# GRAPH-0/JODO

Hardware: AMD Instinct MI355X
Metric: molecules/sec (1000-step ancestral) (higher is better)
Workload: dtype f32

## Files before the change

include/jodo_hip.h:

```cpp
#ifndef JODO_HIP_H
#define JODO_HIP_H
#include <stddef.h>
#include <stdint.h>
#ifdef __cplusplus
extern "C" {
#endif

#define JODO_OK 0
#define JODO_ERR_ARG (-1)
#define JODO_ERR_LAUNCH (-2)
#define JODO_ERR_UNSUPPORTED (-3)

typedef struct {
    int32_t nf;
    int32_t n_layers;
    int32_t n_heads;
    int32_t n_extra;
    int32_t mlp_ratio;
    int32_t in_node_dim;
    int32_t edge_ch;
    int32_t cond_ch;
    float spatial_cut_off;
    float edge_quan_th;
    int32_t layout;
} jodo_cfg;

enum jodo_wslot_global {
    JW_TIME_FREQ = 0, JW_TIME_W1, JW_TIME_B1, JW_TIME_W3, JW_TIME_B3,
    JW_COND_W0, JW_COND_B0, JW_COND_W2, JW_COND_B2, JW_COND_LIN_W, JW_COND_LIN_B,
    JW_MOD_W, JW_MOD_B,
    JW_NODE_EMB_W, JW_NODE_EMB_B, JW_EDGE_EMB_W, JW_EDGE_EMB_B, JW_GBF_TOP,
    JW_NH1_W, JW_NH1_B, JW_NH2_W, JW_NH2_B, JW_NH3_W, JW_NH3_B,
    JW_EH1_W, JW_EH1_B, JW_EH2_W, JW_EH2_B, JW_EH3_W, JW_EH3_B,
    JW_GLOBAL_COUNT
};
enum jodo_wslot_block {
    JB_WQ = 0, JB_BQ, JB_WK, JB_BK, JB_WV, JB_BV,
    JB_EE_W, JB_EE_B, JB_LE0_W, JB_LE1_W, JB_N2E_W, JB_N2E_B,
    JB_FF1_W, JB_FF1_B, JB_FF2_W, JB_FF2_B, JB_FF3_W, JB_FF3_B, JB_FF4_W, JB_FF4_B,
    JB_INE_W, JB_ROW_W, JB_COL_W, JB_IN_B, JB_C0_W, JB_C0_B, JB_C2_W, JB_CSCALE,
    JB_NRO_W, JB_NRO_B, JB_ERO_W, JB_ERO_B, JB_GBF,
    JB_ROWQ_W, JB_COLQ_W, JB_INQ_B, JB_LQ_W, JB_INEC_W, JB_QT_W,
    JB_BLOCK_COUNT
};

typedef struct {
    const char* name;
    const float* data;
    const int64_t* shape;
    int32_t ndim;
} jodo_tensor;
int jodo_dgt_packed_size(const jodo_cfg* cfg, const jodo_tensor* tensors, int n_tensors, size_t* n_floats, int* n_woff);
int jodo_dgt_pack_weights_host(const jodo_cfg* cfg, const jodo_tensor* tensors, int n_tensors, float* packed_host,
                               size_t cap_floats, int64_t* woff_out, int n_woff);
int jodo_dgt_pack_weights(const jodo_cfg* cfg, const jodo_tensor* tensors, int n_tensors, void* packed_dev,
                          size_t cap_floats, int64_t* woff_out, int n_woff, void* stream);

typedef struct jodo_plan jodo_plan;

int jodo_plan_create(const jodo_cfg* cfg, int B, int N, const int32_t* n_nodes_host, int max_chunk,
                     jodo_plan** out);
void jodo_plan_destroy(jodo_plan* plan);
size_t jodo_plan_desc_bytes(const jodo_plan* plan);
size_t jodo_plan_workspace_bytes(const jodo_plan* plan);
int64_t jodo_plan_mod_len(const jodo_plan* plan);
int jodo_plan_upload(jodo_plan* plan, void* desc_dev, void* stream);
int jodo_plan_stats(const jodo_plan* plan, int64_t* out6);

int jodo_dgt_forward(jodo_plan* plan, const void* desc_dev, const float* packed_w, const int64_t* woff,
                     int n_woff, const float* xh, const float* edge_x, const float* cond_x,
                     const float* cond_edge_x, const float* noise_level, const float* context,
                     float* out_xh, float* out_edge, int32_t* flags_dev, void* workspace, void* stream);

int jodo_plan_work(const jodo_plan* plan, int uniform_t, int symmetric, double* mfma_flops_per_class);

enum jodo_plan_option {
    JODO_OPT_FUSE_NEXT_QKV = 0,
    JODO_OPT_DIR_SPLIT = 1,
    JODO_OPT_NODE_POST_WAVES = 2,
    JODO_OPT_ATTN_VARIANT = 3,
    JODO_OPT_PIN_SYMMETRIC = 4,
    JODO_OPT_PIN_UNIFORM_T = 5,
    JODO_OPT_ROT_STATS = 6,
    JODO_OPT_NODE_MIX = 7,
    JODO_OPT_HEADS_MIX = 8,
    JODO_OPT_HALF_ROWS = 9,
    JODO_OPT_PRE_EMBED = 10,
    JODO_OPT_AB_PRE = 11,
    JODO_OPT_Z_SPLIT = 12,
    JODO_OPT_SPLIT_BF16 = 13,
    JODO_OPT_COUNT
};
int jodo_plan_set_option(jodo_plan* plan, int option, int value);

int jodo_debug_attn_schedule(const jodo_plan* plan, int64_t* out8);

int jodo_debug_fetch(jodo_plan* plan, const void* workspace, int what, float* dst_dev, int64_t* count,
                     void* stream);
int jodo_debug_set_max_blocks(jodo_plan* plan, int max_blocks);
int jodo_debug_set_force_directed(jodo_plan* plan, int on);
int jodo_debug_set_timing_buffer(jodo_plan* plan, void* dev16xu64);

enum jodo_prof_class {
    JODO_PROF_PROLOGUE = 0, JODO_PROF_NODE_PRE, JODO_PROF_EDGE_ATTN, JODO_PROF_RESERVED3, JODO_PROF_RESERVED4,
    JODO_PROF_NODE_POST, JODO_PROF_EDGE_UPDATE, JODO_PROF_EPILOGUE, JODO_PROF_COUNT
};
int jodo_profile_enable(jodo_plan* plan, int enable);
int jodo_profile_read(jodo_plan* plan, float* ms_sum, int32_t* launches);

int jodo_sampler_step(int B, int N, int node_feats, int edge_ch, const int32_t* n_nodes_dev, float c_x, float c_pred,
                      float sigma, const float* x, const float* edge_x, const float* pred, const float* edge_pred,
                      const float* eps_pos, const float* eps_feat, const float* eps_edge, float* x_next,
                      float* edge_next, float* x_mean, float* edge_mean, void* stream);
int jodo_sampler_step_tab(int B, int N, int node_feats, int edge_ch, const int32_t* n_nodes_dev, const float* coef_tab_dev,
                          const int32_t* step_dev, const float* x, const float* edge_x, const float* pred,
                          const float* edge_pred, const float* eps_pos, const float* eps_feat, const float* eps_edge,
                          float* x_next, float* edge_next, float* x_mean, float* edge_mean, void* stream);
int jodo_sampler_step_rng(int B, int N, int node_feats, int edge_ch, const int32_t* n_nodes_dev, float c_x, float c_pred,
                          float sigma, const float* coef_tab_dev, const int32_t* step_dev, uint64_t seed, uint32_t draw,
                          const float* x, const float* edge_x, const float* pred, const float* edge_pred, float* x_next,
                          float* edge_next, float* x_mean, float* edge_mean, void* stream);
int jodo_step_begin(int B, const float* coef_tab_dev, const int32_t* step_dev, float* noise_level_out, void* stream);
int jodo_step_end(int32_t* step_dev, void* stream);
int jodo_dpm_update(int B, int N, int node_feats, int edge_ch, const int32_t* n_nodes_dev, const float* coef8_host,
                    const float* coef_tab_dev, const int32_t* step_dev, int tab_stride, int tab_col, const float* x_pos,
                    const float* x_base, const float* edge_base, const float* P, const float* eP, const float* DA, const float* eDA,
                    const float* DB, const float* eDB, const float* PP, const float* eps_pos, float* x_out, float* edge_out,
                    void* stream);
int jodo_dpm_update_rng(int B, int N, int node_feats, int edge_ch, const int32_t* n_nodes_dev, const float* coef8_host,
                        const float* coef_tab_dev, const int32_t* step_dev, int tab_stride, int tab_col, uint64_t seed,
                        uint32_t draw, uint32_t draw_mul, const float* x_pos, const float* x_base, const float* edge_base,
                        const float* P, const float* eP, const float* DA, const float* eDA, const float* DB, const float* eDB,
                        const float* PP, float* x_out, float* edge_out, void* stream);
int jodo_step_begin_at(int B, const float* coef_tab_dev, const int32_t* step_dev, int tab_stride, int tab_col,
                       float* noise_level_out, void* stream);
int jodo_decode(int B, int N, int atom_types, int include_fc, int edge_ch, int compress_edge, int centered,
                float pos_norm, float atom_norm, float fc_norm, float edge_norm, const int32_t* n_nodes_dev,
                const float* xh, const float* edge_x, float* pos_out, uint8_t* atom_type_out, int8_t* fc_out,
                uint8_t* edge_type_out, void* stream);

typedef struct jodo_train jodo_train;
int jodo_train_create(const jodo_cfg* cfg, int B, int N, const int32_t* n_nodes_host, const jodo_tensor* params, int n_params,
                      jodo_train** out);
void jodo_train_destroy(jodo_train* t);
size_t jodo_train_desc_bytes(const jodo_train* t);
size_t jodo_train_workspace_bytes(const jodo_train* t);
int jodo_train_set_option(jodo_train* t, int option, int value);
int jodo_train_debug_locate(const jodo_train* t, int what, int layer, size_t* byte_offset, size_t* count);
int jodo_train_upload(jodo_train* t, void* desc_dev, void* stream);
const void* jodo_train_desc_host(const jodo_train* t);
int jodo_train_forward(jodo_train* t, const void* desc_dev, const float* const* params_dev, int n_params, const float* xh,
                       const float* edge_x, const float* cond_x, const float* cond_edge_x, const float* noise_level,
                       const float* context, float dropout_p, uint64_t seed, float* out_xh, float* out_edge, int32_t* flags_out,
                       void* workspace, void* stream);
int jodo_train_backward(jodo_train* t, const void* desc_dev, const float* const* params_dev, float* const* grads_dev, int n_params,
                        const float* noise_level, const float* d_out_xh, const float* d_out_edge, float dropout_p, uint64_t seed,
                        void* workspace, void* stream);
int jodo_train_gemm(int tA, int tB, int M, int N, int K, const float* A, int lda, const float* B, int ldb, float* C, int ldc,
                    const float* bias, int acc, float* ws, size_t ws_floats, void* stream);
int jodo_train_gemm_ex(int tA, int tB, int M, int N, int K, const float* A, int lda, const float* B, int ldb, float* C, int ldc,
                       const float* bias, int act, float* out2, float* dbias, float* ws, size_t ws_floats, void* stream);

int jodo_adam_step(int64_t n, float* p, const float* g, float* m, float* v, float* vmax, double lr, double beta1, double beta2, double eps,
                   double weight_decay, int64_t step, int decoupled, int amsgrad, void* stream);
int jodo_gradnorm_clip(const float* norm_dev, double* state_dev, double max_grad, float* coef_dev, float* allowed_dev, void* stream);
int jodo_kabsch_rotations(int B, const float* A_dev, float* R_dev, void* stream);

typedef struct {
    int32_t nf, n_layers, n_heads, n_extra, mlp_ratio, in_node_dim, edge_ch;
    float edge_quan_th;
} jodo_cfg2d;
enum jodo2d_wslot_global {
    J2_TIME_FREQ = 0, J2_TIME_W1, J2_TIME_B1, J2_TIME_W3, J2_TIME_B3, J2_MOD_W, J2_MOD_B,
    J2_NODE_EMB_W, J2_NODE_EMB_B, J2_EDGE_EMB_W, J2_EDGE_EMB_B,
    J2_NH1_W, J2_NH1_B, J2_NH2_W, J2_NH2_B, J2_NH3_W, J2_NH3_B,
    J2_EH1_W, J2_EH1_B, J2_EH2_W, J2_EH2_B, J2_EH3_W, J2_EH3_B,
    J2_GLOBAL_COUNT
};
enum jodo2d_wslot_block {
    J2B_QKV_W = 0, J2B_QKV_B, J2B_LE_W, J2B_N2E_W, J2B_N2E_B, J2B_FF1_W, J2B_FF1_B, J2B_FF2_W, J2B_FF2_B,
    J2B_FF3_W, J2B_FF3_B, J2B_FF4_W, J2B_FF4_B, J2B_NRO_W, J2B_NRO_B, J2B_ERO_W, J2B_ERO_B,
    J2B_BLOCK_COUNT
};
int jodo_dgt2d_check_cfg(const jodo_cfg2d* cfg);
int jodo_dgt2d_packed_size(const jodo_cfg2d* cfg, size_t* n_floats, int* n_woff);
int jodo_dgt2d_pack_weights_host(const jodo_cfg2d* cfg, const jodo_tensor* tensors, int n_tensors, float* packed_host,
                                 size_t cap_floats, int64_t* woff_out, int n_woff);
int jodo_dgt2d_layout(const jodo_cfg2d* cfg, int B, int N, const int32_t* n_nodes_host, int64_t* out8);
int jodo_dgt2d_fill_desc(const jodo_cfg2d* cfg, int B, int N, const int32_t* n_nodes_host, int32_t* desc_host, int64_t n_words);
int jodo_dgt2d_forward(const jodo_cfg2d* cfg, int B, int N, const int32_t* n_nodes_host, const void* desc_dev, const float* packed_w,
                       const int64_t* woff, int n_woff, const float* xh, const float* edge_x, const float* cond_x,
                       const float* cond_edge_x, const float* noise_level, float* out_xh, float* out_edge, int32_t* flags_dev,
                       void* workspace, int force_directed, int max_blocks, void* stream);
enum jodo2d_walk { JODO_2D_WALK_DIRECTED = 0, JODO_2D_WALK_PAIR = 1 };
int jodo_dgt2d_pair_layout(const jodo_cfg2d* cfg, int B, int N, const int32_t* n_nodes_host, int64_t* out8);
int jodo_dgt2d_pair_fill_desc(const jodo_cfg2d* cfg, int B, int N, const int32_t* n_nodes_host, int32_t* desc_host, int64_t n_words);
int jodo_dgt2d_forward_walk(const jodo_cfg2d* cfg, int B, int N, const int32_t* n_nodes_host, const void* desc_dev,
                            const void* pair_desc_dev, int walk, const float* packed_w, const int64_t* woff, int n_woff, const float* xh,
                            const float* edge_x, const float* cond_x, const float* cond_edge_x, const float* noise_level, float* out_xh,
                            float* out_edge, int32_t* flags_dev, void* workspace, int force_directed, int max_blocks, void* stream);
int jodo_dgt2d_split_size(const jodo_cfg2d* cfg, size_t* tape_bytes, int64_t* toff_out, int n_woff);
int jodo_dgt2d_pack_split_host(const jodo_cfg2d* cfg, const float* packed_host, const int64_t* woff, int n_woff, void* tape_host,
                               size_t cap_bytes);
int jodo_dgt2d_forward_split(const jodo_cfg2d* cfg, int B, int N, const int32_t* n_nodes_host, const void* desc_dev,
                             const void* pair_desc_dev, int walk, const float* packed_w, const int64_t* woff, int n_woff,
                             const void* tape_dev, const int64_t* toff, const float* xh, const float* edge_x, const float* cond_x,
                             const float* cond_edge_x, const float* noise_level, float* out_xh, float* out_edge, int32_t* flags_dev,
                             void* workspace, int force_directed, int max_blocks, void* stream);
int jodo_debug_gemm2d(int split, const float* x, int rows, int K, int n_out, const void* w_dev, const float* bias, int act, float* y,
                      void* stream);
int jodo_sampler_step_2d(int B, int N, int node_feats, int edge_ch, const int32_t* n_nodes_dev, float cx, float cp, float sigma,
                         const float* x, const float* edge_x, const float* pred, const float* edge_pred, const float* eps_node,
                         const float* eps_edge, float* x_next, float* edge_next, float* x_mean, float* edge_mean, void* stream);
int jodo_sampler_step_2d_rng(int B, int N, int node_feats, int edge_ch, const int32_t* n_nodes_dev, float c_x, float c_pred, float sigma,
                             const float* coef_tab_dev, const int32_t* step_dev, uint64_t seed, uint32_t draw, const float* x,
                             const float* edge_x, const float* pred, const float* edge_pred, float* x_next, float* edge_next,
                             float* x_mean, float* edge_mean, void* stream);
int jodo_dpm_update_2d(int B, int N, int node_feats, int edge_ch, const int32_t* n_nodes_dev, const float* coef8_host,
                       const float* coef_tab_dev, const int32_t* step_dev, int tab_stride, int tab_col, const float* x_base,
                       const float* edge_base, const float* P, const float* eP, const float* DA, const float* eDA, const float* DB,
                       const float* eDB, float* x_out, float* edge_out, void* stream);
int jodo_decode_2d(int B, int N, int atom_types, int include_fc, int edge_ch, int compress_edge, int centered, float atom_norm,
                   float fc_norm, float edge_norm, const int32_t* n_nodes_dev, const float* xh, const float* edge_x,
                   uint8_t* atom_type_out, int8_t* fc_out, uint8_t* edge_type_out, void* stream);

typedef struct jodo_train2d jodo_train2d;
int jodo_train2d_create(const jodo_cfg2d* cfg, int B, int N, const int32_t* n_nodes_host, const jodo_tensor* params, int n_params,
                        jodo_train2d** out);
void jodo_train2d_destroy(jodo_train2d* t);
size_t jodo_train2d_desc_bytes(const jodo_train2d* t);
size_t jodo_train2d_workspace_bytes(const jodo_train2d* t);
const void* jodo_train2d_desc_host(const jodo_train2d* t);
int jodo_train2d_upload(jodo_train2d* t, void* desc_dev, void* stream);
int jodo_train2d_set_option(jodo_train2d* t, int option, int value);
int jodo_train2d_debug_locate(const jodo_train2d* t, int what, int layer, size_t* byte_offset, size_t* count);
int jodo_train2d_forward(jodo_train2d* t, const void* desc_dev, const float* const* params_dev, int n_params, const float* xh,
                         const float* edge_x, const float* cond_x, const float* cond_edge_x, const float* noise_level,
                         const float* context, float dropout_p, uint64_t seed, float* out_xh, float* out_edge, int32_t* flags_out,
                         void* workspace, void* stream);
int jodo_train2d_backward(jodo_train2d* t, const void* desc_dev, const float* const* params_dev, float* const* grads_dev, int n_params,
                          const float* noise_level, const float* d_out_xh, const float* d_out_edge, float dropout_p, uint64_t seed,
                          void* workspace, void* stream);

const char* jodo_last_error(void);

int jodo_debug_mfma_peak(int iters, int chains, int waves_per_simd, float* sink_dev, float* tflops_out);

int jodo_debug_mfma_valu(int iters, int nv, int nt, int waves_per_simd, float* sink_dev, float* tflops_out);

int jodo_dgt_split_size(const jodo_cfg* cfg, size_t* total_bytes, size_t* pair_block_bytes, size_t* node_block_bytes, size_t* attn_block_bytes);
int jodo_dgt_pack_split_host(const jodo_cfg* cfg, const jodo_tensor* tensors, int n_tensors, void* host, size_t cap_bytes);
int jodo_plan_set_split_weights(jodo_plan* plan, const void* tape_dev, size_t bytes);
int jodo_dgt_split_cond_size(const jodo_cfg* cfg, size_t* total_bytes, size_t* pair_block_bytes);
int jodo_dgt_pack_split_cond_host(const jodo_cfg* cfg, const jodo_tensor* tensors, int n_tensors, void* host, size_t cap_bytes);

int jodo_debug_mfma_bf16_valu(int iters, int nv, int chains, int waves_per_simd, float* sink_dev, float* tflops_out);
int jodo_debug_pack_split(const float* W, int n_out, int n_in, float* f32_packed_host, void* split_packed_host);
int jodo_debug_chain(int mode, int K, int tiles, const float* x, int rows, const float* wf, const void* wsp, float* y, int iters,
                     float* ms_out, void* stream);

int jodo_debug_mlp(const float* x, int rows, const float* w1, const float* b1, const float* w2,
                   const float* b2, float* y, void* stream);

#ifdef __cplusplus
}
#endif
#endif
```

jodo_amd/capi.py:

```python
import ctypes
import os

_HERE = os.path.dirname(os.path.abspath(__file__))
LIB_PATH = os.environ.get('JODO_HIP_LIB') or os.path.join(_HERE, 'csrc', 'libjodo_hip.so')
_lib = None


class JodoHipError(RuntimeError):
    pass


def lib():
    global _lib
    if _lib is None:
        if not os.path.isfile(LIB_PATH):
            raise JodoHipError(
                "libjodo_hip.so not found at %s — the HIP extension is required (no CPU fallback). "
                "Build it with: python -c 'import __graft_entry__ as g; g.build()'" % LIB_PATH)
        _lib = ctypes.CDLL(LIB_PATH)
        _lib.jodo_last_error.restype = ctypes.c_char_p
        _bind_2d_sampling(_lib)
        _bind_2d_pair(_lib)
        _bind_2d_split(_lib)
    return _lib


def _bind_2d_sampling(L):
    i, f, p = ctypes.c_int, ctypes.c_float, ctypes.c_void_p
    try:
        step, dec, dpm = L.jodo_sampler_step_2d_rng, L.jodo_decode_2d, L.jodo_dpm_update_2d
    except AttributeError as e:
        raise JodoHipError("%s lacks the 2-D sampling exports (%s): rebuild it with python -c 'import __graft_entry__ as g; g.build()'"
                           % (LIB_PATH, e))
    step.argtypes = [i, i, i, i, p, f, f, f, p, p, ctypes.c_uint64, ctypes.c_uint32] + [p] * 9
    dec.argtypes = [i] * 7 + [f, f, f] + [p] * 7
    dpm.argtypes = [i, i, i, i, p, p, p, p, i, i] + [p] * 11
    step.restype = dec.restype = dpm.restype = i


WALK_DIRECTED, WALK_PAIR = 0, 1


def _bind_2d_pair(L):
    i, p = ctypes.c_int, ctypes.c_void_p
    try:
        lay, fill, fwd = L.jodo_dgt2d_pair_layout, L.jodo_dgt2d_pair_fill_desc, L.jodo_dgt2d_forward_walk
    except AttributeError as e:
        raise JodoHipError("%s lacks the 2-D pair-walk exports (%s): rebuild it with python -c 'import __graft_entry__ as g; g.build()'"
                           % (LIB_PATH, e))
    lay.argtypes = [p, i, i, p, p]
    fill.argtypes = [p, i, i, p, p, ctypes.c_int64]
    fwd.argtypes = [p, i, i, p, p, p, i, p, p, i] + [p] * 9 + [i, i, p]
    lay.restype = fill.restype = fwd.restype = i


def _bind_2d_split(L):
    i, p = ctypes.c_int, ctypes.c_void_p
    try:
        size, pack, fwd, dbg = L.jodo_dgt2d_split_size, L.jodo_dgt2d_pack_split_host, L.jodo_dgt2d_forward_split, L.jodo_debug_gemm2d
    except AttributeError as e:
        raise JodoHipError("%s lacks the 2-D split-bf16 exports (%s): rebuild it with python -c 'import __graft_entry__ as g; g.build()'"
                           % (LIB_PATH, e))
    size.argtypes = [p, p, p, i]
    pack.argtypes = [p, p, p, i, p, ctypes.c_size_t]
    fwd.argtypes = [p, i, i, p, p, p, i, p, p, i, p, p] + [p] * 9 + [i, i, p]
    dbg.argtypes = [i, p, i, i, i, p, p, i, p, p]
    size.restype = pack.restype = fwd.restype = dbg.restype = i


def check(code, what=''):
    if code != 0:
        msg = lib().jodo_last_error()
        raise JodoHipError("%s failed (%d): %s" % (what, code, msg.decode() if msg else ''))


def ptr(t):
    if t is None:
        return ctypes.c_void_p(0)
    return ctypes.c_void_p(t.data_ptr())


def current_stream_ptr():
    import torch
    return ctypes.c_void_p(torch.cuda.current_stream().cuda_stream)


class JodoTensor(ctypes.Structure):
    _fields_ = [('name', ctypes.c_char_p), ('data', ctypes.c_void_p), ('shape', ctypes.POINTER(ctypes.c_int64)),
                ('ndim', ctypes.c_int32)]


_PACKED_SIZE = {}


def pack_weights(cfg_struct, state_dict, device=None):
    import numpy as np
    import torch
    L = lib()
    keep, arr = [], (JodoTensor * len(state_dict))()
    for i, (k, v) in enumerate(state_dict.items()):
        t = np.ascontiguousarray(v.detach().float().cpu().numpy())
        shp = (ctypes.c_int64 * max(t.ndim, 1))(*t.shape)
        name = k.encode()
        keep.append((t, shp, name))
        arr[i] = JodoTensor(name, t.ctypes.data_as(ctypes.c_void_p), shp, t.ndim)
    key = bytes(cfg_struct)
    n_floats, n_woff = ctypes.c_size_t(), ctypes.c_int()
    if key in _PACKED_SIZE:
        n_floats.value, n_woff.value = _PACKED_SIZE[key]
    else:
        check(L.jodo_dgt_packed_size(ctypes.byref(cfg_struct), arr, len(keep), ctypes.byref(n_floats), ctypes.byref(n_woff)),
              'jodo_dgt_packed_size')
        _PACKED_SIZE[key] = (n_floats.value, n_woff.value)
    woff = (ctypes.c_int64 * n_woff.value)()
    if device is None:
        blob = torch.empty(n_floats.value, dtype=torch.float32)
        check(L.jodo_dgt_pack_weights_host(ctypes.byref(cfg_struct), arr, len(keep), ctypes.c_void_p(blob.data_ptr()),
                                           ctypes.c_size_t(n_floats.value), woff, n_woff.value), 'jodo_dgt_pack_weights_host')
    else:
        blob = torch.empty(n_floats.value, dtype=torch.float32, device=device)
        check(L.jodo_dgt_pack_weights(ctypes.byref(cfg_struct), arr, len(keep), ctypes.c_void_p(blob.data_ptr()),
                                      ctypes.c_size_t(n_floats.value), woff, n_woff.value, current_stream_ptr()),
              'jodo_dgt_pack_weights')
    return blob, woff, n_woff.value


def pack_weights_2d(cfg_struct, state_dict, device=None):
    import numpy as np
    import torch
    L = lib()
    keep, arr = [], (JodoTensor * len(state_dict))()
    for i, (k, v) in enumerate(state_dict.items()):
        t = np.ascontiguousarray(v.detach().float().cpu().numpy())
        shp = (ctypes.c_int64 * max(t.ndim, 1))(*t.shape)
        name = k.encode()
        keep.append((t, shp, name))
        arr[i] = JodoTensor(name, t.ctypes.data_as(ctypes.c_void_p), shp, t.ndim)
    n_floats, n_woff = ctypes.c_size_t(), ctypes.c_int()
    check(L.jodo_dgt2d_packed_size(ctypes.byref(cfg_struct), ctypes.byref(n_floats), ctypes.byref(n_woff)), 'jodo_dgt2d_packed_size')
    woff = (ctypes.c_int64 * n_woff.value)()
    blob = torch.empty(n_floats.value, dtype=torch.float32)
    check(L.jodo_dgt2d_pack_weights_host(ctypes.byref(cfg_struct), arr, len(keep), ctypes.c_void_p(blob.data_ptr()),
                                         ctypes.c_size_t(n_floats.value), woff, n_woff.value), 'jodo_dgt2d_pack_weights_host')
    return (blob if device is None else blob.to(device)), woff, n_woff.value


def split_tape_2d(cfg_struct, blob_host, woff, n_woff, device=None):
    import torch
    L = lib()
    total = ctypes.c_size_t()
    toff = (ctypes.c_int64 * n_woff)()
    check(L.jodo_dgt2d_split_size(ctypes.byref(cfg_struct), ctypes.byref(total), toff, n_woff), 'jodo_dgt2d_split_size')
    tape = torch.empty(total.value, dtype=torch.uint8)
    check(L.jodo_dgt2d_pack_split_host(ctypes.byref(cfg_struct), ctypes.c_void_p(blob_host.data_ptr()), woff, n_woff,
                                       ctypes.c_void_p(tape.data_ptr()), ctypes.c_size_t(total.value)), 'jodo_dgt2d_pack_split_host')
    return (tape if device is None else tape.to(device)), toff


def pack_split_tape(cfg_struct, state_dict, device=None):
    import numpy as np
    import torch
    L = lib()
    keep, arr = [], (JodoTensor * len(state_dict))()
    for i, (k, v) in enumerate(state_dict.items()):
        t = np.ascontiguousarray(v.detach().float().cpu().numpy())
        shp = (ctypes.c_int64 * max(t.ndim, 1))(*t.shape)
        name = k.encode()
        keep.append((t, shp, name))
        arr[i] = JodoTensor(name, t.ctypes.data_as(ctypes.c_void_p), shp, t.ndim)
    total, per_block, node_block, attn_block = ctypes.c_size_t(), ctypes.c_size_t(), ctypes.c_size_t(), ctypes.c_size_t()
    check(L.jodo_dgt_split_size(ctypes.byref(cfg_struct), ctypes.byref(total), ctypes.byref(per_block), ctypes.byref(node_block), ctypes.byref(attn_block)),
          'jodo_dgt_split_size')
    tape = torch.empty(total.value, dtype=torch.uint8)
    check(L.jodo_dgt_pack_split_host(ctypes.byref(cfg_struct), arr, len(keep), ctypes.c_void_p(tape.data_ptr()), ctypes.c_size_t(total.value)),
          'jodo_dgt_pack_split_host')
    return tape if device is None else tape.to(device)


def pack_split_cond_tape(cfg_struct, state_dict, device=None):
    import numpy as np
    import torch
    L = lib()
    keep, arr = [], (JodoTensor * len(state_dict))()
    for i, (k, v) in enumerate(state_dict.items()):
        t = np.ascontiguousarray(v.detach().float().cpu().numpy())
        shp = (ctypes.c_int64 * max(t.ndim, 1))(*t.shape)
        name = k.encode()
        keep.append((t, shp, name))
        arr[i] = JodoTensor(name, t.ctypes.data_as(ctypes.c_void_p), shp, t.ndim)
    total, per_block = ctypes.c_size_t(), ctypes.c_size_t()
    check(L.jodo_dgt_split_cond_size(ctypes.byref(cfg_struct), ctypes.byref(total), ctypes.byref(per_block)), 'jodo_dgt_split_cond_size')
    tape = torch.empty(total.value, dtype=torch.uint8)
    check(L.jodo_dgt_pack_split_cond_host(ctypes.byref(cfg_struct), arr, len(keep), ctypes.c_void_p(tape.data_ptr()), ctypes.c_size_t(total.value)),
          'jodo_dgt_pack_split_cond_host')
    return tape if device is None else tape.to(device)
```

jodo_amd/csrc/dgt_forward.hip:

```cpp
#include "dgt_kernels_pre.h"
#include "dgt_kernels_node.h"
#include "dgt_kernels_split_node.h"
#include "dgt_kernels_post.h"
#include "dgt_kernels_wide.h"
#include "jodo_hip_internal.h"
#include "dgt_launch.h"
#include <memory>
#include <utility>

using namespace jd;

namespace {

PlanDev make_plan_dev(const jodo_plan* p, const void* desc_dev) {
    const int* base = static_cast<const int*>(desc_dev);
    PlanDev d;
    d.node_b = base + p->off_node_b; d.node_i = base + p->off_node_i; d.node_n = base + p->off_node_n;
    d.node_noff = base + p->off_node_noff; d.node_eoff = base + p->off_node_eoff;
    d.orig_n = base + p->off_orig_n; d.orig_noff = base + p->off_orig_noff; d.orig_eoff = base + p->off_orig_eoff;
    d.item_strip = base + p->off_item_strip; d.item_t0 = base + p->off_item_t0; d.item_t1 = base + p->off_item_t1;
    d.item_part = base + p->off_item_part; d.strip_parts = base + p->off_strip_parts;
    d.pitem_strip = base + p->off_pitem_strip; d.pitem_t0 = base + p->off_pitem_t0; d.pitem_t1 = base + p->off_pitem_t1;
    d.n_pitems = p->n_pitems;
    d.ag_node = base + p->off_ag_node; d.ai_group = base + p->off_ai_group; d.ai_t0 = base + p->off_ai_t0; d.ai_t1 = base + p->off_ai_t1;
    d.ai_part = base + p->off_ai_part; d.ai_dir = base + p->off_ai_dir; d.ad_group = base + p->off_ad_group; d.ad_t0 = base + p->off_ad_t0; d.ad_t1 = base + p->off_ad_t1;
    d.ad_part = base + p->off_ad_part; d.ad_big = base + p->off_ad_big; d.anode_parts = base + p->off_anode_parts;
    d.aw_off = base + p->off_aw_off; d.a_persist = p->a_persist;
    d.n_agroups = p->n_agroups; d.n_aitems = p->n_aitems; d.n_aditems = p->n_aditems; d.amax_parts = p->amax_parts;
    d.Nn = p->Nn; d.Nn_pad = p->Nn_pad; d.n_strips = p->n_strips; d.n_items = p->n_items; d.B = p->B; d.N = p->N;
    d.max_parts = p->max_parts; d.rows = p->rows;
    d.ut_rows = base + p->off_ut_rows; d.n_ut_pad = p->n_ut_pad;
    d.gt_sa = base + p->off_gt_sa; d.gt_sc = base + p->off_gt_sc; d.n_gtiles = p->n_gtiles;
    return d;
}

template <typename T>
T* ws_ptr(void* ws, size_t off) { return reinterpret_cast<T*>(static_cast<char*>(ws) + off); }

void fill_ws(KArgs& A, const jodo_plan* p, void* ws) {
    const WsLayout& w = p->ws;
    A.hid1 = ws_ptr<float>(ws, w.hid1); A.temb = ws_ptr<float>(ws, w.temb); A.mods = ws_ptr<float>(ws, w.mods);
    A.condh = ws_ptr<float>(ws, w.condh); A.condh2 = ws_ptr<float>(ws, w.condh2);
    A.dpos = ws_ptr<float>(ws, w.dpos); A.cpos = ws_ptr<float>(ws, w.cpos); A.feat = ws_ptr<float>(ws, w.feat);
    A.h = ws_ptr<float>(ws, w.h); A.hhat = ws_ptr<float>(ws, w.hhat); A.astat = ws_ptr<float>(ws, w.astat); A.q = ws_ptr<float>(ws, w.q);
    A.k = ws_ptr<float>(ws, w.k); A.v = ws_ptr<float>(ws, w.v); A.n2e = ws_ptr<float>(ws, w.n2e);
    A.wrow = ws_ptr<float>(ws, w.wrow); A.wcol = ws_ptr<float>(ws, w.wcol); A.ua = ws_ptr<float>(ws, w.ua); A.ub = ws_ptr<float>(ws, w.ub);
    A.rmean = ws_ptr<float>(ws, w.rmean); A.mfold = ws_ptr<float>(ws, w.mfold); A.ffold = ws_ptr<float>(ws, w.ffold); A.ahid = ws_ptr<float>(ws, w.ahid);
    A.apred = ws_ptr<float>(ws, w.apred);
    A.eflag = ws_ptr<int>(ws, w.eflag); A.e = ws_ptr<float>(ws, w.e);
    A.ehid = ws_ptr<float>(ws, w.ehid); A.epred = ws_ptr<float>(ws, w.epred);
    A.e_out = ws_ptr<float>(ws, w.e2);
    A.dposE = ws_ptr<float>(ws, w.dposE); A.gramE = ws_ptr<float>(ws, w.gramE);
    A.wsplit = nullptr; A.wsplit_node = nullptr; A.wsplit_attn = nullptr; A.mfold_s = nullptr; A.ffold_s = nullptr; A.split_cond = 0;
}

int rowgemm(hipStream_t st, const float* X, int64_t ldx, float* Y, int64_t ldy, const float* Wp, const float* bias,
            int rows, int K, int NB, int in_act, int accumulate, const int* uniform_flag, float* Ysilu = nullptr) {
    if (K % 64 != 0) return jodo_set_error(JODO_ERR_ARG, "rowgemm: K=%d not a multiple of 64", K);
    const int nob = (rows <= 64 || uniform_flag) ? 1 : 4;
    const int gx = uniform_flag ? 1 : 0;
    RowGemmArgs G{X, ldx, Y, ldy, Wp, bias, rows, K, NB, in_act, accumulate, uniform_flag, nob, gx, Ysilu};
    dim3 grid((rows + 31) / 32, (NB + nob - 1) / nob);
    if (gx) grid = dim3(grid.y, grid.x);
    hipLaunchKernelGGL(k_rowgemm, grid, dim3(64), 0, st, G);
    return jodo_check_launch("k_rowgemm");
}

struct ProfScope {
    jodo_plan* p; hipStream_t st; int cls; bool on;
    static hipEvent_t get(jodo_plan* p) {
        if (!p->prof_pool.empty()) { hipEvent_t e = (hipEvent_t)p->prof_pool.back(); p->prof_pool.pop_back(); return e; }
        hipEvent_t e; (void)hipEventCreate(&e); return e;
    }
    ProfScope(jodo_plan* p_, hipStream_t st_, int cls_)
        : p(p_), st(st_), cls(cls_), on(p_->prof_enabled == 1 || (p_->prof_enabled == 2 && cls_ == JODO_PROF_EDGE_UPDATE) || p_->prof_enabled == 16 + cls_) {
        if (on) { hipEvent_t e = get(p); (void)hipEventRecord(e, st); p->prof_ev.push_back(e); }
    }
    ~ProfScope() {
        if (on) { hipEvent_t e = get(p); (void)hipEventRecord(e, st); p->prof_ev.push_back(e); p->prof_cls.push_back(cls); }
    }
};

template <int D, int KQ>
int launch_embed_nodes(hipStream_t st, const KArgs& A) {
    LAUNCH((wide::k_embed_nodes<D, KQ>), A.pd.n_strips, 64, A);
    return JODO_OK;
}
template <int D, int NBK>
int launch_edge_head(hipStream_t st, const KArgs& A, bool merged) {
    if (merged) {
        LAUNCH((wide::k_heads_sym<D, NBK>), (unsigned)(A.pd.n_strips + A.pd.n_ut_pad / 32), 64, A);
        return JODO_OK;
    }
    LAUNCH((wide::k_node_head<D>), A.pd.n_strips, 64, A);
    if (A.pd.n_ut_pad > 0 && A.pin_sym != 2) LAUNCH((wide::k_edge_head<D, NBK, true>), (unsigned)(A.pd.n_ut_pad / 32), 64, A);
    if (A.pin_sym != 1) LAUNCH((wide::k_edge_head<D, NBK, false>), (unsigned)((A.pd.rows + 31) / 32), 64, A);
    return JODO_OK;
}

__global__ __launch_bounds__(64, 1) void k_pre_embed(KArgs A) {
    const int npre = A.pd.n_strips * 3;
    if ((int)blockIdx.x < npre) node_pre_body<false>(A, (int)blockIdx.x);
    else wide::embed_edges_body<256>(A, (int)blockIdx.x - npre);
}


__global__ __launch_bounds__(64, 1) void k_node_ab_pre(KArgs A) {
    const int npre = A.mix_nw, nab = A.ab1 - A.ab0;
    const int b = (int)blockIdx.x;
    if (b < npre) node_pre_body<true>(A, b);
    else if (b < npre + nab) wide::node_ab_body<256>(A, A.ab0 + b - npre);
    else wide::node_gram_body<256>(A, A.g0 + b - npre - nab);
}

template <int D>
__global__ __launch_bounds__(64, 1) void k_node_ab_pre_w(KArgs A) {
    const int npre = A.mix_nw, nab = A.ab1 - A.ab0;
    const int b = (int)blockIdx.x;
    if (b < npre) wide::node_pre_body<D, true>(A, b);
    else if (b < npre + nab) wide::node_ab_body<D>(A, A.ab0 + b - npre);
    else wide::node_gram_body<D>(A, A.g0 + b - npre - nab);
}
template <int D>
__global__ __launch_bounds__(64, 1) void k_pre_embed_w(KArgs A) {
    const int npre = A.pd.n_strips * 3;
    if ((int)blockIdx.x < npre) wide::node_pre_body<D, false>(A, (int)blockIdx.x);
    else wide::embed_edges_body<D>(A, (int)blockIdx.x - npre);
}

template <int R, int NW>
__global__ __launch_bounds__(NW * 64, 1) void k_node_mix(KArgs A) {
    __shared__ float4 part[NW * 8 * 4 * 64];
    const int wg = blockIdx.x, wave = threadIdx.x >> 6;
    if (wg < A.mix_nw) { node_postw_body<R, NW>(A, wg + A.strip0, part); return; }
    const int nab = (A.ab1 - A.ab0 + NW - 1) / NW;
    if (wg < A.mix_nw + nab) {
        const int it = A.ab0 + (wg - A.mix_nw) * NW + wave;
        if (it < A.ab1) wide::node_ab_body<256>(A, it);
        return;
    }
    const int t = A.g0 + (wg - A.mix_nw - nab) * NW + wave;
    if (t < A.g1) wide::node_gram_body<256>(A, t);
}

int launch_node_post_256(jodo_plan* p, hipStream_t st, KArgs& A, bool with_ab, bool next_pre) {
    const DgtDims& d = p->dims;
    const int force = p->opt[JODO_OPT_NODE_POST_WAVES];
    const bool rem_only = force >= 10;
    const int full = (force && !rem_only) ? (force == 1 ? p->n_strips : 0) : (p->n_strips / 1024) * 1024;
    const int rem = p->n_strips - full;
    const int nw = rem_only ? force - 10 : (force ? force : (rem <= 256 ? 4 : (rem <= 512 ? 2 : 1)));
    const bool split_node = A.wsplit_node != nullptr && A.rot == 1;
    if (split_node) {
        A.strip0 = 0;
        const int wgs = (p->n_strips + 3) / 4;
        if (d.r == 2) { LAUNCH((split::k_node_post_split<2, 1>), wgs, split::SPLIT_WAVES * 64, A); LAUNCH((split::k_node_post_split<2, 2>), wgs, split::SPLIT_WAVES * 64, A); }
        else { LAUNCH((split::k_node_post_split<4, 1>), wgs, split::SPLIT_WAVES * 64, A); LAUNCH((split::k_node_post_split<4, 2>), wgs, split::SPLIT_WAVES * 64, A); }
    }
    const bool split_ab = split_node && with_ab && A.ffold_s != nullptr && !next_pre;
    if (split_ab) {
        A.ab0 = 0; A.ab1 = 2 * p->n_strips;
        LAUNCH(split::k_node_ab_split, (2 * p->n_strips + split::SPLIT_WAVES - 1) / split::SPLIT_WAVES, split::SPLIT_WAVES * 64, A);
    }
    if (full > 0 && !split_node) {
        A.strip0 = 0;
        if (d.r == 2) LAUNCH(k_node_post<2>, full, 64, A); else LAUNCH(k_node_post<4>, full, 64, A);
    }
    A.ab0 = 0; A.ab1 = 2 * p->n_strips; A.g0 = 0; A.g1 = A.rot ? p->n_gtiles : 0; A.mix_nw = 0;
    const bool mix = !split_node && with_ab && full > 0 && rem > 0 && nw >= 2 && p->opt[JODO_OPT_NODE_MIX] != 0;
    if (mix) {
        if (p->gt_cache_full != full) {
            const int32_t* sa = p->desc.data() + p->off_gt_sa, *sc = p->desc.data() + p->off_gt_sc;
            int c = 0;
            while (c < p->n_gtiles && sa[c] < full && sc[c] < full) ++c;
            p->gt_cache_full = full; p->gt_cache_count = c;
        }
        const int gpre = A.rot ? p->gt_cache_count : 0;
        A.strip0 = full; A.mix_nw = rem; A.ab0 = 0; A.ab1 = 2 * full; A.g0 = 0; A.g1 = gpre;
        const int g1 = rem + (A.ab1 - A.ab0 + nw - 1) / nw + (A.g1 - A.g0 + nw - 1) / nw;
        if (nw == 2) { if (d.r == 2) LAUNCH((k_node_mix<2, 2>), g1, 128, A); else LAUNCH((k_node_mix<4, 2>), g1, 128, A); }
        else { if (d.r == 2) LAUNCH((k_node_mix<2, 4>), g1, 256, A); else LAUNCH((k_node_mix<4, 4>), g1, 256, A); }
        A.strip0 = 0; A.mix_nw = 0; A.ab0 = 2 * full; A.ab1 = 2 * p->n_strips; A.g0 = gpre; A.g1 = A.rot ? p->n_gtiles : 0;
        const int g2 = (A.ab1 - A.ab0 + 1) / 2 + (A.g1 - A.g0 + 1) / 2;
        if (d.r == 2) LAUNCH((k_node_mix<2, 2>), g2, 128, A); else LAUNCH((k_node_mix<4, 2>), g2, 128, A);
        A.ab0 = 0; A.g0 = 0;
        return JODO_OK;
    }
    if (rem > 0 && !split_node) {
        A.strip0 = full;
        if (nw == 1) { if (d.r == 2) LAUNCH(k_node_post<2>, rem, 64, A); else LAUNCH(k_node_post<4>, rem, 64, A); }
        else if (nw == 2) { if (d.r == 2) LAUNCH((k_node_postw<2, 2>), rem, 128, A); else LAUNCH((k_node_postw<4, 2>), rem, 128, A); }
        else { if (d.r == 2) LAUNCH((k_node_postw<2, 4>), rem, 256, A); else LAUNCH((k_node_postw<4, 4>), rem, 256, A); }
    }
    A.strip0 = 0;
    if (next_pre) {
        A.mix_nw = 3 * p->n_strips;
        if (!with_ab) { A.ab1 = A.ab0; A.g1 = A.g0; }
        LAUNCH(k_node_ab_pre, A.mix_nw + (A.ab1 - A.ab0) + (A.g1 - A.g0), 64, A);
        A.mix_nw = 0;
        return JODO_OK;
    }
    if (with_ab) {
        if (!split_ab) LAUNCH((wide::k_node_ab<256>), p->n_strips * 2, 64, A);
        if (A.rot && p->n_gtiles > 0) LAUNCH((wide::k_node_gram<256>), p->n_gtiles, 64, A);
    }
    return JODO_OK;
}

template <int D, bool TUNED>
int forward_blocks(jodo_plan* p, hipStream_t st, KArgs& A, const int64_t* woff, float* const posbuf[2], std::unique_ptr<ProfScope>& pro) {
    const DgtDims& d = p->dims;
    int rc = JODO_OK;
    LAUNCH(k_pack_nodes, (p->Nn_pad + 255) / 256, 256, A);
    switch (d.ndp / 8) {
        case 1: rc = launch_embed_nodes<D, 1>(st, A); break;
        case 2: rc = launch_embed_nodes<D, 2>(st, A); break;
        case 3: rc = launch_embed_nodes<D, 3>(st, A); break;
        case 4: rc = launch_embed_nodes<D, 4>(st, A); break;
        case 5: rc = launch_embed_nodes<D, 5>(st, A); break;
        case 6: rc = launch_embed_nodes<D, 6>(st, A); break;
        case 7: rc = launch_embed_nodes<D, 7>(st, A); break;
        case 8: rc = launch_embed_nodes<D, 8>(st, A); break;
        default: return jodo_set_error(JODO_ERR_UNSUPPORTED, "node input width %d", d.ndp);
    }
    if (rc) return rc;
    const bool embed_merged = p->n_items > 0 && p->opt[JODO_OPT_PRE_EMBED] != 0 && ((p->max_blocks >= 0 && p->max_blocks < d.L) ? p->max_blocks : d.L) > 0;
    if (p->n_items > 0 && !embed_merged) LAUNCH((wide::k_embed_edges<D>), p->n_items, 64, A);
    const bool pin_pair = p->opt[JODO_OPT_PIN_SYMMETRIC] == 1 && !p->force_directed, pin_dir = p->opt[JODO_OPT_PIN_SYMMETRIC] == 2 || p->force_directed;
    const bool can_fold = p->n_pitems > 0 && !pin_dir && p->opt[JODO_OPT_PIN_UNIFORM_T] != 2 && d.cond_ch == 0;
    A.rot = can_fold ? p->opt[JODO_OPT_ROT_STATS] : 0;
    if (can_fold) {
        if (d.L > 16) return jodo_set_error(JODO_ERR_UNSUPPORTED, "more than 16 blocks");
        FoldOffs F;
        for (int l = 0; l < 16; ++l) {
            F.c0[l] = l < d.L ? woff[JW_GLOBAL_COUNT + l * JB_BLOCK_COUNT + JB_C0_W] : 0;
            F.ine[l] = l < d.L ? woff[JW_GLOBAL_COUNT + l * JB_BLOCK_COUNT + (A.rot ? JB_INEC_W : JB_INE_W)] : 0;
        }
        LAUNCH((wide::k_fold_coord<D, D / 16>), d.L * (D / 32) * (d.De / 4), 64, A, F, A.mfold, 0, A.mfold_s);
        if (A.rot) {
            for (int l = 0; l < d.L; ++l) F.ine[l] = woff[JW_GLOBAL_COUNT + l * JB_BLOCK_COUNT + JB_QT_W];
            LAUNCH((wide::k_fold_coord<D, D / 8>), d.L * (D / 32) * (D / 8), 64, A, F, A.ffold, 1, A.ffold_s);
        }
    }
    pro.reset();
    const int nblocks = (p->max_blocks >= 0 && p->max_blocks < d.L) ? p->max_blocks : d.L;
    const bool fuse_pre = TUNED && p->opt[JODO_OPT_FUSE_NEXT_QKV] != 0 && nblocks > 1 && p->n_strips >= 1024;
    const bool ab_pre = !fuse_pre && p->opt[JODO_OPT_AB_PRE] != 0 && nblocks > 1 && (!TUNED || (p->n_strips < 1024 && p->opt[JODO_OPT_NODE_POST_WAVES] == 0));
    int cur = 0;
    for (int l = 0; l < nblocks; ++l) {
        A.layer = l;
        A.mod_base = 32 + (int64_t)l * d.MB;
        for (int i = 0; i < JB_BLOCK_COUNT; ++i) A.wb[i] = woff[JW_GLOBAL_COUNT + l * JB_BLOCK_COUNT + i];
        A.wsplit = nullptr; A.wsplit_node = nullptr; A.wsplit_attn = nullptr;
        if (A.mfold_s) {
            size_t total = 0, pair_block = 0, node_block = 0, attn_block = 0;
            (void)jodo_dgt_split_size(&p->cfg, &total, &pair_block, &node_block, &attn_block);
            const char* base = static_cast<const char*>(p->split_w);
            A.wsplit = reinterpret_cast<const unsigned short*>(base + (size_t)l * pair_block);
            if (node_block > 0) A.wsplit_node = reinterpret_cast<const unsigned short*>(base + (size_t)d.L * pair_block + (size_t)l * node_block);
            if (attn_block > 0 && p->opt[JODO_OPT_SPLIT_BF16] == 2) A.wsplit_attn = reinterpret_cast<const unsigned short*>(base + (size_t)d.L * (pair_block + node_block) + (size_t)l * attn_block);
        } else if (A.split_cond) {
            size_t total = 0, pair_block = 0;
            (void)jodo_dgt_split_cond_size(&p->cfg, &total, &pair_block);
            A.wsplit = reinterpret_cast<const unsigned short*>(static_cast<const char*>(p->split_w) + (size_t)l * pair_block);
        }
        A.pos_in = posbuf[cur]; A.pos_out = posbuf[cur ^ 1];
        {
            ProfScope ps(p, st, JODO_PROF_NODE_PRE);
            if constexpr (TUNED) {
                if (!fuse_pre && !ab_pre) {
                    A.pre_mode = 0;
                    if (l == 0 && embed_merged) LAUNCH(k_pre_embed, p->n_strips * 3 + p->n_items, 64, A);
                    else LAUNCH(k_node_pre, p->n_strips * 3, 64, A);
                } else {
                    LAUNCH(k_pos_final, (p->Nn_pad + 255) / 256, 256, A);
                    if (l == 0) {
                        A.pre_mode = 1;
                        if (embed_merged) LAUNCH(k_pre_embed, p->n_strips * 3 + p->n_items, 64, A);
                        else LAUNCH(k_node_pre, p->n_strips * 3, 64, A);
                    }
                }
            } else if (!ab_pre) {
                A.pre_mode = 0;
                if (l == 0 && embed_merged) LAUNCH((k_pre_embed_w<D>), p->n_strips * 3 + p->n_items, 64, A);
                else LAUNCH((wide::k_node_pre<D>), p->n_strips * 3, 64, A);
            } else {
                LAUNCH(k_pos_final, (p->Nn_pad + 255) / 256, 256, A);
                if (l == 0) {
                    A.pre_mode = 1;
                    if (embed_merged) LAUNCH((k_pre_embed_w<D>), p->n_strips * 3 + p->n_items, 64, A);
                    else LAUNCH((wide::k_node_pre<D>), p->n_strips * 3, 64, A);
                }
            }
        }
        cur ^= 1;
        {
            ProfScope ps(p, st, JODO_PROF_EDGE_ATTN);
            rc = jd_launch_edge_attn(p, st, A, D, TUNED, pin_pair, pin_dir);
            if (rc) return rc;
        }
        {
            ProfScope ps(p, st, JODO_PROF_NODE_POST);
            if constexpr (TUNED) {
                A.fuse_next = (fuse_pre && l + 1 < nblocks) ? 1 : 0;
                const bool next_pre = ab_pre && l + 1 < nblocks;
                if (A.fuse_next || next_pre) {
                    static const int slots[6] = {JB_WQ, JB_BQ, JB_WK, JB_BK, JB_WV, JB_BV};
                    for (int i = 0; i < 6; ++i) A.wbn[i] = woff[JW_GLOBAL_COUNT + (l + 1) * JB_BLOCK_COUNT + slots[i]];
                    A.mod_base_next = 32 + (int64_t)(l + 1) * d.MB;
                }
                rc = launch_node_post_256(p, st, A, p->n_pitems > 0 && !pin_dir, next_pre);
                if (rc) return rc;
            } else {
                if (d.r == 2) LAUNCH((wide::k_node_post<D, 2>), p->n_strips, 64, A); else LAUNCH((wide::k_node_post<D, 4>), p->n_strips, 64, A);
                A.ab0 = 0; A.g0 = 0;
                const bool with_ab = p->n_pitems > 0 && !pin_dir;
                if (ab_pre && l + 1 < nblocks) {
                    static const int slots[6] = {JB_WQ, JB_BQ, JB_WK, JB_BK, JB_WV, JB_BV};
                    for (int i = 0; i < 6; ++i) A.wbn[i] = woff[JW_GLOBAL_COUNT + (l + 1) * JB_BLOCK_COUNT + slots[i]];
                    A.mod_base_next = 32 + (int64_t)(l + 1) * d.MB;
                    A.mix_nw = 3 * p->n_strips;
                    A.ab1 = with_ab ? 2 * p->n_strips : 0;
                    A.g1 = (with_ab && A.rot) ? p->n_gtiles : 0;
                    LAUNCH((k_node_ab_pre_w<D>), A.mix_nw + A.ab1 + A.g1, 64, A);
                    A.mix_nw = 0;
                } else {
                    if (with_ab) LAUNCH((wide::k_node_ab<D>), p->n_strips * 2, 64, A);
                    if (A.rot && p->n_gtiles > 0) LAUNCH((wide::k_node_gram<D>), p->n_gtiles, 64, A);
                }
            }
        }
        if (p->n_items > 0) {
            ProfScope ps(p, st, JODO_PROF_EDGE_UPDATE);
            rc = jd_launch_edge_update(p, st, A, D, pin_pair, pin_dir);
            if (rc) return rc;
            std::swap(A.e, A.e_out);
            p->last_e_buf ^= 1;
        }
    }
    ProfScope epi(p, st, JODO_PROF_EPILOGUE);
    A.pos_in = posbuf[cur]; A.pos_out = posbuf[cur ^ 1];
    A.layer = nblocks;
    LAUNCH(k_pos_final, (p->Nn_pad + 255) / 256, 256, A);
    p->last_pos_buf = cur ^ 1;
    const bool heads_mix = A.pin_sym == 1 && A.pd.n_ut_pad > 0 && p->opt[JODO_OPT_HEADS_MIX] != 0;
    switch (d.KEH / 32) {
        case 3: rc = launch_edge_head<D, 3>(st, A, heads_mix); break;
        case 4: rc = launch_edge_head<D, 4>(st, A, heads_mix); break;
        case 5: rc = launch_edge_head<D, 5>(st, A, heads_mix); break;
        case 6: rc = launch_edge_head<D, 6>(st, A, heads_mix); break;
        case 7: rc = launch_edge_head<D, 7>(st, A, heads_mix); break;
        case 8: rc = launch_edge_head<D, 8>(st, A, heads_mix); break;
        case 9: rc = launch_edge_head<D, 9>(st, A, heads_mix); break;
        case 10: rc = launch_edge_head<D, 10>(st, A, heads_mix); break;
        case 11: rc = launch_edge_head<D, 11>(st, A, heads_mix); break;
        case 12: rc = launch_edge_head<D, 12>(st, A, heads_mix); break;
        case 13: rc = launch_edge_head<D, 13>(st, A, heads_mix); break;
        case 15: rc = launch_edge_head<D, 15>(st, A, heads_mix); break;
        default: return jodo_set_error(JODO_ERR_UNSUPPORTED, "edge head width %d", d.KEH);
    }
    if (rc) return rc;
    LAUNCH(k_finalize_nodes, (p->B * p->N + 255) / 256, 256, A);
    {
        const size_t tot = (size_t)p->B * p->N * p->N;
        LAUNCH(k_finalize_edges, (unsigned)((tot + 255) / 256), 256, A);
    }
    return JODO_OK;
}

}

extern "C" int jodo_dgt_forward(jodo_plan* p, const void* desc_dev, const float* packed_w, const int64_t* woff,
                                int n_woff, const float* xh, const float* edge_x, const float* cond_x,
                                const float* cond_edge_x, const float* noise_level, const float* context,
                                float* out_xh, float* out_edge, int32_t* flags_dev, void* workspace, void* stream) {
    if (!p || !desc_dev || !packed_w || !woff || !xh || !edge_x || !noise_level || !out_xh || !out_edge || !flags_dev ||
        !workspace)
        return jodo_set_error(JODO_ERR_ARG, "dgt_forward: null argument");
    const DgtDims& d = p->dims;
    if (n_woff != JW_GLOBAL_COUNT + d.L * JB_BLOCK_COUNT)
        return jodo_set_error(JODO_ERR_ARG, "dgt_forward: weight table has %d slots, expected %d", n_woff,
                              JW_GLOBAL_COUNT + d.L * JB_BLOCK_COUNT);
    if ((cond_x == nullptr) != (cond_edge_x == nullptr))
        return jodo_set_error(JODO_ERR_ARG, "dgt_forward: cond_x and cond_edge_x must both be given or both NULL");
    if (d.cond_ch > 0 && !context) return jodo_set_error(JODO_ERR_ARG, "dgt_forward: conditional model needs context");
    hipStream_t st = (hipStream_t)stream;

    KArgs A;
    A.pd = make_plan_dev(p, desc_dev);
    A.d = d;
    A.W = packed_w;
    for (int i = 0; i < JW_GLOBAL_COUNT; ++i) A.wg[i] = woff[i];
    for (int i = 0; i < JB_BLOCK_COUNT; ++i) A.wb[i] = 0;
    A.mod_base = 0; A.layer = 0; A.force_directed = p->force_directed; A.pin_sym = p->force_directed ? 0 : p->opt[JODO_OPT_PIN_SYMMETRIC];
    A.half_rows = (A.pin_sym == 1 && p->n_pitems > 0 && p->opt[JODO_OPT_HALF_ROWS] != 0) ? 1 : 0;
    A.pin_uni = p->opt[JODO_OPT_PIN_UNIFORM_T]; A.pre_mode = 0; A.strip0 = 0; A.item0 = 0; A.dir_split = 0; A.rot = 0; A.mix_nw = 0; A.ab0 = 0; A.ab1 = 0; A.g0 = 0; A.g1 = 0; A.fuse_next = 0; A.mod_base_next = 0;
    for (int i = 0; i < 6; ++i) A.wbn[i] = 0;
    fill_ws(A, p, workspace);
    if (p->opt[JODO_OPT_SPLIT_BF16] >= 1 && p->split_w && (d.D == 256 || d.D == 384) && d.cond_ch == 0 && !p->force_directed && p->n_pitems > 0 && p->pitems_single &&
        p->opt[JODO_OPT_PIN_SYMMETRIC] == 1 && p->opt[JODO_OPT_PIN_UNIFORM_T] == 1 && p->opt[JODO_OPT_ROT_STATS] == 1) {
        size_t total = 0, per_block = 0, node_block = 0, attn_block = 0;
        if (jodo_dgt_split_size(&p->cfg, &total, &per_block, &node_block, &attn_block) == JODO_OK && total == p->split_bytes)
            A.mfold_s = ws_ptr<unsigned short>(workspace, p->ws.mfold_s);
        if (A.mfold_s && node_block > 0) A.ffold_s = ws_ptr<unsigned short>(workspace, p->ws.ffold_s);
    }
    if (p->opt[JODO_OPT_SPLIT_BF16] >= 1 && p->split_w && d.D == 256 && d.cond_ch > 0 && !p->force_directed && p->n_pitems > 0 && p->pitems_single &&
        p->opt[JODO_OPT_PIN_SYMMETRIC] == 1 && p->opt[JODO_OPT_PIN_UNIFORM_T] == 2) {
        size_t total = 0, per_block = 0;
        if (jodo_dgt_split_cond_size(&p->cfg, &total, &per_block) == JODO_OK && total == p->split_bytes) A.split_cond = 1;
    }
    float* posbuf[2] = {ws_ptr<float>(workspace, p->ws.pos0), ws_ptr<float>(workspace, p->ws.pos1)};
    A.pos_in = posbuf[0]; A.pos_out = posbuf[1];
    A.flags = flags_dev;
    A.dbgt = static_cast<unsigned long long*>(p->dbg_timing);
    A.xh = xh; A.edge_x = edge_x; A.cond_x = cond_x; A.cond_edge_x = cond_edge_x; A.noise = noise_level; A.context = context;
    A.out_xh = out_xh; A.out_edge = out_edge;
    const float* W = packed_w;
    int rc;

    p->last_e_buf = 0;
    std::unique_ptr<ProfScope> pro(new ProfScope(p, st, JODO_PROF_PROLOGUE));
    LAUNCH(k_flags_init, 1, 256, A);
    { const size_t tot = (size_t)p->B * p->N * p->N; LAUNCH(k_check_sym, (unsigned)((tot + 255) / 256), 256, A); }
    LAUNCH(k_time1, p->B, 256, A);
    const int* uflag = d.cond_ch > 0 ? nullptr : flags_dev + FLAG_UNIFORM_T;
    float* tembs = ws_ptr<float>(workspace, p->ws.tembs);
    rc = rowgemm(st, A.hid1, d.T, A.temb, d.T, W + A.wg[JW_TIME_W3], W + A.wg[JW_TIME_B3], p->B, d.T, d.T / 32, 0, 0, uflag,
                 d.cond_ch > 0 ? nullptr : tembs);
    if (rc) return rc;
    if (d.cond_ch > 0) {
        LAUNCH(k_cond1, p->B * d.cond_ch, 256, A);
        rc = rowgemm(st, A.condh, d.D, A.condh2, d.D, W + A.wg[JW_COND_W2], W + A.wg[JW_COND_B2], p->B * d.cond_ch, d.D,
                     d.D / 32, 0, 0, nullptr);
        if (rc) return rc;
        rc = rowgemm(st, A.condh2, (int64_t)d.cond_ch * d.D, A.temb, d.T, W + A.wg[JW_COND_LIN_W], W + A.wg[JW_COND_LIN_B],
                     p->B, d.cond_ch * d.D, d.T / 32, 0, 1, nullptr, tembs);
        if (rc) return rc;
    }
    rc = rowgemm(st, tembs, d.T, A.mods, d.Mtot, W + A.wg[JW_MOD_W], W + A.wg[JW_MOD_B], p->B, d.T, (int)(d.Mtot / 32), 0, 0,
                 uflag);
    if (rc) return rc;
    if (!d.wide) return forward_blocks<256, true>(p, st, A, woff, posbuf, pro);
    if (d.D == 128) return forward_blocks<128, false>(p, st, A, woff, posbuf, pro);
    return d.D == 256 ? forward_blocks<256, false>(p, st, A, woff, posbuf, pro) : forward_blocks<384, false>(p, st, A, woff, posbuf, pro);
}

extern "C" int jodo_debug_fetch(jodo_plan* p, const void* workspace, int what, float* dst, int64_t* count, void* stream) {
    if (!p || !workspace || !dst || !count) return jodo_set_error(JODO_ERR_ARG, "debug_fetch: null");
    const char* ws = static_cast<const char*>(workspace);
    const void* src = nullptr;
    int64_t n = 0;
    switch (what) {
        case 0: src = ws + p->ws.h; n = (int64_t)p->Nn * p->dims.D; break;
        case 1: src = ws + (p->last_e_buf ? p->ws.e2 : p->ws.e); n = p->rows * p->dims.De; break;
        case 2: src = ws + (p->last_pos_buf ? p->ws.pos1 : p->ws.pos0); n = (int64_t)p->Nn * 4; break;
        case 3: src = ws + p->ws.hhat; n = (int64_t)p->Nn * p->amax_parts * p->dims.D; break;
        case 5: src = ws + p->ws.mods; n = p->dims.Mtot; break;
        case 6: src = ws + p->ws.q; n = (int64_t)p->Nn * p->dims.QKP; break;
        default: return jodo_set_error(JODO_ERR_ARG, "debug_fetch: unknown selector %d", what);
    }
    hipError_t e = hipMemcpyAsync(dst, src, (size_t)n * sizeof(float), hipMemcpyDeviceToDevice, (hipStream_t)stream);
    if (e != hipSuccess) return jodo_set_error(JODO_ERR_LAUNCH, "debug_fetch: %s", hipGetErrorString(e));
    *count = n;
    return JODO_OK;
}
```

jodo_amd/csrc/dgt_kernels_common.h:

```cpp
#pragma once
#include "dgt_device.h"
#include "dgt_plan.h"

enum { FLAG_NAN = 0, FLAG_FIRST = 1, FLAG_UNIFORM_T = 2, FLAG_COND_NONZERO = 3, FLAG_ASYM = 4, FLAG_NAN_COUNT = 5, FLAG_PIN_VIOLATED = 6 };

struct KArgs {
    PlanDev pd;
    DgtDims d;
    const float* W;
    int64_t wg[JW_GLOBAL_COUNT];
    int64_t wb[JB_BLOCK_COUNT];
    int64_t mod_base;
    int layer;
    int force_directed;
    int pin_sym, pin_uni;
    int strip0;
    int half_rows;
    int item0, dir_split;
    int mix_nw, ab0, ab1, g0, g1;
    int rot;
    int fuse_next;
    int64_t wbn[6];
    int64_t mod_base_next;
    int pre_mode;
    float *hid1, *temb, *mods, *condh, *condh2;
    float *pos_in, *pos_out, *dpos, *cpos, *feat, *h, *hhat, *astat, *q, *k, *v, *n2e, *wrow, *wcol, *ua, *ub, *rmean, *mfold, *ffold, *ahid, *apred;
    int* eflag;
    float *e, *ehid, *epred, *dposE, *gramE;
    float* e_out;
    const unsigned short* wsplit;
    const unsigned short* wsplit_attn;
    const unsigned short* wsplit_node;
    unsigned short* mfold_s;
    unsigned short* ffold_s;
    int split_cond;
    int* flags;
    unsigned long long* dbgt;
    const float *xh, *edge_x, *cond_x, *cond_edge_x, *noise, *context;
    float *out_xh, *out_edge;
};

struct FoldOffs { int64_t c0[16], ine[16]; };

namespace jd {

constexpr int PAIR_GROUP_LANES = 128;

__device__ __forceinline__ bool rot_active(const KArgs& A) { return A.rot && A.flags[FLAG_UNIFORM_T] && !A.flags[FLAG_ASYM]; }
}

namespace jd {

__device__ __forceinline__ const float4* wq(const KArgs& A, int64_t off, int lane) {
    return reinterpret_cast<const float4*>(A.W + off) + lane;
}

__device__ __forceinline__ const float* mod_row(const KArgs& A, int node_b) {
    const int trow = A.flags[FLAG_UNIFORM_T] ? 0 : node_b;
    return A.mods + (size_t)trow * A.d.Mtot;
}

struct LaneNode {
    int v, b, i, n, noff, eoff;
    bool valid;
};

__device__ __forceinline__ LaneNode lane_node(const KArgs& A, int strip, int j) {
    LaneNode L;
    L.v = strip * 32 + j;
    L.b = A.pd.node_b[L.v];
    L.i = A.pd.node_i[L.v];
    L.n = A.pd.node_n[L.v];
    L.noff = A.pd.node_noff[L.v];
    L.eoff = A.pd.node_eoff[L.v];
    L.valid = L.n > 0;
    return L;
}

__device__ __forceinline__ float4 advance_position(const KArgs& A, float4 p, int v, int strip, int n, int i, int eoff) {
    double sx = 0., sy = 0., sz = 0.;
    if (A.flags[FLAG_ASYM]) {
        const int parts = A.pd.strip_parts[strip];
        for (int q = 0; q < parts; ++q) {
            const float4 dp = reinterpret_cast<const float4*>(A.dpos)[(size_t)v * A.pd.max_parts + q];
            sx += dp.x; sy += dp.y; sz += dp.z;
        }
    } else {
        const float4* row = reinterpret_cast<const float4*>(A.dposE) + (size_t)eoff + (size_t)i * n;
        int c = 0;
        for (; c + 8 <= n; c += 8) {
            float4 d[8];
#pragma unroll
            for (int u = 0; u < 8; ++u) d[u] = row[c + u];
#pragma unroll
            for (int u = 0; u < 8; ++u)
                if (c + u != i) { sx += d[u].x; sy += d[u].y; sz += d[u].z; }
        }
        for (; c + 4 <= n; c += 4) {
            const float4 d0 = row[c], d1 = row[c + 1], d2 = row[c + 2], d3 = row[c + 3];
            if (c != i) { sx += d0.x; sy += d0.y; sz += d0.z; }
            if (c + 1 != i) { sx += d1.x; sy += d1.y; sz += d1.z; }
            if (c + 2 != i) { sx += d2.x; sy += d2.y; sz += d2.z; }
            if (c + 3 != i) { sx += d3.x; sy += d3.y; sz += d3.z; }
        }
        for (; c < n; ++c) {
            if (c == i) continue;
            const float4 dp = row[c];
            sx += dp.x; sy += dp.y; sz += dp.z;
        }
    }
    p.x += (float)sx; p.y += (float)sy; p.z += (float)sz;
    return p;
}

__device__ __forceinline__ float gelu_erf(float x) { return 0.5f * x * (1.f + erff(x * 0.70710678118654752f)); }

}
```

jodo_amd/csrc/dgt_kernels_wide.h:

```cpp
#pragma once
#include "dgt_kernels_common.h"
#include "dgt_kernels_attn.h"

namespace jd {
namespace wide {

constexpr int NHEAD_BLOCKS = 14;

template <int D_>
struct Dim {
    static constexpr int D = D_, De = D_ / 4, ND = D_ / 32, NE = D_ / 128;
    static constexpr int HD = D_ / 2, HE = D_ / 8;
    static constexpr int KQD = D_ / 8, KQE = D_ / 32;
    static constexpr int PG = (D_ % 256 == 0) ? 8 : 4;
    static constexpr int C = D_ / 16;
    static constexpr float INV_SQRT_C = D_ == 256 ? 0.25f : (D_ == 384 ? 0.20412414523193150f : (D_ == 128 ? 0.35355339059327379f : 0.f));
    static constexpr int M_EDGE = 6 * D_, M_EQUI = 6 * D_ + 6 * (D_ / 4), M_GBF = 6 * D_ + 6 * (D_ / 4) + 2 * D_;
    static constexpr int M_WG = M_GBF + 32, M_BS = M_WG + D_;
};

template <int D, int KQ>
__global__ __launch_bounds__(64) void k_embed_nodes(KArgs A) {
    using X = Dim<D>;
    const int lane = threadIdx.x & 63, j = lane & 31, half = lane >> 5;
    const int v = blockIdx.x * 32 + j;
    float x[KQ * 4];
    const float4* src = reinterpret_cast<const float4*>(A.feat + (size_t)v * (KQ * 8) + half * (KQ * 4));
#pragma unroll
    for (int q = 0; q < KQ; ++q) {
        const float4 t = src[q];
        x[q * 4 + 0] = t.x; x[q * 4 + 1] = t.y; x[q * 4 + 2] = t.z; x[q * 4 + 3] = t.w;
    }
    const float4* w = wq(A, A.wg[JW_NODE_EMB_W], lane);
    const float* bias = A.W + A.wg[JW_NODE_EMB_B];
#pragma unroll
    for (int b = 0; b < X::ND; ++b) {
        f32x16 acc = mfma_block<KQ>(w + (size_t)b * KQ * 64, x, zero16());
        float r[16];
        acc_bias(acc, bias + b * 32 + half * 16, r);
        store16(A.h + (size_t)v * D + b * 32 + half * 16, r);
        store16(A.ahid + (size_t)v * A.d.KNH + b * 32 + half * 16, r);
    }
}

template <int D>
__device__ __forceinline__ void embed_edges_body(const KArgs& A, int it) {
    using X = Dim<D>;
    const int lane = threadIdx.x & 63, j = lane & 31, half = lane >> 5;
    const int strip = A.pd.item_strip[it], t0 = A.pd.item_t0[it], t1 = A.pd.item_t1[it];
    const LaneNode L = lane_node(A, strip, j);
    const int ch = A.d.ch;
    const bool first = A.flags[FLAG_COND_NONZERO] == 0;
    const float* mr = mod_row(A, L.b);
    const float gscale = mr[0], gshift = mr[1];
    const float4 pc = reinterpret_cast<const float4*>(A.cpos)[L.v];
    const float* tab = A.W + A.wg[JW_GBF_TOP];
    const float4* w = wq(A, A.wg[JW_EDGE_EMB_W], lane);
    const float* bias = A.W + A.wg[JW_EDGE_EMB_B];
    for (int t = t0; t < t1; ++t) {
        const bool ok = L.valid && t < L.n;
        const int tc = ok ? t : 0;
        const int u = L.noff + tc;
        const size_t r = (size_t)L.eoff + (size_t)L.i * L.n + tc;
        int dd = tc - L.i;
        if (dd < 0) dd += L.n;
        const bool wr = ok && (!A.half_rows || L.n > PAIR_GROUP_LANES || (dd != 0 && (2 * dd < L.n || (2 * dd == L.n && 2 * L.i < L.n))));
        const float4 pu = reinterpret_cast<const float4*>(A.cpos)[u];
        const float dx = pc.x - pu.x, dy = pc.y - pu.y, dz = pc.z - pu.z;
        const float d2c = dx * dx + dy * dy + dz * dz;
        const size_t din = (((size_t)L.b * A.pd.N + L.i) * A.pd.N + tc) * ch;
        float ein[4];
#pragma unroll
        for (int s = 0; s < 4; ++s) {
            const int f = half * 4 + s;
            float val = 0.f;
            if (f < ch) val = A.edge_x[din + f];
            else if (f < 2 * ch && A.cond_edge_x) val = A.cond_edge_x[din + (f - ch)];
            ein[s] = val;
        }
        int adj2d = 1;
        if (A.cond_edge_x) adj2d = A.cond_edge_x[din] >= A.d.edge_th ? 1 : 0;
        const int adjsp = d2c <= A.d.cutoff ? 1 : 0;
        float G[X::HE];
        if (first) {
#pragma unroll
            for (int s = 0; s < X::HE; ++s) G[s] = 0.f;
        } else {
            gbf_n<X::NE>(d2c, gscale, gshift, tab, half, G);
        }
#pragma unroll
        for (int b = 0; b < X::NE; ++b) {
            f32x16 acc = mfma_block<X::KQE>(w + (size_t)(b * (X::KQE + 1)) * 64, G, zero16());
            acc = mfma_block<1>(w + (size_t)(b * (X::KQE + 1) + X::KQE) * 64, ein, acc);
            float rr[16];
            acc_bias(acc, bias + b * 32 + half * 16, rr);
            if (wr) {
                store16(A.e + r * X::De + b * 32 + half * 16, rr);
                store16(A.ehid + r * A.d.KEH + b * 32 + half * 16, rr);
            }
        }
        if (ok && half == 0) A.eflag[r] = adj2d | (adjsp << 1);
    }
}
template <int D>
__global__ __launch_bounds__(64) void k_embed_edges(KArgs A) { embed_edges_body<D>(A, (int)blockIdx.x); }

template <int D, bool NEXT = false>
__device__ __forceinline__ void node_pre_body(const KArgs& A, int blk) {
    using X = Dim<D>;
    const int lane = threadIdx.x & 63, j = lane & 31, half = lane >> 5;
    const int strip = blk / 3, piece = blk % 3;
    const LaneNode L = lane_node(A, strip, j);
    if (!NEXT && piece == 0 && A.pre_mode == 0) {
        float4 p = reinterpret_cast<const float4*>(A.pos_in)[L.v];
        if (A.layer > 0) p = advance_position(A, p, L.v, strip, L.n, L.i, L.eoff);
        if (half == 0) reinterpret_cast<float4*>(A.pos_out)[L.v] = p;
    }
    const float* mr = mod_row(A, L.b) + (NEXT ? A.mod_base_next : A.mod_base);
    float hx[X::HD];
    load_nat<X::ND>(A.h + (size_t)L.v * D, half, hx);
    layer_norm<X::HD>(hx);
    modulate<X::ND>(hx, mr, mr + D, half);
    const WSrc ws = make_wsrc(A.W, lane);
    const unsigned woff = (unsigned)((NEXT ? A.wbn[2 * piece] : A.wb[piece == 0 ? JB_WQ : (piece == 1 ? JB_WK : JB_WV)]) * 4);
    const float* bias = A.W + (NEXT ? A.wbn[2 * piece + 1] : A.wb[piece == 0 ? JB_BQ : (piece == 1 ? JB_BK : JB_BV)]);
    float* outp = piece == 0 ? A.q : (piece == 1 ? A.k : A.v);
    const int nb = piece == 2 ? X::ND : NHEAD_BLOCKS;
    WPipe<X::PG> wp;
    wpipe_prime(wp, ws, woff);
#pragma unroll 1
    for (int b = 0; b < nb; ++b) {
        const unsigned cur = woff + (unsigned)b * X::KQD * 1024;
        const unsigned nxt = b + 1 < nb ? cur + X::KQD * 1024 : woff;
        float bb[16], r[16];
        load16(bias + b * 32 + half * 16, bb);
        f32x16 acc = mfma_block_p<X::KQD>(wp, ws, cur, nxt, hx, zero16());
#pragma unroll
        for (int s = 0; s < 16; ++s) r[s] = acc[s] + bb[s];
        store16T(outp, nb, L.v, half, b, r);
    }
}
template <int D>
__global__ __launch_bounds__(64, 1) void k_node_pre(KArgs A) { node_pre_body<D, false>(A, (int)blockIdx.x); }

template <int D, int R>
__global__ __launch_bounds__(64, 1) void k_node_post(KArgs A) {
    using X = Dim<D>;
    constexpr int NPASS = 1, NOB = X::ND / NPASS;
    constexpr int NCH = R * D / 64;
    constexpr int KQ2 = R * D / 8;
    const int lane = threadIdx.x & 63, j = lane & 31, half = lane >> 5;
    const int strip = blockIdx.x;
    const LaneNode L = lane_node(A, strip, j);
    const float* mr = mod_row(A, L.b) + A.mod_base;
    const float* ng1 = mr + 2 * D, *ns2 = mr + 3 * D, *nc2 = mr + 4 * D, *ng2 = mr + 5 * D;
    const WSrc ws = make_wsrc(A.W, lane);
    const unsigned oN2E = (unsigned)(A.wb[JB_N2E_W] * 4), oF1 = (unsigned)(A.wb[JB_FF1_W] * 4), oF2 = (unsigned)(A.wb[JB_FF2_W] * 4);
    const bool rot = rot_active(A);
    const unsigned oRow = (unsigned)(A.wb[rot ? JB_ROWQ_W : JB_ROW_W] * 4), oCol = (unsigned)(A.wb[rot ? JB_COLQ_W : JB_COL_W] * 4), oNro = (unsigned)(A.wb[JB_NRO_W] * 4);
    WPipe<X::PG> wp;
    wpipe_prime(wp, ws, oN2E);
    float hx[X::HD];
    attn_merge<D>(A, L.v, half, hx);
#pragma unroll
    for (int b = 0; b < X::NE; ++b) {
        const unsigned cur = oN2E + (unsigned)b * X::KQD * 1024;
        f32x16 acc = mfma_block_p<X::KQD>(wp, ws, cur, b + 1 < X::NE ? cur + X::KQD * 1024 : oF1, hx, zero16());
        float r[16];
#pragma unroll
        for (int s = 0; s < 16; ++s) r[s] = acc[s];
        store16T(A.n2e, X::NE, L.v, half, b, r);
    }
    {
        const float* hrow = A.h + (size_t)L.v * D;
#pragma unroll
        for (int b = 0; b < X::ND; ++b) {
            float g[16], h0[16];
            load16(ng1 + b * 32 + half * 16, g);
            load16(hrow + b * 32 + half * 16, h0);
#pragma unroll
            for (int s = 0; s < 16; ++s) hx[b * 16 + s] = fmaf(g[s], hx[b * 16 + s], h0[s]);
        }
        layer_norm<X::HD>(hx);
        modulate<X::ND>(hx, ns2, nc2, half);
    }
    {
        const float* b1 = A.W + A.wb[JB_FF1_B];
        const float* b2 = A.W + A.wb[JB_FF2_B];
        float* hrow = A.h + (size_t)L.v * D;
#pragma unroll
        for (int ps = 0; ps < NPASS; ++ps) {
            f32x16 o[NOB];
#pragma unroll
            for (int b = 0; b < NOB; ++b) o[b] = zero16();
#pragma unroll 1
            for (int c = 0; c < NCH; ++c) {
                float hid[32];
#pragma unroll
                for (int b2i = 0; b2i < 2; ++b2i) {
                    const unsigned cur = oF1 + (unsigned)(c * 2 + b2i) * X::KQD * 1024;
                    const unsigned nxt = b2i == 0 ? cur + X::KQD * 1024 : oF2 + (unsigned)((ps * NOB) * KQ2 + c * 8) * 1024;
                    float bb[16];
                    load16(b1 + (c * 2 + b2i) * 32 + half * 16, bb);
                    f32x16 acc = mfma_block_p<X::KQD>(wp, ws, cur, nxt, hx, zero16());
                    silu_bias16(acc, bb, hid + b2i * 16);
                }
#pragma unroll
                for (int ob = 0; ob < NOB; ++ob) {
                    const unsigned cur = oF2 + (unsigned)((ps * NOB + ob) * KQ2 + c * 8) * 1024;
                    const unsigned nxt = ob + 1 < NOB ? oF2 + (unsigned)((ps * NOB + ob + 1) * KQ2 + c * 8) * 1024
                                                      : (c + 1 < NCH ? oF1 + (unsigned)((c + 1) * 2) * X::KQD * 1024
                                                                     : (ps + 1 < NPASS ? oF1 : oRow));
                    o[ob] = mfma_block_p<8>(wp, ws, cur, nxt, hid, o[ob]);
                }
            }
#pragma unroll
            for (int ob = 0; ob < NOB; ++ob) {
                const int b = ps * NOB + ob;
                float bb[16], g[16], r[16];
                load16(b2 + b * 32 + half * 16, bb);
                load16(ng2 + b * 32 + half * 16, g);
#pragma unroll
                for (int s = 0; s < 16; ++s) r[s] = fmaf(g[s], o[ob][s] + bb[s], hx[b * 16 + s]);
                store16(hrow + b * 32 + half * 16, r);
            }
        }
        load_nat<X::ND>(hrow, half, hx);
    }
    {
        const float* bin = A.W + A.wb[rot ? JB_INQ_B : JB_IN_B];
#pragma unroll 1
        for (int b = 0; b < X::ND; ++b) {
            const unsigned cr = oRow + (unsigned)b * X::KQD * 1024, cc = oCol + (unsigned)b * X::KQD * 1024;
            float bb[16], r[16];
            load16(bin + b * 32 + half * 16, bb);
            f32x16 acc = mfma_block_p<X::KQD>(wp, ws, cr, cc, hx, zero16());
#pragma unroll
            for (int s = 0; s < 16; ++s) r[s] = acc[s] + bb[s];
            store16T(A.wrow, X::ND, L.v, half, b, r);
            acc = mfma_block_p<X::KQD>(wp, ws, cc, b + 1 < X::ND ? cr + X::KQD * 1024 : oNro, hx, zero16());
#pragma unroll
            for (int s = 0; s < 16; ++s) r[s] = acc[s];
            store16T(A.wcol, X::ND, L.v, half, b, r);
        }
    }
    {
        const float* bias = A.W + A.wb[JB_NRO_B];
        const int nro = A.d.cnp / 32;
#pragma unroll 1
        for (int b = 0; b < nro; ++b) {
            const unsigned cur = oNro + (unsigned)b * X::KQD * 1024;
            float bb[16], r[16];
            load16(bias + b * 32 + half * 16, bb);
            f32x16 acc = mfma_block_p<X::KQD>(wp, ws, cur, b + 1 < nro ? cur + X::KQD * 1024 : oNro, hx, zero16());
#pragma unroll
            for (int s = 0; s < 16; ++s) r[s] = acc[s] + bb[s];
            store16(A.ahid + (size_t)L.v * A.d.KNH + D + A.layer * A.d.cnp + b * 32 + half * 16, r);
        }
    }
}

template <int D>
__device__ __forceinline__ void node_ab_body(const KArgs& A, int item) {
    if (D != 256 && !A.flags[FLAG_UNIFORM_T]) return;
    using X = Dim<D>;
    const int lane = threadIdx.x & 63, j = lane & 31, half = lane >> 5;
    const int strip = item >> 1, piece = item & 1;
    const LaneNode L = lane_node(A, strip, j);
    const bool rot = rot_active(A);
    const float* qsc = mod_row(A, L.b) + A.mod_base + X::M_EQUI + D;
    const TRow src = trow(piece == 0 ? A.wrow : A.wcol, X::ND, L.v, half);
    float x[X::HD];
    float sum = 0.f;
    if (rot) {
#pragma unroll
        for (int b = 0; b < X::ND; ++b) {
            float t[16];
            load16T(src, b, t);
#pragma unroll
            for (int s = 0; s < 16; ++s) x[b * 16 + s] = t[s];
        }
    } else {
#pragma unroll
        for (int b = 0; b < X::ND; ++b) {
            float t[16], g[16];
            load16T(src, b, t);
            load16(qsc + b * 32 + half * 16, g);
#pragma unroll
            for (int s = 0; s < 16; ++s) { sum += t[s]; x[b * 16 + s] = t[s] * (1.f + g[s]); }
        }
    }
    if (!rot) {
        const float red = pair_sum(sum);
        if (half == 0) A.rmean[(size_t)L.v * 2 + piece] = red * (1.f / D);
    }
    const float* wbase = rot ? A.ffold + (size_t)A.layer * D * D : A.W;
    const WSrc ws = make_wsrc(wbase, lane);
    const unsigned o0 = rot ? 0u : (unsigned)(A.wb[JB_C0_W] * 4);
    WPipe<X::PG> wp;
    wpipe_prime(wp, ws, o0);
    float* dst = piece == 0 ? A.ua : A.ub;
#pragma unroll 1
    for (int b = 0; b < X::ND; ++b) {
        const unsigned cur = o0 + (unsigned)b * X::KQD * 1024;
        f32x16 acc = mfma_block_p<X::KQD>(wp, ws, cur, b + 1 < X::ND ? cur + X::KQD * 1024 : o0, x, zero16());
        float r[16];
#pragma unroll
        for (int s = 0; s < 16; ++s) r[s] = acc[s];
        store16T(dst, X::ND, L.v, half, b, r);
    }
}
template <int D>
__global__ __launch_bounds__(64, 1) void k_node_ab(KArgs A) { node_ab_body<D>(A, A.ab0 + (int)blockIdx.x); }

template <int D>
__device__ __forceinline__ void node_gram_body(const KArgs& A, int tile) {
    if (!rot_active(A)) return;
    using X = Dim<D>;
    const int lane = threadIdx.x & 63, j = lane & 31, half = lane >> 5;
    const int sa = A.pd.gt_sa[tile], sc = A.pd.gt_sc[tile];
    const float4* ra = reinterpret_cast<const float4*>(A.wrow) + (size_t)sa * X::ND * 256 + lane;
    const float4* cc = reinterpret_cast<const float4*>(A.wcol) + (size_t)sc * X::ND * 256 + lane;
    const int vc = sc * 32 + j, val = sa * 32 + j;
    const int nc = A.pd.node_n[vc], noffc = A.pd.node_noff[vc], ic = A.pd.node_i[vc];
    const bool centre = A.rot != 2;
    const int refa = (centre && A.pd.node_n[val] > 0) ? A.pd.node_noff[val] : val, refc = (centre && nc > 0) ? noffc : vc;
    const float4* ma = reinterpret_cast<const float4*>(A.wcol) + (size_t)(refa >> 5) * X::ND * 256 + (refa & 31) + 32 * half;
    const float4* mc = reinterpret_cast<const float4*>(A.wcol) + (size_t)(refc >> 5) * X::ND * 256 + (refc & 31) + 32 * half;
    const float sgn = centre ? 1.f : 0.f;
    f32x16 acc = zero16();
    float na[4] = {0.f, 0.f, 0.f, 0.f}, nc4[4] = {0.f, 0.f, 0.f, 0.f};
#pragma unroll
    for (int b = 2 * X::NE; b < X::ND; ++b)
#pragma unroll
        for (int q = 0; q < 4; ++q) {
            const float4 a0 = ra[(b * 4 + q) * 64], c0 = cc[(b * 4 + q) * 64], pa = ma[(b * 4 + q) * 64], pc = mc[(b * 4 + q) * 64];
            const float4 a = make_float4(fmaf(sgn, pa.x, a0.x), fmaf(sgn, pa.y, a0.y), fmaf(sgn, pa.z, a0.z), fmaf(sgn, pa.w, a0.w));
            const float4 c = make_float4(fmaf(-sgn, pc.x, c0.x), fmaf(-sgn, pc.y, c0.y), fmaf(-sgn, pc.z, c0.z), fmaf(-sgn, pc.w, c0.w));
            acc = __builtin_amdgcn_mfma_f32_32x32x2f32(a.x, c.x, acc, 0, 0, 0);
            acc = __builtin_amdgcn_mfma_f32_32x32x2f32(a.y, c.y, acc, 0, 0, 0);
            acc = __builtin_amdgcn_mfma_f32_32x32x2f32(a.z, c.z, acc, 0, 0, 0);
            acc = __builtin_amdgcn_mfma_f32_32x32x2f32(a.w, c.w, acc, 0, 0, 0);
            na[0] = fmaf(a.x, a.x, na[0]); na[1] = fmaf(a.y, a.y, na[1]); na[2] = fmaf(a.z, a.z, na[2]); na[3] = fmaf(a.w, a.w, na[3]);
            nc4[0] = fmaf(c.x, c.x, nc4[0]); nc4[1] = fmaf(c.y, c.y, nc4[1]); nc4[2] = fmaf(c.z, c.z, nc4[2]); nc4[3] = fmaf(c.w, c.w, nc4[3]);
        }
    const float nR = pair_sum((na[0] + na[1]) + (na[2] + na[3]));
    const float nC = pair_sum((nc4[0] + nc4[1]) + (nc4[2] + nc4[3]));
    const size_t eoffc = (size_t)A.pd.node_eoff[vc];
#pragma unroll
    for (int s = 0; s < 16; ++s) {
        const int m = 8 * (s >> 2) + 4 * half + (s & 3), va = sa * 32 + m;
        const float nRa = __shfl(nR, m);
        if (nc > 0 && A.pd.node_n[va] > 0 && A.pd.node_noff[va] == noffc)
            A.gramE[eoffc + (size_t)A.pd.node_i[va] * nc + ic] = nRa + nC + 2.f * acc[s];
    }
}
template <int D>
__global__ __launch_bounds__(64) void k_node_gram(KArgs A) { node_gram_body<D>(A, A.g0 + (int)blockIdx.x); }

template <int D, int KQI>
__global__ __launch_bounds__(64) void k_fold_coord(KArgs A, FoldOffs F, float* out, int need_rot, unsigned short* out_s = nullptr) {
    if (!A.flags[FLAG_UNIFORM_T] || (need_rot && !rot_active(A))) return;
    using X = Dim<D>;
    constexpr int PER_L = X::ND * KQI;
    const int l = blockIdx.x / PER_L, r = blockIdx.x % PER_L, nb = r / KQI, q = r % KQI;
    const int lane = threadIdx.x & 63, i = lane & 31, kh = lane >> 5;
    const float* sc = A.mods + 32 + (size_t)l * A.d.MB + X::M_EQUI + D;
    const float4* c0 = reinterpret_cast<const float4*>(A.W + F.c0[l]) + (size_t)nb * X::KQD * 64;
    const float4* ine = reinterpret_cast<const float4*>(A.W + F.ine[l]);
    double a0 = 0., a1 = 0., a2 = 0., a3 = 0.;
#pragma unroll 2
    for (int qj = 0; qj < X::KQD; ++qj) {
#pragma unroll
        for (int khj = 0; khj < 2; ++khj) {
            const float4 w = c0[qj * 64 + i + 32 * khj];
            const float wv[4] = {w.x, w.y, w.z, w.w};
#pragma unroll
            for (int cj = 0; cj < 4; ++cj) {
                const int m = 4 * qj + cj, j = (m >> 4) * 32 + khj * 16 + (m & 15);
                const int s_ = j & 15, h_ = (j >> 4) & 1, ij = (s_ & 3) + 4 * h_ + 8 * (s_ >> 2);
                const float4 v = ine[((size_t)(j >> 5) * KQI + q) * 64 + ij + 32 * kh];
                const double f = (double)wv[cj] * (1.0 + (double)sc[j]);
                a0 += f * v.x; a1 += f * v.y; a2 += f * v.z; a3 += f * v.w;
            }
        }
    }
    const float m4[4] = {(float)a0, (float)a1, (float)a2, (float)a3};
    reinterpret_cast<float4*>(out)[((size_t)l * PER_L + r) * 64 + lane] = make_float4(m4[0], m4[1], m4[2], m4[3]);
    if (out_s) {
        unsigned short t[3][4];
#pragma unroll
        for (int c = 0; c < 4; ++c) {
            const __bf16 h = (__bf16)m4[c];
            const float r1 = m4[c] - (float)h;
            const __bf16 m = (__bf16)r1;
            const __bf16 lo = (__bf16)(r1 - (float)m);
            t[0][c] = __builtin_bit_cast(unsigned short, h); t[1][c] = __builtin_bit_cast(unsigned short, m); t[2][c] = __builtin_bit_cast(unsigned short, lo);
        }
        constexpr int NS = KQI / 2;
        const size_t stepbase = (((size_t)l * X::ND + nb) * NS + (q >> 1)) * 3;
#pragma unroll
        for (int term = 0; term < 3; ++term) {
            unsigned short* dst = out_s + ((stepbase + term) * 64 + lane) * 8 + 4 * (q & 1);
            *reinterpret_cast<uint2*>(dst) = make_uint2((unsigned)t[term][0] | ((unsigned)t[term][1] << 16), (unsigned)t[term][2] | ((unsigned)t[term][3] << 16));
        }
    }
}

template <int D, int R>
__global__ __launch_bounds__(64, 1) void k_edge_update(KArgs A) {
    if (!A.flags[FLAG_ASYM]) return;
    using X = Dim<D>;
    constexpr int NCH = R * X::De / 64;
    constexpr int KQ4 = R * X::De / 8;
    const int lane = threadIdx.x & 63, j = lane & 31, half = lane >> 5;
    const int it = blockIdx.x;
    const int strip = A.pd.item_strip[it], t0 = A.pd.item_t0[it], t1 = A.pd.item_t1[it], part = A.pd.item_part[it];
    const LaneNode L = lane_node(A, strip, j);
    const float* mrow = mod_row(A, L.b) + A.mod_base;
    const float* eg1 = mrow + X::M_EDGE + 2 * X::De;
    const float* qsh = mrow + X::M_EQUI;
    const float gscale = mrow[X::M_GBF + 0], gshift = mrow[X::M_GBF + 1];
    const float4 pv = reinterpret_cast<const float4*>(A.pos_out)[L.v];
    const float cscale = A.W[A.wb[JB_CSCALE]];
    const WSrc ws = make_wsrc(A.W, lane);
    const unsigned o3 = (unsigned)(A.wb[JB_FF3_W] * 4), o4 = (unsigned)(A.wb[JB_FF4_W] * 4);
    const unsigned oro = (unsigned)(A.wb[JB_ERO_W] * 4), oi = (unsigned)(A.wb[JB_INE_W] * 4), o0 = (unsigned)(A.wb[JB_C0_W] * 4);
    WPipe<X::PG> wp;
    wpipe_prime(wp, ws, o3);
    float dax = 0.f, day = 0.f, daz = 0.f;
    for (int t = t0; t < t1; ++t) {
        const bool inr = L.valid && t < L.n;
        const bool ok = inr && t != L.i;
        const int tc = inr ? t : 0;
        const int u = L.noff + tc;
        const size_t r = (size_t)L.eoff + (size_t)L.i * L.n + tc;
        const float* eg1_ = launder(eg1);
        const float* es2_ = eg1_ + X::De, *ec2_ = es2_ + X::De, *eg2_ = ec2_ + X::De;
        const float* qsh_ = launder(qsh);
        const float* qsc_ = qsh_ + D;
        const float* cst = launder(A.W);
        const float* n2bias_ = cst + A.wb[JB_N2E_B], *b3_ = cst + A.wb[JB_FF3_B], *b4_ = cst + A.wb[JB_FF4_B];
        const float* b0_ = cst + A.wb[JB_C0_B], *w2_ = cst + A.wb[JB_C2_W], *tab_ = cst + A.wb[JB_GBF];
        const float* bro_ = cst + A.wb[JB_ERO_B];
        TRow wrow = trow(A.wrow, X::ND, L.v, half);
        wrow.p = launder(wrow.p);
        const TRow wcol = trow(A.wcol, X::ND, u, half);
        const float4 pu = reinterpret_cast<const float4*>(A.pos_out)[u];
        const float dx = pv.x - pu.x, dy = pv.y - pu.y, dz = pv.z - pu.z;
        const float d2 = dx * dx + dy * dy + dz * dz;
        float G[X::HE];
        gbf_n<X::NE>(d2, gscale, gshift, tab_, half, G);
        float en[X::HE];
        {
            const TRow ra = trow(A.n2e, X::NE, L.v, half), rc = trow(A.n2e, X::NE, u, half);
#pragma unroll
            for (int b = 0; b < X::NE; ++b) {
                float e[16], ta[16], tc2[16], g[16], bb[16];
                load16(A.e + r * X::De + b * 32 + half * 16, e);
                load16T(ra, b, ta);
                load16T(rc, b, tc2);
                load16(eg1_ + b * 32 + half * 16, g);
                load16(n2bias_ + b * 32 + half * 16, bb);
#pragma unroll
                for (int s = 0; s < 16; ++s) en[b * 16 + s] = fmaf(g[s], ta[s] + tc2[s] + bb[s], e[s]);
            }
        }
        layer_norm<X::HE>(en);
        modulate<X::NE>(en, es2_, ec2_, half);
        {
            f32x16 o[X::NE];
#pragma unroll
            for (int b = 0; b < X::NE; ++b) o[b] = zero16();
#pragma unroll
            for (int c = 0; c < NCH; ++c) {
                float hid[32];
#pragma unroll
                for (int b2 = 0; b2 < 2; ++b2) {
                    const unsigned wcur = o3 + (unsigned)(c * 2 + b2) * X::KQE * 1024;
                    const unsigned wnx = b2 == 0 ? wcur + X::KQE * 1024 : o4 + (unsigned)(c * 8) * 1024;
                    float bb[16];
                    load16(b3_ + (c * 2 + b2) * 32 + half * 16, bb);
                    f32x16 acc = mfma_block_p<X::KQE>(wp, ws, wcur, wnx, en, zero16());
                    silu_bias16(acc, bb, hid + b2 * 16);
                }
#pragma unroll
                for (int ob = 0; ob < X::NE; ++ob) {
                    const unsigned wcur = o4 + (unsigned)(ob * KQ4 + c * 8) * 1024;
                    const unsigned wnx = ob + 1 < X::NE ? o4 + (unsigned)((ob + 1) * KQ4 + c * 8) * 1024
                                                        : (c + 1 < NCH ? o3 + (unsigned)((c + 1) * 2) * X::KQE * 1024 : oro);
                    o[ob] = mfma_block_p<8>(wp, ws, wcur, wnx, hid, o[ob]);
                }
            }
#pragma unroll
            for (int b = 0; b < X::NE; ++b) {
                float ob4[16], og2[16];
                load16(b4_ + b * 32 + half * 16, ob4);
                load16(eg2_ + b * 32 + half * 16, og2);
#pragma unroll
                for (int s = 0; s < 16; ++s) en[b * 16 + s] = fmaf(og2[s], o[b][s] + ob4[s], en[b * 16 + s]);
            }
        }
        if (inr) store_nat<X::NE>(A.e_out + r * X::De, half, en);
        {
            float bb[16];
            load16(bro_ + half * 16, bb);
            f32x16 acc = mfma_block_p<X::KQE>(wp, ws, oro, oi, en, zero16());
            float rr[16];
#pragma unroll
            for (int s = 0; s < 16; ++s) rr[s] = acc[s] + bb[s];
            if (inr && (half == 0 || A.d.cep == 32)) store16(A.ehid + r * A.d.KEH + X::De + A.layer * A.d.cep + half * 16, rr);
        }
        float uu[X::HD];
#pragma unroll
        for (int b = 0; b < X::ND; ++b) {
            const unsigned we = oi + (unsigned)(b * 2 * X::KQE) * 1024, wg_ = we + X::KQE * 1024;
            float a1[16], a2[16];
            load16T(wrow, b, a1);
            load16T(wcol, b, a2);
            f32x16 acc = mfma_block_p<X::KQE>(wp, ws, we, wg_, en, zero16());
            acc = mfma_block_p<X::KQE>(wp, ws, wg_, b + 1 < X::ND ? wg_ + X::KQE * 1024 : o0, G, acc);
#pragma unroll
            for (int s = 0; s < 16; ++s) uu[b * 16 + s] = acc[s] + a1[s] + a2[s];
        }
        layer_norm<X::HD>(uu);
        modulate<X::ND>(uu, qsh_, qsc_, half);
        float c0 = 0.f, c1 = 0.f, c2 = 0.f;
#pragma unroll 1
        for (int b = 0; b < X::ND; ++b) {
            const unsigned wcur = o0 + (unsigned)b * X::KQD * 1024;
            const unsigned wnx = b + 1 < X::ND ? wcur + X::KQD * 1024 : o3;
            float bb[16], k0[16], k1[16], k2[16];
            load16(b0_ + b * 32 + half * 16, bb);
            load16(w2_ + b * 32 + half * 16, k0);
            load16(w2_ + D + b * 32 + half * 16, k1);
            load16(w2_ + 2 * D + b * 32 + half * 16, k2);
            f32x16 acc = mfma_block_p<X::KQD>(wp, ws, wcur, wnx, uu, zero16());
#pragma unroll
            for (int s = 0; s < 16; ++s) {
                const float ys = silu_f(acc[s] + bb[s]);
                c0 = fmaf(ys, k0[s], c0);
                c1 = fmaf(ys, k1[s], c1);
                c2 = fmaf(ys, k2[s], c2);
            }
        }
        c0 = tanh_f(pair_sum(c0));
        c1 = tanh_f(pair_sum(c1));
        c2 = tanh_f(pair_sum(c2));
        const int fl = A.eflag[r];
        const float iota = (c0 + ((fl & 1) ? c1 : 0.f) + ((fl & 2) ? c2 : 0.f)) * (1.f / 3.f);
        const float nrm = fmaxf(sqrtf(d2), 1e-8f);
        const float f = ok ? cscale * iota / nrm : 0.f;
        dax = fmaf(dx, f, dax);
        day = fmaf(dy, f, day);
        daz = fmaf(dz, f, daz);
    }
    if (half == 0)
        reinterpret_cast<float4*>(A.dpos)[(size_t)L.v * A.pd.max_parts + part] = make_float4(dax, day, daz, 0.f);
}

template <int D, int R, bool FOLD = false, bool ROT = false, int ZW = 1>
__global__ __launch_bounds__(ZW * 64, 1) void k_edge_update_sym(KArgs A) {
    static_assert(FOLD || !ROT, "the rotated statistics need the shared modulation row");
    static_assert(ZW == 1 || D == 256 || FOLD, "the Z split needs the hoisted form (one coord_mlp.0 per pair)");
    if (A.flags[FLAG_ASYM]) return;
    if ((A.flags[FLAG_UNIFORM_T] != 0) != FOLD) return;
    using X = Dim<D>;
    constexpr int NCH = R * X::De / 64;
    constexpr int KQ4 = R * X::De / 8;
    const int lane = threadIdx.x & 63, jl = lane & 31, half = lane >> 5;
    const int zw = ZW > 1 ? (int)(threadIdx.x >> 6) : 0;
    const int zb0 = zw * (X::ND / ZW), zb1 = zb0 + X::ND / ZW;
    static_assert(X::ND % ZW == 0, "Z blocks per wave");
    const int it = A.item0 + (A.dir_split ? (int)(blockIdx.x >> 1) : (int)blockIdx.x);
    const int dsel = A.dir_split ? (int)(blockIdx.x & 1) : -1;
    const int strip = A.pd.pitem_strip[it], t0 = A.pd.pitem_t0[it], t1 = A.pd.pitem_t1[it];
    const LaneNode L = lane_node(A, strip, jl);
    const float* mrow = mod_row(A, L.b) + A.mod_base;
    const float* eg1 = mrow + X::M_EDGE + 2 * X::De;
    const float* qsh = mrow + X::M_EQUI;
    const float gscale = mrow[X::M_GBF + 0], gshift = mrow[X::M_GBF + 1];
    const float4 pv = reinterpret_cast<const float4*>(A.pos_out)[L.v];
    const float cscale = A.W[A.wb[JB_CSCALE]];
    const WSrc ws = make_wsrc(A.W, lane);
    const unsigned o3 = (unsigned)(A.wb[JB_FF3_W] * 4), o4 = (unsigned)(A.wb[JB_FF4_W] * 4);
    const unsigned oro = (unsigned)(A.wb[JB_ERO_W] * 4), oi = (unsigned)(A.wb[JB_INE_W] * 4), o0 = (unsigned)(A.wb[JB_C0_W] * 4);
    WPipe<X::PG> wp;
    wpipe_prime(wp, ws, o3);
    constexpr bool HOIST = D == 256 || FOLD;
    constexpr int PLB = D > 256 ? X::ND / 2 : 0;
    __shared__ float4 pl[PLB > 0 ? PLB * 4 * 64 : 1];
    __shared__ float4 w2s[HOIST ? 3 * D / 4 : 1];
    __shared__ float zred[ZW > 1 ? (ZW - 1) * 12 * 64 : 1];
    if constexpr (HOIST) {
        const float4* src = reinterpret_cast<const float4*>(A.W + A.wb[JB_C2_W]);
        for (int i = threadIdx.x; i < 3 * D / 4; i += ZW * 64) w2s[i] = src[i];
        __syncthreads();
    }
    float park[HOIST ? 1 : (X::ND - PLB) * 16];
    PT_INIT
    for (int t = t0; t < t1; ++t) {
        const PairLane P = pair_of(L, t + 1);
        const float* eg1_ = launder(eg1);
        const float* es2_ = eg1_ + X::De, *ec2_ = es2_ + X::De, *eg2_ = ec2_ + X::De;
        const float* qsh_ = launder(qsh);
        const float* qsc_ = qsh_ + D;
        const float* cst = launder(A.W);
        const float* n2bias_ = cst + A.wb[JB_N2E_B], *b3_ = cst + A.wb[JB_FF3_B], *b4_ = cst + A.wb[JB_FF4_B];
        const float* b0_ = cst + A.wb[JB_C0_B], *w2_ = cst + A.wb[JB_C2_W], *tab_ = cst + A.wb[JB_GBF];
        const float* bro_ = cst + A.wb[JB_ERO_B];
        const BRow wrow_i = brow(A.wrow, X::ND, L.v, half), wcol_i = brow(A.wcol, X::ND, L.v, half);
        const BRow wrow_j = brow(A.wrow, X::ND, P.u, half), wcol_j = brow(A.wcol, X::ND, P.u, half);
        const float4 pu = reinterpret_cast<const float4*>(A.pos_out)[P.u];
        const float dx = pv.x - pu.x, dy = pv.y - pu.y, dz = pv.z - pu.z;
        const float d2 = dx * dx + dy * dy + dz * dz;
        float G[X::HE];
        gbf_n<X::NE>(d2, gscale, gshift, tab_, half, G);
        float en[X::HE];
        {
            const TRow ra = trow(A.n2e, X::NE, L.v, half), rc = trow(A.n2e, X::NE, P.u, half);
#pragma unroll
            for (int b = 0; b < X::NE; ++b) {
                float e[16], ta[16], tc2[16], g[16], bb[16];
                load16(A.e + P.rij * X::De + b * 32 + half * 16, e);
                load16T(ra, b, ta);
                load16T(rc, b, tc2);
                load16(eg1_ + b * 32 + half * 16, g);
                load16(n2bias_ + b * 32 + half * 16, bb);
#pragma unroll
                for (int s = 0; s < 16; ++s) en[b * 16 + s] = fmaf(g[s], ta[s] + tc2[s] + bb[s], e[s]);
            }
        }
        layer_norm<X::HE>(en);
        modulate<X::NE>(en, es2_, ec2_, half);
        PT(0);
        {
            f32x16 o[X::NE];
#pragma unroll
            for (int b = 0; b < X::NE; ++b) o[b] = zero16();
#pragma unroll
            for (int c = 0; c < NCH; ++c) {
                float hid[32];
#pragma unroll
                for (int b2 = 0; b2 < 2; ++b2) {
                    const unsigned wcur = o3 + (unsigned)(c * 2 + b2) * X::KQE * 1024;
                    const unsigned wnx = b2 == 0 ? wcur + X::KQE * 1024 : o4 + (unsigned)(c * 8) * 1024;
                    float bb[16];
                    load16(b3_ + (c * 2 + b2) * 32 + half * 16, bb);
                    f32x16 acc = mfma_block_p<X::KQE>(wp, ws, wcur, wnx, en, zero16());
                    silu_bias16(acc, bb, hid + b2 * 16);
                }
#pragma unroll
                for (int ob = 0; ob < X::NE; ++ob) {
                    const unsigned wcur = o4 + (unsigned)(ob * KQ4 + c * 8) * 1024;
                    const unsigned wnx = ob + 1 < X::NE ? o4 + (unsigned)((ob + 1) * KQ4 + c * 8) * 1024
                                                        : (c + 1 < NCH ? o3 + (unsigned)((c + 1) * 2) * X::KQE * 1024 : oro);
                    o[ob] = mfma_block_p<8>(wp, ws, wcur, wnx, hid, o[ob]);
                }
            }
#pragma unroll
            for (int b = 0; b < X::NE; ++b) {
                float ob4[16], og2[16];
                load16(b4_ + b * 32 + half * 16, ob4);
                load16(eg2_ + b * 32 + half * 16, og2);
#pragma unroll
                for (int s = 0; s < 16; ++s) en[b * 16 + s] = fmaf(og2[s], o[b][s] + ob4[s], en[b * 16 + s]);
            }
        }
        if (P.ok && dsel != 1 && zw == 0) {
            store_nat<X::NE>(A.e_out + P.rij * X::De, half, en);
            if (!A.half_rows || L.n > PAIR_GROUP_LANES) store_nat<X::NE>(A.e_out + P.rji * X::De, half, en);
        }
        PT(1);
        unsigned opq = 0;
        asm volatile("" : "+v"(opq));
        BRow ua_i = brow(A.ua, X::ND, L.v, half), ub_i = brow(A.ub, X::ND, L.v, half);
        const BRow ua_j = brow(A.ua, X::ND, P.u, half), ub_j = brow(A.ub, X::ND, P.u, half);
        BRow own_r = wrow_i, own_c = wcol_i;
        ua_i.voff += opq; ub_i.voff += opq; own_r.voff += opq; own_c.voff += opq;
        float n0[16], n1[16], n2[16], n3[16];
        constexpr int NB2 = 2 * X::NE;
        constexpr int KQL = 2 * X::KQE;
        const unsigned oL = (unsigned)(A.wb[JB_LQ_W] * 4);
        float gr0 = 0.f, gr1 = 0.f;
        if constexpr (ROT) {
            bload16(own_r, NB2 - 1, n0); bload16(wcol_j, NB2 - 1, n1); bload16(wrow_j, NB2 - 1, n2); bload16(own_c, NB2 - 1, n3);
            gr0 = A.gramE[P.rij]; gr1 = A.gramE[P.rji];
        }
        {
            float bb[16];
            load16(bro_ + half * 16, bb);
            f32x16 acc;
            if constexpr (ROT) acc = mfma_block_g<X::KQE, (4 < X::PG ? 4 : X::PG)>(wp, ws, oro, ws, oL + (unsigned)((NB2 - 1) * KQL + 4 * (NB2 - 1)) * 1024, en, zero16());
            else acc = mfma_block_p<X::KQE>(wp, ws, oro, oi, en, zero16());
            float rr[16];
#pragma unroll
            for (int s = 0; s < 16; ++s) rr[s] = acc[s] + bb[s];
            if (P.ok && dsel != 1 && zw == 0 && (half == 0 || A.d.cep == 32)) {
                store16(A.ehid + P.rij * A.d.KEH + X::De + A.layer * A.d.cep + half * 16, rr);
                if (!A.half_rows || L.n > PAIR_GROUP_LANES) store16(A.ehid + P.rji * A.d.KEH + X::De + A.layer * A.d.cep + half * 16, rr);
            }
        }
        PT(2);
        if constexpr (HOIST) {
            float sg[FOLD ? 1 : X::HD];
            const WSrc wm = make_wsrc(A.mfold + (size_t)A.layer * D * 2 * X::De, lane);
            f32x2 q02 = {0.f, 0.f}, q12 = {0.f, 0.f};
            float rstd0, rstd1, mr0 = 0.f, mr1 = 0.f;
            if constexpr (ROT) {
                float z[2 * X::HE];
#pragma unroll
                for (int s = 0; s < X::HE; ++s) { z[s] = en[s]; z[X::HE + s] = G[s]; }
                static_for<NB2>([&](auto kc) {
                    constexpr int k = decltype(kc)::value, b = NB2 - 1 - k;
                    constexpr int KQ = 4 * (NB2 - b), KQN = 4 * (NB2 - b + 1);
                    constexpr int NXT = (k + 1 < NB2 && KQN < X::PG) ? KQN : X::PG;
                    float t0[16], t1[16];
#pragma unroll
                    for (int s = 0; s < 16; s += 2) {
                        const f32x2 a = pk2(n0[s], n0[s + 1]) + pk2(n1[s], n1[s + 1]), c = pk2(n2[s], n2[s + 1]) + pk2(n3[s], n3[s + 1]);
                        t0[s] = a.x; t0[s + 1] = a.y; t1[s] = c.x; t1[s + 1] = c.y;
                    }
                    auto next_rows = [&]() {
                        if constexpr (k + 1 < NB2) { bload16(own_r, b - 1, n0); bload16(wcol_j, b - 1, n1); bload16(wrow_j, b - 1, n2); bload16(own_c, b - 1, n3); }
                        else { bload16(ua_i, zb0, n0); bload16(ub_j, zb0, n1); bload16(ua_j, zb0, n2); bload16(ub_i, zb0, n3); }
                    };
                    const unsigned cur = oL + (unsigned)(b * KQL + 4 * b) * 1024;
                    f32x16 acc;
                    if constexpr (k + 1 < NB2) acc = mfma_block_g<KQ, NXT>(wp, ws, cur, ws, oL + (unsigned)((b - 1) * KQL + 4 * (b - 1)) * 1024, z + 16 * b, zero16(), next_rows);
                    else acc = mfma_block_g<KQ, NXT>(wp, ws, cur, wm, (unsigned)zb0 * 2 * X::KQE * 1024, z + 16 * b, zero16(), next_rows);
                    PT(3);
#pragma unroll
                    for (int s = 0; s < 16; s += 2) {
                        const f32x2 sv = pk2(acc[s], acc[s + 1]);
                        const f32x2 d0 = sv + pk2(t0[s], t0[s + 1]), d1 = sv + pk2(t1[s], t1[s + 1]);
                        q02 = __builtin_elementwise_fma(d0, d0, q02);
                        q12 = __builtin_elementwise_fma(d1, d1, q12);
                    }
                    PT(4);
                });
                rstd0 = __builtin_amdgcn_rsqf(fmaxf((pair_sum(q02.x + q02.y) + gr0) * (1.f / D), 0.f) + 1e-6f);
                rstd1 = __builtin_amdgcn_rsqf(fmaxf((pair_sum(q12.x + q12.y) + gr1) * (1.f / D), 0.f) + 1e-6f);
            } else {
            const float m00 = A.rmean[(size_t)L.v * 2] + A.rmean[(size_t)P.u * 2 + 1];
            const float m01 = A.rmean[(size_t)P.u * 2] + A.rmean[(size_t)L.v * 2 + 1];
            f32x2 ssum2 = {0.f, 0.f};
            bload16(own_r, 0, n0); bload16(wcol_j, 0, n1); bload16(wrow_j, 0, n2); bload16(own_c, 0, n3);
#pragma unroll
            for (int b = 0; b < X::ND; ++b) {
                const unsigned we = oi + (unsigned)(b * 2 * X::KQE) * 1024, wg_ = we + X::KQE * 1024;
                float g[16], t0[16], t1[16];
                if constexpr (!FOLD) load16(qsc_ + b * 32 + half * 16, g);
#pragma unroll
                for (int s = 0; s < 16; s += 2) {
                    const f32x2 a = (pk2(n0[s], n0[s + 1]) + pk2(n1[s], n1[s + 1])) - m00, c = (pk2(n2[s], n2[s + 1]) + pk2(n3[s], n3[s + 1])) - m01;
                    t0[s] = a.x; t0[s + 1] = a.y; t1[s] = c.x; t1[s + 1] = c.y;
                }
                auto next_rows = [&]() {
                    if (b + 1 < X::ND) { bload16(own_r, b + 1, n0); bload16(wcol_j, b + 1, n1); bload16(wrow_j, b + 1, n2); bload16(own_c, b + 1, n3); }
                    else { bload16(ua_i, zb0, n0); bload16(ub_j, zb0, n1); bload16(ua_j, zb0, n2); bload16(ub_i, zb0, n3); }
                };
                f32x16 acc = mfma_block_p<X::KQE>(wp, ws, we, wg_, en, zero16());
                if (FOLD && b + 1 == X::ND) acc = mfma_block_p2<X::KQE>(wp, ws, wg_, wm, (unsigned)zb0 * 2 * X::KQE * 1024, G, acc, next_rows);
                else acc = mfma_block_p2<X::KQE>(wp, ws, wg_, ws, b + 1 < X::ND ? wg_ + X::KQE * 1024 : o0 + (unsigned)zb0 * X::KQD * 1024, G, acc, next_rows);
                PT(3);
#pragma unroll
                for (int s = 0; s < 16; s += 2) {
                    const f32x2 sv = pk2(acc[s], acc[s + 1]);
                    ssum2 = ssum2 + sv;
                    if constexpr (!FOLD) { const f32x2 m = sv * (pk2(g[s], g[s + 1]) + 1.f); sg[b * 16 + s] = m.x; sg[b * 16 + s + 1] = m.y; }
                    const f32x2 d0 = sv + pk2(t0[s], t0[s + 1]), d1 = sv + pk2(t1[s], t1[s + 1]);
                    q02 = __builtin_elementwise_fma(d0, d0, q02);
                    q12 = __builtin_elementwise_fma(d1, d1, q12);
                }
                PT(4);
            }
            const float meanS = pair_sum(ssum2.x + ssum2.y) * (1.f / D);
            rstd0 = __builtin_amdgcn_rsqf(fmaxf(pair_sum(q02.x + q02.y) * (1.f / D) - meanS * meanS, 0.f) + 1e-6f);
            rstd1 = __builtin_amdgcn_rsqf(fmaxf(pair_sum(q12.x + q12.y) * (1.f / D) - meanS * meanS, 0.f) + 1e-6f);
            mr0 = (meanS + m00) * rstd0; mr1 = (meanS + m01) * rstd1;
            }
            PT(4);
            const float* wg_v = launder(mrow + X::M_WG);
            const float* bs_v = wg_v + D;
            f32x2 c00 = {0.f, 0.f}, c01 = c00, c02 = c00, c10 = c00, c11 = c00, c12 = c00;
#pragma unroll 1
            for (int b = zb0; b < zb1; ++b) {
                float t0[16], t1[16], wgb[16], bsb[16];
#pragma unroll
                for (int s = 0; s < 16; s += 2) {
                    const f32x2 a = pk2(n0[s], n0[s + 1]) + pk2(n1[s], n1[s + 1]), c = pk2(n2[s], n2[s + 1]) + pk2(n3[s], n3[s + 1]);
                    t0[s] = a.x; t0[s + 1] = a.y; t1[s] = c.x; t1[s + 1] = c.y;
                }
                auto next_rows = [&]() {
                    const int bn = b + 1 < zb1 ? b + 1 : b;
                    bload16(ua_i, bn, n0); bload16(ub_j, bn, n1); bload16(ua_j, bn, n2); bload16(ub_i, bn, n3);
                };
                if constexpr (!ROT) load16(wg_v + b * 32 + half * 16, wgb);
                load16(bs_v + b * 32 + half * 16, bsb);
                f32x16 z;
                if constexpr (FOLD) {
                    const unsigned mcur = (unsigned)b * 2 * X::KQE * 1024;
                    WSrc wn = wm;
                    unsigned noff = mcur + 2 * X::KQE * 1024;
                    if (b + 1 == zb1) { wn = ws; noff = o3; }
                    z = mfma_block_p<X::KQE>(wp, wm, mcur, mcur + X::KQE * 1024, en, zero16());
                    z = mfma_block_p2<X::KQE>(wp, wm, mcur + X::KQE * 1024, wn, noff, G, z, next_rows);
                } else {
                    const unsigned wcur = o0 + (unsigned)b * X::KQD * 1024;
                    z = mfma_block_p2<X::KQD>(wp, ws, wcur, ws, b + 1 < zb1 ? wcur + X::KQD * 1024 : o3, sg, zero16(), next_rows);
                }
                PT(5);
#pragma unroll
                for (int hq = 0; hq < 2; ++hq) {
                    float k0[8], k1[8], k2[8], ca[8];
                    auto ld8 = [&](const float* p8, float (&r)[8]) {
                        const float4 a = reinterpret_cast<const float4*>(p8)[0], c = reinterpret_cast<const float4*>(p8)[1];
                        r[0] = a.x; r[1] = a.y; r[2] = a.z; r[3] = a.w; r[4] = c.x; r[5] = c.y; r[6] = c.z; r[7] = c.w;
                    };
                    const int fo = b * 32 + half * 16 + hq * 8;
                    const float* w2l = reinterpret_cast<const float*>(w2s);
                    ld8(w2l + fo, k0); ld8(w2l + D + fo, k1); ld8(w2l + 2 * D + fo, k2);
#pragma unroll
                    for (int s = 0; s < 8; s += 2) {
                        const f32x2 bs2 = pk2(bsb[hq * 8 + s], bsb[hq * 8 + s + 1]);
                        f32x2 c = bs2;
                        if constexpr (!ROT) c = __builtin_elementwise_fma((f32x2)(-mr0), pk2(wgb[hq * 8 + s], wgb[hq * 8 + s + 1]), bs2);
                        ca[s] = c.x; ca[s + 1] = c.y;
                    }
                    pipeline_fence();
#pragma unroll
                    for (int s = 0; s < 8; s += 2) {
                        const f32x2 pre = pk2(z[hq * 8 + s], z[hq * 8 + s + 1]) + pk2(t0[hq * 8 + s], t0[hq * 8 + s + 1]);
                        const f32x2 ys0 = silu_f2(__builtin_elementwise_fma(pre, (f32x2)(rstd0), pk2(ca[s], ca[s + 1])));
                        c00 = __builtin_elementwise_fma(ys0, pk2(k0[s], k0[s + 1]), c00);
                        c01 = __builtin_elementwise_fma(ys0, pk2(k1[s], k1[s + 1]), c01);
                        c02 = __builtin_elementwise_fma(ys0, pk2(k2[s], k2[s + 1]), c02);
                    }
                    pipeline_fence();
#pragma unroll
                    for (int s = 0; s < 8; s += 2) {
                        const f32x2 bs2 = pk2(bsb[hq * 8 + s], bsb[hq * 8 + s + 1]);
                        f32x2 c = bs2;
                        if constexpr (!ROT) c = __builtin_elementwise_fma((f32x2)(-mr1), pk2(wgb[hq * 8 + s], wgb[hq * 8 + s + 1]), bs2);
                        ca[s] = c.x; ca[s + 1] = c.y;
                    }
#pragma unroll
                    for (int s = 0; s < 8; s += 2) {
                        const f32x2 pre = pk2(z[hq * 8 + s], z[hq * 8 + s + 1]) + pk2(t1[hq * 8 + s], t1[hq * 8 + s + 1]);
                        const f32x2 ys1 = silu_f2(__builtin_elementwise_fma(pre, (f32x2)(rstd1), pk2(ca[s], ca[s + 1])));
                        c10 = __builtin_elementwise_fma(ys1, pk2(k0[s], k0[s + 1]), c10);
                        c11 = __builtin_elementwise_fma(ys1, pk2(k1[s], k1[s + 1]), c11);
                        c12 = __builtin_elementwise_fma(ys1, pk2(k2[s], k2[s + 1]), c12);
                    }
                    pipeline_fence();
                }
                PT(7);
            }
            PT(7);
            if constexpr (ZW > 1) {
                float* zr = zred + lane;
                if (zw > 0) {
                    float* o = zr + (zw - 1) * 12 * 64;
                    o[0 * 64] = c00.x; o[1 * 64] = c00.y; o[2 * 64] = c01.x; o[3 * 64] = c01.y; o[4 * 64] = c02.x; o[5 * 64] = c02.y;
                    o[6 * 64] = c10.x; o[7 * 64] = c10.y; o[8 * 64] = c11.x; o[9 * 64] = c11.y; o[10 * 64] = c12.x; o[11 * 64] = c12.y;
                }
                __syncthreads();
                if (zw == 0) {
#pragma unroll
                    for (int w = 1; w < ZW; ++w) {
                        const float* o = zr + (w - 1) * 12 * 64;
                        c00.x += o[0 * 64]; c00.y += o[1 * 64]; c01.x += o[2 * 64]; c01.y += o[3 * 64]; c02.x += o[4 * 64]; c02.y += o[5 * 64];
                        c10.x += o[6 * 64]; c10.y += o[7 * 64]; c11.x += o[8 * 64]; c11.y += o[9 * 64]; c12.x += o[10 * 64]; c12.y += o[11 * 64];
                    }
                }
                if (t + 1 < t1) __syncthreads();
            }
            const float nrm = fmaxf(sqrtf(d2), 1e-8f);
#pragma unroll
            for (int dir = 0; dir < 2; ++dir) {
                const float c0 = tanh_f(pair_sum(dir == 0 ? c00.x + c00.y : c10.x + c10.y));
                const float c1 = tanh_f(pair_sum(dir == 0 ? c01.x + c01.y : c11.x + c11.y));
                const float c2 = tanh_f(pair_sum(dir == 0 ? c02.x + c02.y : c12.x + c12.y));
                const size_t rr = dir == 0 ? P.rij : P.rji;
                const int fl = A.eflag[rr];
                const float iota = (c0 + ((fl & 1) ? c1 : 0.f) + ((fl & 2) ? c2 : 0.f)) * (1.f / 3.f);
                const float f = cscale * iota / nrm;
                const float sgn = dir == 0 ? 1.f : -1.f;
                if (P.ok && half == 0 && zw == 0)
                    reinterpret_cast<float4*>(A.dposE)[rr] = make_float4(sgn * dx * f, sgn * dy * f, sgn * dz * f, 0.f);
            }
            PT(6);
        } else {
    #pragma unroll
            for (int b = 0; b < X::ND; ++b) {
                const unsigned we = oi + (unsigned)(b * 2 * X::KQE) * 1024, wg_ = we + X::KQE * 1024;
                f32x16 acc = mfma_block_p<X::KQE>(wp, ws, we, wg_, en, zero16());
                acc = mfma_block_p<X::KQE>(wp, ws, wg_, b + 1 < X::ND ? wg_ + X::KQE * 1024 : o0, G, acc);
    #pragma unroll
                for (int s = 0; s < 16; ++s) {
                    if (b < X::ND - PLB) park[(b < X::ND - PLB ? b : 0) * 16 + s] = acc[s];
                }
                if (b >= X::ND - PLB) {
    #pragma unroll
                    for (int q = 0; q < 4; ++q)
                        pl[((b - (X::ND - PLB)) * 4 + q) * 64 + lane] = make_float4(acc[q * 4 + 0], acc[q * 4 + 1], acc[q * 4 + 2], acc[q * 4 + 3]);
                }
            }
            PT(3);
    #pragma unroll 1
            for (int dir = 0; dir < 2; ++dir) {
                if (dsel >= 0 && dir != dsel) continue;
                BRow ra = wrow_i, rc = wcol_j;
                if (dir == 1) { ra.voff = wrow_j.voff; rc.voff = wcol_i.voff; }
                float uu[X::HD];
                constexpr int GB = D == 256 ? 4 : 2;
    #pragma unroll
                for (int g = 0; g < X::ND / GB; ++g) {
                    float a1[GB * 16], a2[GB * 16];
    #pragma unroll
                    for (int k = 0; k < GB; ++k) {
                        float t1[16], t2[16];
                        bload16(ra, g * GB + k, t1);
                        bload16(rc, g * GB + k, t2);
    #pragma unroll
                        for (int s = 0; s < 16; ++s) { a1[k * 16 + s] = t1[s]; a2[k * 16 + s] = t2[s]; }
                    }
                    pipeline_fence();
    #pragma unroll
                    for (int k = 0; k < GB; ++k) {
                        const int b = g * GB + k;
                        float pk[16];
                        if (b < X::ND - PLB) {
    #pragma unroll
                            for (int s = 0; s < 16; ++s) pk[s] = park[(b < X::ND - PLB ? b : 0) * 16 + s];
                        } else {
    #pragma unroll
                            for (int q = 0; q < 4; ++q) {
                                const float4 t = pl[((b - (X::ND - PLB)) * 4 + q) * 64 + lane];
                                pk[q * 4 + 0] = t.x; pk[q * 4 + 1] = t.y; pk[q * 4 + 2] = t.z; pk[q * 4 + 3] = t.w;
                            }
                        }
    #pragma unroll
                        for (int s = 0; s < 16; ++s) uu[b * 16 + s] = pk[s] + (a1[k * 16 + s] + a2[k * 16 + s]);
                    }
                }
                PT(6);
                layer_norm<X::HD>(uu);
                modulate<X::ND>(uu, qsh_, qsc_, half);
                PT(4);
                float c0 = 0.f, c1 = 0.f, c2 = 0.f;
    #pragma unroll 1
                for (int b = 0; b < X::ND; ++b) {
                    const unsigned wcur = o0 + (unsigned)b * X::KQD * 1024;
                    const unsigned wnx = b + 1 < X::ND ? wcur + X::KQD * 1024 : ((dir == 0 && dsel < 0) ? o0 : o3);
                    float bb[16], k0[16], k1[16], k2[16];
                    load16(b0_ + b * 32 + half * 16, bb);
                    load16(w2_ + b * 32 + half * 16, k0);
                    load16(w2_ + D + b * 32 + half * 16, k1);
                    load16(w2_ + 2 * D + b * 32 + half * 16, k2);
                    f32x16 acc = mfma_block_p<X::KQD>(wp, ws, wcur, wnx, uu, zero16());
    #pragma unroll
                    for (int s = 0; s < 16; ++s) {
                        const float ys = silu_f(acc[s] + bb[s]);
                        c0 = fmaf(ys, k0[s], c0);
                        c1 = fmaf(ys, k1[s], c1);
                        c2 = fmaf(ys, k2[s], c2);
                    }
                }
                PT(dir == 0 ? 5 : 7);
                c0 = tanh_f(pair_sum(c0));
                c1 = tanh_f(pair_sum(c1));
                c2 = tanh_f(pair_sum(c2));
                const size_t rr = dir == 0 ? P.rij : P.rji;
                const int fl = A.eflag[rr];
                const float iota = (c0 + ((fl & 1) ? c1 : 0.f) + ((fl & 2) ? c2 : 0.f)) * (1.f / 3.f);
                const float nrm = fmaxf(sqrtf(d2), 1e-8f);
                const float f = cscale * iota / nrm;
                const float sgn = dir == 0 ? 1.f : -1.f;
                if (P.ok && half == 0)
                    reinterpret_cast<float4*>(A.dposE)[rr] = make_float4(sgn * dx * f, sgn * dy * f, sgn * dz * f, 0.f);
                PT(6);
            }
        }
    }
    PT_FLUSH;
}

template <int D>
__device__ __forceinline__ void node_head_body(const KArgs& A, int strip) {
    using X = Dim<D>;
    const int lane = threadIdx.x & 63, j = lane & 31, half = lane >> 5;
    const int v = strip * 32 + j;
    const int KNH = A.d.KNH;
    const WSrc ws = make_wsrc(A.W, lane);
    const unsigned o1 = (unsigned)(A.wg[JW_NH1_W] * 4), o2 = (unsigned)(A.wg[JW_NH2_W] * 4), o3 = (unsigned)(A.wg[JW_NH3_W] * 4);
    WPipe<4> wp;
    wpipe_prime(wp, ws, o1);
    f32x16 o[X::ND];
#pragma unroll
    for (int b = 0; b < X::ND; ++b) o[b] = zero16();
    {
        const int kq = KNH / 8, nch = KNH / 64;
#pragma unroll 1
        for (int c = 0; c < nch; ++c) {
            float x[32];
            load_nat<2>(A.ahid + (size_t)v * KNH + c * 64, half, x);
#pragma unroll
            for (int ob = 0; ob < X::ND; ++ob) {
                const unsigned cur = o1 + (unsigned)(ob * kq + c * 8) * 1024;
                const unsigned nxt = ob + 1 < X::ND ? o1 + (unsigned)((ob + 1) * kq + c * 8) * 1024
                                                    : (c + 1 < nch ? o1 + (unsigned)((c + 1) * 8) * 1024 : o2);
                o[ob] = mfma_block_p<8>(wp, ws, cur, nxt, x, o[ob]);
            }
        }
    }
    float a1[X::HD];
    {
        const float* bias = A.W + A.wg[JW_NH1_B];
#pragma unroll
        for (int b = 0; b < X::ND; ++b) {
            float r[16];
            acc_bias(o[b], bias + b * 32 + half * 16, r);
#pragma unroll
            for (int s = 0; s < 16; ++s) a1[b * 16 + s] = silu_f(r[s]);
        }
    }
    float a2[X::HD / 2];
    {
        const float* bias = A.W + A.wg[JW_NH2_B];
#pragma unroll
        for (int b = 0; b < X::ND / 2; ++b) {
            const unsigned cur = o2 + (unsigned)(b * X::KQD) * 1024;
            f32x16 acc = mfma_block_p<X::KQD>(wp, ws, cur, b + 1 < X::ND / 2 ? cur + X::KQD * 1024 : o3, a1, zero16());
            float r[16];
            acc_bias(acc, bias + b * 32 + half * 16, r);
#pragma unroll
            for (int s = 0; s < 16; ++s) a2[b * 16 + s] = silu_f(r[s]);
        }
    }
    {
        f32x16 acc = mfma_block_p<X::KQD / 2>(wp, ws, o3, o3, a2, zero16());
        float r[16];
        acc_bias(acc, A.W + A.wg[JW_NH3_B] + half * 16, r);
        store16(A.apred + (size_t)v * 32 + half * 16, r);
    }
}
template <int D>
__global__ __launch_bounds__(64, 1) void k_node_head(KArgs A) { node_head_body<D>(A, (int)blockIdx.x); }

template <int D, int NBK, bool SYM>
__device__ __forceinline__ void edge_head_body(const KArgs& A, int blk) {
    if ((A.flags[FLAG_ASYM] != 0) == SYM) return;
    using X = Dim<D>;
    const int lane = threadIdx.x & 63, j = lane & 31, half = lane >> 5;
    const int ur = SYM ? A.pd.ut_rows[((size_t)blk * 32 + j) * 2] : 0, um = SYM ? A.pd.ut_rows[((size_t)blk * 32 + j) * 2 + 1] : 0;
    const size_t r = SYM ? (size_t)(ur < 0 ? 0 : ur) : (size_t)blk * 32 + j;
    const WSrc ws = make_wsrc(A.W, lane);
    const unsigned o1 = (unsigned)(A.wg[JW_EH1_W] * 4), o2 = (unsigned)(A.wg[JW_EH2_W] * 4), o3 = (unsigned)(A.wg[JW_EH3_W] * 4);
    WPipe<4> wp;
    wpipe_prime(wp, ws, o1);
    float x[NBK * 16];
    load_nat<NBK>(A.ehid + r * (NBK * 32), half, x);
    float a1[X::De];
    {
        const float* bias = A.W + A.wg[JW_EH1_B];
#pragma unroll
        for (int b = 0; b < 2 * X::NE; ++b) {
            const unsigned cur = o1 + (unsigned)(b * NBK * 4) * 1024;
            f32x16 acc = mfma_block_p<NBK * 4>(wp, ws, cur, b + 1 < 2 * X::NE ? cur + (unsigned)(NBK * 4) * 1024 : o2, x, zero16());
            float rr[16];
            acc_bias(acc, bias + b * 32 + half * 16, rr);
#pragma unroll
            for (int s = 0; s < 16; ++s) a1[b * 16 + s] = silu_f(rr[s]);
        }
    }
    float a2[X::De / 2];
    {
        const float* bias = A.W + A.wg[JW_EH2_B];
#pragma unroll
        for (int b = 0; b < X::NE; ++b) {
            const unsigned cur = o2 + (unsigned)(b * (X::De / 4)) * 1024;
            f32x16 acc = mfma_block_p<X::De / 4>(wp, ws, cur, b + 1 < X::NE ? cur + (unsigned)(X::De / 4) * 1024 : o3, a1, zero16());
            float rr[16];
            acc_bias(acc, bias + b * 32 + half * 16, rr);
#pragma unroll
            for (int s = 0; s < 16; ++s) a2[b * 16 + s] = silu_f(rr[s]);
        }
    }
    {
        f32x16 acc = mfma_block_p<X::De / 8>(wp, ws, o3, o3, a2, zero16());
        float rr[16];
        acc_bias(acc, A.W + A.wg[JW_EH3_B] + half * 16, rr);
        if (SYM) {
            if (half == 0 && ur >= 0) {
                reinterpret_cast<float4*>(A.epred)[ur] = make_float4(rr[0], rr[1], rr[2], rr[3]);
                reinterpret_cast<float4*>(A.epred)[um] = make_float4(rr[0], rr[1], rr[2], rr[3]);
            }
        } else if (half == 0 && r < (size_t)A.pd.rows) {
            reinterpret_cast<float4*>(A.epred)[r] = make_float4(rr[0], rr[1], rr[2], rr[3]);
        }
    }
}
template <int D, int NBK, bool SYM>
__global__ __launch_bounds__(64, 1) void k_edge_head(KArgs A) { edge_head_body<D, NBK, SYM>(A, (int)blockIdx.x); }

template <int D, int NBK>
__global__ __launch_bounds__(64, 1) void k_heads_sym(KArgs A) {
    const int ns = A.pd.n_strips;
    if ((int)blockIdx.x < ns) node_head_body<D>(A, (int)blockIdx.x);
    else edge_head_body<D, NBK, true>(A, (int)blockIdx.x - ns);
}

}
}
```

jodo_amd/csrc/dgt_plan.cpp:

```cpp
#include <algorithm>
#include <numeric>
#include <utility>
#include <new>
#include "dgt_plan.h"
#include "jodo_hip_internal.h"

static size_t align_up(size_t x, size_t a) { return (x + a - 1) / a * a; }

static std::vector<int> xcd_order(const std::vector<int32_t>& strip, int group) {
    const int n = (int)strip.size();
    std::vector<std::vector<int>> q(8);
    for (int i = 0; i < n; ++i) q[strip[i] & 7].push_back(i);
    size_t pos[8] = {0, 0, 0, 0, 0, 0, 0, 0};
    std::vector<int> out;
    out.reserve(n);
    int wg = 0;
    while ((int)out.size() < n) {
        int c = wg & 7, tries = 0;
        while (pos[c] >= q[c].size() && tries < 8) { c = (c + 1) & 7; ++tries; }
        for (int k = 0; k < group && pos[c] < q[c].size(); ++k) out.push_back(q[c][pos[c]++]);
        ++wg;
    }
    return out;
}

static void permute(std::vector<int32_t>& a, const std::vector<int>& ord) {
    std::vector<int32_t> b(a.size());
    for (size_t i = 0; i < ord.size(); ++i) b[i] = a[ord[i]];
    a.swap(b);
}

int dgt_dims_from_cfg(const jodo_cfg* c, DgtDims* d) {
    if (c->nf != 128 && c->nf != 256 && c->nf != 384)
        return jodo_set_error(JODO_ERR_UNSUPPORTED, "nf=%d: kernels are built for nf=128, nf=256 and nf=384", c->nf);
    if (c->layout != 0 && c->layout != 1) return jodo_set_error(JODO_ERR_ARG, "layout=%d (0 or 1)", c->layout);
    if (c->n_heads != 16 || c->n_extra != 2)
        return jodo_set_error(JODO_ERR_UNSUPPORTED, "n_heads=%d n_extra_heads=%d: kernels are built for 16/2", c->n_heads, c->n_extra);
    if (c->mlp_ratio != 2 && c->mlp_ratio != 4)
        return jodo_set_error(JODO_ERR_UNSUPPORTED, "mlp_ratio=%d: supported 2, 4", c->mlp_ratio);
    if (c->n_layers < 1 || c->n_layers > 32) return jodo_set_error(JODO_ERR_ARG, "n_layers=%d", c->n_layers);
    if (c->in_node_dim < 1 || 2 * c->in_node_dim > 64) return jodo_set_error(JODO_ERR_ARG, "in_node_dim=%d", c->in_node_dim);
    if (c->edge_ch < 1 || c->edge_ch > 4) return jodo_set_error(JODO_ERR_ARG, "edge_ch=%d (1..4)", c->edge_ch);
    if (c->cond_ch < 0 || c->cond_ch > 8) return jodo_set_error(JODO_ERR_ARG, "cond_ch=%d", c->cond_ch);
    d->D = c->nf; d->De = c->nf / 4; d->T = c->nf * 4; d->L = c->n_layers; d->H = c->n_heads; d->XH = c->n_extra;
    d->SH = d->H - d->XH; d->C = d->D / d->H; d->SC = (d->H * d->C) / d->SH; d->r = c->mlp_ratio;
    d->nd = c->in_node_dim; d->ch = c->edge_ch; d->cond_ch = c->cond_ch;
    const int cn = (2 * d->D) / d->L, ce = (2 * d->De) / d->L;
    d->cnp = std::max(d->D / 4, (cn + 31) / 32 * 32);
    d->cep = std::max((d->D / 16 + 15) / 16 * 16, (ce + 15) / 16 * 16);
    if (d->cep > 32) return jodo_set_error(JODO_ERR_UNSUPPORTED, "n_layers=%d at nf=%d: edge readout width %d beyond one 32-row block", d->L, d->D, ce);
    d->wide = (c->nf != 256 || c->layout == 1 || d->cnp != 64) ? 1 : 0;
    int tail = d->SC - 16;
    d->QKP = d->wide ? d->SH * 32 : (d->SH / 2 + (tail + 1) / 2) * 32;
    d->ndp = (2 * d->nd + 7) / 8 * 8;
    d->einp = (2 * d->ch + 7) / 8 * 8;
    d->KNH = d->D + d->L * d->cnp; d->KEH = d->De + d->L * d->cep;
    if (d->KEH % 32 != 0) return jodo_set_error(JODO_ERR_UNSUPPORTED, "edge head width %d not a multiple of 32", d->KEH);
    d->MB = 6 * d->D + 6 * d->De + 2 * d->D + 32 + 2 * d->D;
    d->Mtot = 32 + (int64_t)d->L * d->MB;
    d->cutoff = c->spatial_cut_off; d->edge_th = c->edge_quan_th;
    return JODO_OK;
}

extern "C" int jodo_plan_create(const jodo_cfg* cfg, int B, int N, const int32_t* n_nodes, int max_chunk,
                                jodo_plan** out) {
    if (!cfg || !n_nodes || !out || B <= 0 || N <= 0) return jodo_set_error(JODO_ERR_ARG, "plan_create: bad argument");
    jodo_plan* p = new (std::nothrow) jodo_plan();
    if (!p) return jodo_set_error(JODO_ERR_ARG, "plan_create: out of host memory");
    p->cfg = *cfg;
    int rc = dgt_dims_from_cfg(cfg, &p->dims);
    if (rc != JODO_OK) { delete p; return rc; }
    for (int b = 0; b < B; ++b)
        if (n_nodes[b] < 1 || n_nodes[b] > N) {
            delete p;
            return jodo_set_error(JODO_ERR_ARG, "plan_create: n_nodes[%d]=%d outside [1,%d]", b, n_nodes[b], N);
        }
    int pair_chunk = (max_chunk >> 16) & 0xff, spair_chunk = (max_chunk >> 24) & 0xff;
    max_chunk &= 0xffff;
    if (max_chunk <= 0) {
        int64_t strip_nmax_sum = 0;
        {
            std::vector<int> sorted(n_nodes, n_nodes + B);
            std::sort(sorted.begin(), sorted.end(), [](int a, int b) { return a > b; });
            int64_t v = 0;
            int strip = -1;
            for (int m = 0; m < B; ++m) {
                const int first = (int)(v / 32), last = (int)((v + sorted[m] - 1) / 32);
                for (int s = std::max(first, strip + 1); s <= last; ++s) strip_nmax_sum += sorted[m];
                strip = std::max(strip, last);
                v += sorted[m];
            }
        }
        max_chunk = 8;
        while (max_chunk > 2 && strip_nmax_sum / max_chunk < 2048) --max_chunk;
    }
    if (pair_chunk <= 0) pair_chunk = 1;
    const bool spair_auto = spair_chunk <= 0;
    p->B = B; p->N = N; p->max_blocks = -1; p->last_pos_buf = 0; p->last_e_buf = 0;
    p->opt[JODO_OPT_FUSE_NEXT_QKV] = 1; p->opt[JODO_OPT_DIR_SPLIT] = 1; p->opt[JODO_OPT_NODE_POST_WAVES] = 0; p->opt[JODO_OPT_ATTN_VARIANT] = 0; p->opt[JODO_OPT_HEADS_MIX] = 1; p->opt[JODO_OPT_HALF_ROWS] = 1; p->opt[JODO_OPT_PRE_EMBED] = 1; p->opt[JODO_OPT_AB_PRE] = 1; p->opt[JODO_OPT_Z_SPLIT] = 1;
    p->opt[JODO_OPT_PIN_SYMMETRIC] = 0; p->opt[JODO_OPT_PIN_UNIFORM_T] = 0; p->opt[JODO_OPT_ROT_STATS] = 1; p->opt[JODO_OPT_NODE_MIX] = 1;
    p->opt[JODO_OPT_SPLIT_BF16] = 0; p->split_w = nullptr; p->split_bytes = 0;
    p->prof_enabled = 0; p->force_directed = 0; p->dbg_timing = nullptr;

    std::vector<int> order(B);
    std::iota(order.begin(), order.end(), 0);
    std::stable_sort(order.begin(), order.end(), [&](int a, int b) { return n_nodes[a] > n_nodes[b]; });

    int64_t Nn = 0, rows = 0, dir = 0;
    for (int b = 0; b < B; ++b) { Nn += n_nodes[b]; rows += (int64_t)n_nodes[b] * n_nodes[b]; dir += (int64_t)n_nodes[b] * (n_nodes[b] - 1); }
    if (rows >= (int64_t)1 << 31) { delete p; return jodo_set_error(JODO_ERR_UNSUPPORTED, "batch too large: %lld dense edge rows", (long long)rows); }
    p->Nn = (int)Nn; p->Nn_pad = (int)align_up((size_t)Nn, 32); p->n_strips = p->Nn_pad / 32;
    p->rows = rows; p->dir_edges = dir;

    std::vector<int32_t> node_b(p->Nn_pad, 0), node_i(p->Nn_pad, 0), node_n(p->Nn_pad, 0), node_noff(p->Nn_pad, 0),
        node_eoff(p->Nn_pad, 0), orig_n(B), orig_noff(B), orig_eoff(B);
    int v = 0; int64_t eoff = 0;
    for (int m = 0; m < B; ++m) {
        int b = order[m], n = n_nodes[b];
        orig_n[b] = n; orig_noff[b] = v; orig_eoff[b] = (int32_t)eoff;
        for (int i = 0; i < n; ++i) {
            node_b[v + i] = b; node_i[v + i] = i; node_n[v + i] = n; node_noff[v + i] = v; node_eoff[v + i] = (int32_t)eoff;
        }
        v += n; eoff += (int64_t)n * n;
    }
    std::vector<int32_t> it_strip, it_t0, it_t1, it_part, strip_parts(p->n_strips, 0);
    int max_parts = 1;
    for (int s = 0; s < p->n_strips; ++s) {
        int nmax = 0;
        for (int j = 0; j < 32; ++j) nmax = std::max(nmax, (int)node_n[s * 32 + j]);
        if (nmax == 0) continue;
        int parts = (nmax + max_chunk - 1) / max_chunk;
        int chunk = (nmax + parts - 1) / parts;
        parts = (nmax + chunk - 1) / chunk;
        max_parts = std::max(max_parts, parts);
        strip_parts[s] = parts;
        for (int q = 0; q < parts; ++q) {
            it_strip.push_back(s); it_t0.push_back(q * chunk); it_t1.push_back(std::min(nmax, (q + 1) * chunk)); it_part.push_back(q);
        }
    }
    p->n_items = (int)it_strip.size(); p->max_parts = max_parts;
    {
        const std::vector<int> ord = xcd_order(it_strip, 4);
        permute(it_strip, ord); permute(it_t0, ord); permute(it_t1, ord); permute(it_part, ord);
    }
    std::vector<int32_t> pi_strip, pi_t0, pi_t1;
    for (int s = 0; s < p->n_strips; ++s) {
        int nmax = 0;
        for (int j = 0; j < 32; ++j) nmax = std::max(nmax, (int)node_n[s * 32 + j]);
        const int dmax = nmax / 2;
        if (dmax == 0) continue;
        int parts = (dmax + pair_chunk - 1) / pair_chunk;
        int chunk = (dmax + parts - 1) / parts;
        parts = (dmax + chunk - 1) / chunk;
        for (int q = 0; q < parts; ++q) { pi_strip.push_back(s); pi_t0.push_back(q * chunk); pi_t1.push_back(std::min(dmax, (q + 1) * chunk)); }
    }
    p->n_pitems = (int)pi_strip.size();
    p->pitems_single = 1;
    for (size_t i = 0; i < pi_strip.size(); ++i) if (pi_t1[i] - pi_t0[i] != 1) p->pitems_single = 0;
    {
        const std::vector<int> ord = xcd_order(pi_strip, 1);
        permute(pi_strip, ord); permute(pi_t0, ord); permute(pi_t1, ord);
    }
    std::vector<int32_t> ag_node, ai_group, ai_t0, ai_t1, ai_part, ai_dir, ad_group, ad_t0, ad_t1, ad_part, ad_big, anode_parts(p->Nn_pad, 0), aw_off;
    int amax_parts = 1;
    {
        constexpr int G = 128;
        const bool persist = spair_auto;
        int achunk = (spair_auto || spair_chunk == 255) ? 0 : spair_chunk;
        std::vector<int> mol_n(B), mol_noff(B);
        for (int m = 0; m < B; ++m) { mol_n[m] = n_nodes[order[m]]; mol_noff[m] = orig_noff[order[m]]; }
        std::vector<char> used(B, 0);
        std::vector<int> g_nmax, g_big;
        int head = 0;
        while (head < B) {
            if (used[head]) { ++head; continue; }
            if (mol_n[head] > G) {
                for (int o = 0; o < mol_n[head]; o += G) {
                    for (int k = 0; k < G; ++k) ag_node.push_back(o + k < mol_n[head] ? mol_noff[head] + o + k : -1);
                    g_nmax.push_back(mol_n[head]); g_big.push_back(1);
                }
                used[head++] = 1;
                continue;
            }
            int fill = 0, nmax = mol_n[head];
            std::vector<int32_t> lanes;
            for (int m = head; m < B && fill < G; ++m) {
                if (used[m] || mol_n[m] > G - fill) continue;
                for (int k = 0; k < mol_n[m]; ++k) lanes.push_back(mol_noff[m] + k);
                fill += mol_n[m]; used[m] = 1;
            }
            lanes.resize(G, -1);
            ag_node.insert(ag_node.end(), lanes.begin(), lanes.end());
            g_nmax.push_back(nmax); g_big.push_back(0);
        }
        const int ng = (int)g_nmax.size();
        p->n_agroups = ng;
        if (persist) achunk = 6;
        if (achunk <= 0 && p->dims.wide) {
            int64_t iters = 0;
            for (int g = 0; g < ng; ++g) iters += std::max(1, g_nmax[g] / 2);
            achunk = 6;
            while (achunk > 1 && iters / achunk < 2 * 256) --achunk;
        }
        if (achunk <= 0) {
            std::vector<double> slot(256);
            double best = 0.0;
            for (int c = 1; c <= 16; ++c) {
                std::vector<int> len;
                for (int g = 0; g < ng; ++g) {
                    if (g_big[g]) { len.push_back(g_nmax[g]); continue; }
                    const int dmax = g_nmax[g] / 2, parts = std::max(1, (dmax + c - 1) / c), cp = dmax > 0 ? (dmax + parts - 1) / parts : 0;
                    for (int q = 0; q < parts; ++q) len.push_back(std::min(dmax, (q + 1) * cp) - std::min(dmax, q * cp));
                }
                std::stable_sort(len.begin(), len.end(), [](int a, int b) { return a > b; });
                std::fill(slot.begin(), slot.end(), 0.0);
                for (int l : len) { auto it = std::min_element(slot.begin(), slot.end()); *it += 0.8 + (double)l; }
                const double mk = *std::max_element(slot.begin(), slot.end());
                if (achunk <= 0 || mk <= best) { best = mk; achunk = c; }
            }
        }
        struct It { int g, t0, t1, part, big; };
        std::vector<It> pit, dit;
        std::vector<int> g_parts(ng, 1), pit_dir;
        if (persist) {
            const double a_item = 0.3;
            const double w_dir = 0.9;
            auto g_len = [&](int g) { return g_big[g] ? g_nmax[g] : g_nmax[g] / 2; };
            auto g_wgt = [&](int g) { return g_big[g] ? w_dir : 1.0; };
            double total = 0.0;
            for (int g = 0; g < ng; ++g) total += a_item + g_wgt(g) * (double)g_len(g);
            double T = std::max(total / JODO_ATT_SLOTS, a_item + 1.0);
            aw_off.assign(JODO_ATT_SLOTS + 1, 0);
            for (int attempt = 0; attempt < 400; ++attempt, T *= 1.004) {
                pit.clear();
                int slot = 0;
                double load = 0.0;
                auto next_slot = [&]() { if (slot + 1 < JODO_ATT_SLOTS) { ++slot; load = 0.0; } };
                for (int g = 0; g < ng; ++g) {
                    const int len = g_len(g);
                    const double wg = g_wgt(g);
                    int t = 0, part = 0;
                    do {
                        double room = T - load - a_item;
                        if (room < 0.75 && load > 0.0 && slot + 1 < JODO_ATT_SLOTS) { next_slot(); room = T - a_item; }
                        int take = std::min(len - t, std::max(1, (int)(room / wg + 0.5)));
                        take = std::max(take, 0);
                        pit.push_back({g, t, t + take, part++, slot});
                        load += a_item + wg * (double)take;
                        t += take;
                        if (load >= T - 0.5) next_slot();
                    } while (t < len);
                    g_parts[g] = part;
                }
                if (load <= T + 0.5) break;
            }
            for (const It& it : pit) aw_off[it.big + 1]++;
            for (int sl = 0; sl < JODO_ATT_SLOTS; ++sl) aw_off[sl + 1] += aw_off[sl];
            for (It& it : pit) { it.big = 0; pit_dir.push_back(g_big[it.g]); }
        }
        for (int g = 0; g < ng; ++g) {
            const int nmax = g_nmax[g], dmax = nmax / 2;
            int parts;
            if (persist) parts = g_parts[g];
            else if (g_big[g]) parts = std::max(1, (nmax + 2 * achunk - 1) / (2 * achunk));
            else parts = std::max(1, (dmax + achunk - 1) / achunk);
            amax_parts = std::max(amax_parts, parts);
            const int cp = dmax > 0 ? (dmax + parts - 1) / parts : 0, cd = (nmax + parts - 1) / parts;
            for (int q = 0; q < parts; ++q) {
                if (!g_big[g] && !persist) pit.push_back({g, std::min(dmax, q * cp), std::min(dmax, (q + 1) * cp), q, 0});
                dit.push_back({g, std::min(nmax, q * cd), std::min(nmax, (q + 1) * cd), q, (g_big[g] && !persist) ? 1 : 0});
            }
            for (int k = 0; k < G; ++k) { const int v = ag_node[(size_t)g * G + k]; if (v >= 0) anode_parts[v] = parts; }
        }
        auto lpt = [](const It& a, const It& b) { return (a.t1 - a.t0) > (b.t1 - b.t0); };
        if (!persist) std::stable_sort(pit.begin(), pit.end(), lpt);
        std::stable_sort(dit.begin(), dit.end(), lpt);
        for (const It& it : pit) { ai_group.push_back(it.g); ai_t0.push_back(it.t0); ai_t1.push_back(it.t1); ai_part.push_back(it.part); }
        ai_dir.assign(pit.size(), 0);
        for (size_t i = 0; i < pit_dir.size(); ++i) ai_dir[i] = pit_dir[i];
        p->n_ai_dir = 0;
        for (size_t i = 0; i < ai_dir.size(); ++i) p->n_ai_dir += ai_dir[i] ? 1 : 0;
        for (const It& it : dit) { ad_group.push_back(it.g); ad_t0.push_back(it.t0); ad_t1.push_back(it.t1); ad_part.push_back(it.part); ad_big.push_back(it.big); }
        p->n_aitems = (int)pit.size(); p->n_aditems = (int)dit.size(); p->amax_parts = amax_parts;
        p->a_persist = persist ? 1 : 0;
        if (!persist) aw_off.assign(1, 0);
        p->has_big = 0;
        for (int g = 0; g < ng; ++g) p->has_big |= (g_big[g] && !persist) ? 1 : 0;
    }

    auto put = [&](const std::vector<int32_t>& a, size_t* off) {
        *off = p->desc.size();
        p->desc.insert(p->desc.end(), a.begin(), a.end());
        while (p->desc.size() % 64) p->desc.push_back(0);
    };
    put(node_b, &p->off_node_b); put(node_i, &p->off_node_i); put(node_n, &p->off_node_n);
    put(node_noff, &p->off_node_noff); put(node_eoff, &p->off_node_eoff);
    put(orig_n, &p->off_orig_n); put(orig_noff, &p->off_orig_noff); put(orig_eoff, &p->off_orig_eoff);
    put(it_strip, &p->off_item_strip); put(it_t0, &p->off_item_t0); put(it_t1, &p->off_item_t1); put(it_part, &p->off_item_part); put(strip_parts, &p->off_strip_parts);
    put(pi_strip, &p->off_pitem_strip); put(pi_t0, &p->off_pitem_t0); put(pi_t1, &p->off_pitem_t1);
    put(ag_node, &p->off_ag_node); put(ai_group, &p->off_ai_group); put(ai_t0, &p->off_ai_t0); put(ai_t1, &p->off_ai_t1); put(ai_part, &p->off_ai_part); put(ai_dir, &p->off_ai_dir);
    put(ad_group, &p->off_ad_group); put(ad_t0, &p->off_ad_t0); put(ad_t1, &p->off_ad_t1); put(ad_part, &p->off_ad_part); put(ad_big, &p->off_ad_big);
    put(anode_parts, &p->off_anode_parts); put(aw_off, &p->off_aw_off);
    {
        std::vector<int32_t> ut;
        for (int b = 0; b < B; ++b) {
            const int n = orig_n[b];
            const int64_t e0 = orig_eoff[b];
            for (int i = 0; i < n; ++i)
                for (int d = 1; 2 * d <= n; ++d) {
                    if (2 * d == n && 2 * i >= n) continue;
                    const int j = (i + d) % n;
                    ut.push_back((int32_t)(e0 + (int64_t)i * n + j)); ut.push_back((int32_t)(e0 + (int64_t)j * n + i));
                }
        }
        while ((ut.size() / 2) % 32) { ut.push_back(-1); ut.push_back(-1); }
        p->n_ut_pad = (int)(ut.size() / 2);
        put(ut, &p->off_ut_rows);
    }
    {
        std::vector<int32_t> gsa, gsc;
        for (int s = 0; s < p->n_strips; ++s) {
            int lo = s, hi = s;
            for (int j = 0; j < 32; ++j) {
                const int v0 = s * 32 + j;
                if (node_n[v0] <= 0) continue;
                lo = std::min(lo, (int)node_noff[v0] / 32);
                hi = std::max(hi, (int)(node_noff[v0] + node_n[v0] - 1) / 32);
            }
            for (int c = lo; c <= hi; ++c) { gsa.push_back(s); gsc.push_back(c); }
        }
        {
            std::vector<int> ord(gsa.size());
            std::iota(ord.begin(), ord.end(), 0);
            std::stable_sort(ord.begin(), ord.end(), [&](int a, int b) { return std::max(gsa[a], gsc[a]) < std::max(gsa[b], gsc[b]); });
            permute(gsa, ord); permute(gsc, ord);
        }
        p->n_gtiles = (int)gsa.size(); p->gt_cache_full = -1; p->gt_cache_count = 0;
        put(gsa, &p->off_gt_sa); put(gsc, &p->off_gt_sc);
    }

    const DgtDims& d = p->dims;
    size_t o = 0;
    auto take = [&](size_t bytes) { size_t at = o; o = align_up(o + bytes, 256); return at; };
    const size_t f = sizeof(float), NP = (size_t)p->Nn_pad, R = (size_t)rows + 32, Bp = align_up((size_t)B, 32);
    WsLayout& w = p->ws;
    w.hid1 = take(Bp * d.T * f); w.temb = take(Bp * d.T * f); w.tembs = take(Bp * d.T * f); w.mods = take(Bp * (size_t)d.Mtot * f);
    w.condh = take(Bp * (size_t)std::max(1, d.cond_ch) * d.D * f); w.condh2 = take(Bp * (size_t)std::max(1, d.cond_ch) * d.D * f);
    w.pos0 = take(NP * 4 * f); w.pos1 = take(NP * 4 * f); w.dpos = take(NP * max_parts * 4 * f); w.cpos = take(NP * 4 * f);
    w.feat = take(NP * d.ndp * f); w.h = take(NP * d.D * f); w.hhat = take(NP * amax_parts * d.D * f);
    w.astat = take(NP * amax_parts * 32 * f);
    w.q = take(NP * d.QKP * f); w.k = take(NP * d.QKP * f); w.v = take(NP * d.D * f); w.n2e = take(NP * d.De * f);
    w.wrow = take(NP * d.D * f); w.wcol = take(NP * d.D * f); w.ua = take(NP * d.D * f); w.ub = take(NP * d.D * f); w.rmean = take(NP * 2 * f); w.mfold = take((size_t)d.L * d.D * 2 * d.De * f); w.mfold_s = take((size_t)d.L * d.D * 2 * d.De * 6); w.ffold_s = take((size_t)d.L * d.D * d.D * 6); w.ffold = take((size_t)d.L * d.D * d.D * f); w.ahid = take(NP * d.KNH * f);
    w.apred = take(NP * 32 * f);
    w.eflag = take(R * sizeof(int32_t)); w.e = take(R * d.De * f); w.e2 = take(R * d.De * f);
    w.ehid = take(R * d.KEH * f); w.epred = take(R * 4 * f); w.dposE = take(R * 4 * f); w.gramE = take(R * f);
    w.total = o;
    *out = p;
    return JODO_OK;
}

extern "C" void jodo_plan_destroy(jodo_plan* p) {
    if (!p) return;
    for (void* e : p->prof_ev) (void)hipEventDestroy((hipEvent_t)e);
    for (void* e : p->prof_pool) (void)hipEventDestroy((hipEvent_t)e);
    delete p;
}
extern "C" int jodo_profile_enable(jodo_plan* p, int enable) {
    if (!p) return jodo_set_error(JODO_ERR_ARG, "null plan");
    p->prof_enabled = enable;
    return JODO_OK;
}
extern "C" int jodo_profile_read(jodo_plan* p, float* ms_sum, int32_t* launches) {
    if (!p || !ms_sum || !launches) return jodo_set_error(JODO_ERR_ARG, "profile_read: null");
    for (int c = 0; c < JODO_PROF_COUNT; ++c) { ms_sum[c] = 0.f; launches[c] = 0; }
    for (size_t i = 0; i + 1 < p->prof_ev.size(); i += 2) {
        hipEvent_t a = (hipEvent_t)p->prof_ev[i], b = (hipEvent_t)p->prof_ev[i + 1];
        hipError_t e = hipEventSynchronize(b);
        float ms = 0.f;
        if (e == hipSuccess) e = hipEventElapsedTime(&ms, a, b);
        if (e != hipSuccess) return jodo_set_error(JODO_ERR_LAUNCH, "profile_read: %s", hipGetErrorString(e));
        const int c = p->prof_cls[i / 2];
        ms_sum[c] += ms; launches[c] += 1;
        p->prof_pool.push_back(p->prof_ev[i]); p->prof_pool.push_back(p->prof_ev[i + 1]);
    }
    p->prof_ev.clear(); p->prof_cls.clear();
    return JODO_OK;
}
extern "C" size_t jodo_plan_desc_bytes(const jodo_plan* p) { return p ? p->desc.size() * sizeof(int32_t) : 0; }
extern "C" size_t jodo_plan_workspace_bytes(const jodo_plan* p) { return p ? p->ws.total : 0; }
extern "C" int64_t jodo_plan_mod_len(const jodo_plan* p) { return p ? p->dims.Mtot : 0; }
extern "C" int jodo_plan_stats(const jodo_plan* p, int64_t* o) {
    if (!p || !o) return jodo_set_error(JODO_ERR_ARG, "plan_stats: null");
    o[0] = p->Nn; o[1] = p->rows; o[2] = p->dir_edges; o[3] = p->n_strips; o[4] = p->n_items; o[5] = p->max_parts;
    return JODO_OK;
}

namespace {
inline double proj(int out, int K) { return (double)((out + 31) / 32) * (double)((K + 7) / 8 * 4); }
}
extern "C" int jodo_plan_work(const jodo_plan* p, int uniform_t, int symmetric, double* mfma_flops) {
    if (!p || !mfma_flops) return jodo_set_error(JODO_ERR_ARG, "plan_work: null");
    const DgtDims& d = p->dims;
    const bool tuned = !d.wide, sym = symmetric && !p->force_directed && p->n_pitems > 0;
    const int D = d.D, De = d.De, L = d.L, r = d.r;
    const int32_t* dsc = p->desc.data();
    double cls[JODO_PROF_COUNT] = {0, 0, 0, 0, 0, 0, 0, 0};
    const double strips = p->n_strips;
    const double rowgroups = (uniform_t && d.cond_ch == 0) ? 1.0 : (double)((p->B + 31) / 32);
    cls[JODO_PROF_PROLOGUE] += rowgroups * (proj(d.T, d.T) + proj((int)d.Mtot, d.T));
    if (d.cond_ch > 0) cls[JODO_PROF_PROLOGUE] += (double)((p->B * d.cond_ch + 31) / 32) * proj(D, D) + (double)((p->B + 31) / 32) * proj(d.T, d.cond_ch * D);
    cls[JODO_PROF_PROLOGUE] += strips * proj(D, d.ndp);
    double dir_iters = 0, pair_iters = 0;
    for (int i = 0; i < p->n_items; ++i) dir_iters += dsc[p->off_item_t1 + i] - dsc[p->off_item_t0 + i];
    for (int i = 0; i < p->n_pitems; ++i) pair_iters += dsc[p->off_pitem_t1 + i] - dsc[p->off_pitem_t0 + i];
    cls[(p->opt[JODO_OPT_PRE_EMBED] != 0 && L > 0) ? JODO_PROF_NODE_PRE : JODO_PROF_PROLOGUE] += dir_iters * proj(De, d.einp + De);
    const int nqb = tuned ? 8 : d.SH;
    const double qkv = 2.0 * nqb * (D / 2) + proj(D, D);
    const bool fuse_pre = tuned && p->opt[JODO_OPT_FUSE_NEXT_QKV] != 0 && L > 1 && p->n_strips >= 1024;
    const bool ab_pre = !fuse_pre && p->opt[JODO_OPT_AB_PRE] != 0 && L > 1 && (!tuned || (p->n_strips < 1024 && p->opt[JODO_OPT_NODE_POST_WAVES] == 0));
    cls[JODO_PROF_NODE_PRE] += strips * qkv * ((fuse_pre || ab_pre) ? 1 : L);
    if (fuse_pre || ab_pre) cls[JODO_PROF_NODE_POST] += strips * qkv * (L - 1);
    cls[JODO_PROF_NODE_POST] += L * strips * (proj(De, D) + proj(r * D, D) + proj(D, r * D) + 2 * proj(D, D) + proj(d.cnp, D));
    const bool hoist = sym && (D == 256 || uniform_t);
    if (p->n_pitems > 0 && (D == 256 || uniform_t)) cls[JODO_PROF_NODE_POST] += L * strips * 2 * proj(D, D);
    const double att_iter = proj(De, 2 * De) + nqb * (double)(De / 2) + proj(D, De);
    double att_iters = 0;
    for (int i = 0; i < p->n_aitems; ++i) if (sym) att_iters += 4.0 * (dsc[p->off_ai_t1 + i] - dsc[p->off_ai_t0 + i]);
    for (int i = 0; i < p->n_aditems; ++i)
        if (!sym || dsc[p->off_ad_big + i]) att_iters += 4.0 * (dsc[p->off_ad_t1 + i] - dsc[p->off_ad_t0 + i]);
    cls[JODO_PROF_EDGE_ATTN] += L * att_iters * att_iter;
    const double trunk = proj(r * De, De) + proj(De, r * De) + proj(d.cep, De) + proj(D, 2 * De);
    if (sym) {
        const bool fold = uniform_t && d.cond_ch == 0;
        const double c0 = fold ? proj(D, 2 * De) : (hoist ? proj(D, D) : 2 * proj(D, D));
        double tr = trunk;
        if (fold && p->opt[JODO_OPT_ROT_STATS]) {
            tr -= proj(D, 2 * De);
            for (int b = 0; b < 2 * De / 32; ++b) tr += (double)(2 * De - 32 * b) / 2;
            cls[JODO_PROF_NODE_POST] += L * (double)p->n_gtiles * (double)(D - 2 * De) / 2;
        }
        cls[JODO_PROF_EDGE_UPDATE] += L * pair_iters * (tr + c0);
        if (p->opt[JODO_OPT_Z_SPLIT] != 0 && hoist && p->opt[JODO_OPT_PIN_UNIFORM_T] != (fold ? 2 : 1)) {
            const int rem = p->n_pitems % 1024;
            const int zw = rem > 0 ? (rem <= 256 ? 4 : ((p->opt[JODO_OPT_Z_SPLIT] == 2 && rem <= 512) ? 2 : 1)) : 1;
            cls[JODO_PROF_EDGE_UPDATE] += L * (double)rem * (zw - 1) * tr;
        }
    } else {
        cls[JODO_PROF_EDGE_UPDATE] += L * dir_iters * (trunk + proj(D, D));
    }
    cls[JODO_PROF_EPILOGUE] += strips * (proj(D, d.KNH) + proj(D / 2, D) + proj(d.nd, D / 2));
    const double eh = 2 * proj(De, d.KEH) + proj(De, 2 * De) + proj(32, De);
    cls[JODO_PROF_EPILOGUE] += (sym ? (double)(p->n_ut_pad / 32) : (double)((p->rows + 31) / 32)) * eh;
    for (int c = 0; c < JODO_PROF_COUNT; ++c) mfma_flops[c] = cls[c] * 4096.0;
    return JODO_OK;
}

extern "C" int jodo_plan_upload(jodo_plan* p, void* desc_dev, void* stream) {
    if (!p || !desc_dev) return jodo_set_error(JODO_ERR_ARG, "plan_upload: null");
    hipError_t e = hipMemcpyAsync(desc_dev, p->desc.data(), p->desc.size() * sizeof(int32_t), hipMemcpyHostToDevice,
                                  (hipStream_t)stream);
    if (e != hipSuccess) return jodo_set_error(JODO_ERR_LAUNCH, "plan_upload: %s", hipGetErrorString(e));
    return JODO_OK;
}
extern "C" int jodo_debug_set_timing_buffer(jodo_plan* p, void* dev16xu64) {
    if (!p) return jodo_set_error(JODO_ERR_ARG, "null plan");
    p->dbg_timing = dev16xu64;
    return JODO_OK;
}
extern "C" int jodo_debug_set_force_directed(jodo_plan* p, int on) {
    if (!p) return jodo_set_error(JODO_ERR_ARG, "null plan");
    if (on && p->opt[JODO_OPT_PIN_SYMMETRIC] == 1)
        return jodo_set_error(JODO_ERR_ARG, "set_force_directed: the plan is pinned to the symmetric path");
    p->force_directed = on;
    return JODO_OK;
}
extern "C" int jodo_plan_set_option(jodo_plan* p, int option, int value) {
    if (!p) return jodo_set_error(JODO_ERR_ARG, "null plan");
    if (option < 0 || option >= JODO_OPT_COUNT) return jodo_set_error(JODO_ERR_ARG, "plan_set_option: unknown option %d", option);
    if (option == JODO_OPT_NODE_POST_WAVES && value != 0 && value != 1 && value != 2 && value != 4 && value != 12 && value != 14)
        return jodo_set_error(JODO_ERR_ARG, "plan_set_option: node-post waves per strip must be 0 (auto), 1, 2 or 4");
    if (option == JODO_OPT_SPLIT_BF16 && (value < 0 || value > 2))
        return jodo_set_error(JODO_ERR_ARG, "plan_set_option: the split-bf16 form is 0 (off), 1 (pair update + node kernel) or 2 (also the attention kernel: experiments, measured slower), got %d", value);
    if ((option == JODO_OPT_FUSE_NEXT_QKV || option == JODO_OPT_DIR_SPLIT || option == JODO_OPT_NODE_MIX || option == JODO_OPT_HEADS_MIX || option == JODO_OPT_HALF_ROWS || option == JODO_OPT_PRE_EMBED || option == JODO_OPT_AB_PRE) && value != 0 && value != 1)
        return jodo_set_error(JODO_ERR_ARG, "plan_set_option: option %d is a switch (0 or 1), got %d", option, value);
    if (option == JODO_OPT_Z_SPLIT && (value < 0 || value > 2))
        return jodo_set_error(JODO_ERR_ARG, "plan_set_option: the Z split is 0 (off), 1 (four waves for a last round of <= 256 items) or 2 (also two waves up to 512), got %d", value);
    if (option == JODO_OPT_ROT_STATS && (value < 0 || value > 2))
        return jodo_set_error(JODO_ERR_ARG, "plan_set_option: rotated statistics are 0 (off), 1 (on) or 2 (on, uncentred Gram tiles: tests), got %d", value);
    if (option == JODO_OPT_PIN_SYMMETRIC && value == 1 && p->force_directed)
        return jodo_set_error(JODO_ERR_ARG, "plan_set_option: the symmetric pin contradicts jodo_debug_set_force_directed");
    if ((option == JODO_OPT_PIN_SYMMETRIC || option == JODO_OPT_PIN_UNIFORM_T) && (value < 0 || value > 2))
        return jodo_set_error(JODO_ERR_ARG, "plan_set_option: a pin is 0 (none), 1 or 2, got %d", value);
    if (option == JODO_OPT_ATTN_VARIANT && (value < 0 || value > 3))
        return jodo_set_error(JODO_ERR_ARG, "plan_set_option: attention variant must be 0..3, got %d", value);
    p->opt[option] = value;
    return JODO_OK;
}
extern "C" int jodo_debug_attn_schedule(const jodo_plan* p, int64_t* o) {
    if (!p || !o) return jodo_set_error(JODO_ERR_ARG, "attn_schedule: null");
    const int32_t* d = p->desc.data();
    int64_t iters = 0;
    for (int i = 0; i < p->n_aitems; ++i) iters += d[p->off_ai_t1 + i] - d[p->off_ai_t0 + i];
    o[0] = p->n_aitems; o[1] = iters; o[2] = p->amax_parts; o[3] = p->a_persist; o[4] = o[5] = o[6] = o[7] = 0;
    {
        std::vector<std::vector<std::pair<int, int>>> per((size_t)p->n_agroups);
        std::vector<std::vector<int>> parts((size_t)p->n_agroups);
        for (int i = 0; i < p->n_aitems; ++i) {
            const int g = d[p->off_ai_group + i];
            if (g < 0 || g >= p->n_agroups) return jodo_set_error(JODO_ERR_ARG, "attn_schedule: item %d names group %d", i, g);
            per[g].push_back({d[p->off_ai_t0 + i], d[p->off_ai_t1 + i]});
            parts[g].push_back(d[p->off_ai_part + i]);
        }
        for (int g = 0; g < p->n_agroups; ++g) {
            int nmax = 0, want_parts = 0;
            for (int k = 0; k < 128; ++k) {
                const int v = d[p->off_ag_node + (size_t)g * 128 + k];
                if (v >= 0) { nmax = std::max(nmax, (int)d[p->off_node_n + v]); want_parts = d[p->off_anode_parts + v]; }
            }
            const bool bigg = nmax > 128;
            if (bigg && !p->a_persist) { if (!per[g].empty()) return jodo_set_error(JODO_ERR_ARG, "attn_schedule: pair items for the big group %d", g); continue; }
            for (int i = 0; i < p->n_aitems; ++i)
                if (d[p->off_ai_group + i] == g && d[p->off_ai_dir + i] != (bigg ? 1 : 0)) return jodo_set_error(JODO_ERR_ARG, "attn_schedule: item %d of group %d has the wrong mode", i, g);
            std::sort(per[g].begin(), per[g].end());
            std::sort(parts[g].begin(), parts[g].end());
            int at = 0;
            for (const auto& it : per[g]) {
                if (it.first != at || it.second < it.first) return jodo_set_error(JODO_ERR_ARG, "attn_schedule: group %d offsets not tiled at %d", g, at);
                at = it.second;
            }
            const int want_len = bigg ? nmax : nmax / 2;
            if (at != want_len || per[g].empty()) return jodo_set_error(JODO_ERR_ARG, "attn_schedule: group %d covers %d of %d offsets", g, at, want_len);
            for (size_t q = 0; q < parts[g].size(); ++q)
                if (parts[g][q] != (int)q) return jodo_set_error(JODO_ERR_ARG, "attn_schedule: group %d partial indices are not 0..%d", g, (int)parts[g].size() - 1);
            if ((int)parts[g].size() != want_parts) return jodo_set_error(JODO_ERR_ARG, "attn_schedule: group %d has %d items, its atoms expect %d partials", g, (int)parts[g].size(), want_parts);
        }
    }
    if (p->a_persist) {
        int64_t lo = INT64_MAX, hi = 0, mi = 0, idle = 0;
        for (int s = 0; s < JODO_ATT_SLOTS; ++s) {
            const int k0 = d[p->off_aw_off + s], k1 = d[p->off_aw_off + s + 1];
            int64_t l = 0;
            for (int k = k0; k < k1; ++k) l += d[p->off_ai_t1 + k] - d[p->off_ai_t0 + k];
            lo = std::min(lo, l); hi = std::max(hi, l); mi = std::max<int64_t>(mi, k1 - k0); idle += (k1 == k0);
        }
        o[4] = lo; o[5] = hi; o[6] = mi; o[7] = idle;
    }
    return JODO_OK;
}
extern "C" int jodo_plan_set_split_weights(jodo_plan* p, const void* tape_dev, size_t bytes) {
    if (!p) return jodo_set_error(JODO_ERR_ARG, "null plan");
    if (tape_dev) {
        size_t total = 0, per_block = 0, node_block = 0, attn_block = 0;
        const int rc = p->dims.cond_ch > 0 ? jodo_dgt_split_cond_size(&p->cfg, &total, &per_block)
                                           : jodo_dgt_split_size(&p->cfg, &total, &per_block, &node_block, &attn_block);
        if (rc != JODO_OK) return rc;
        if (bytes != total) return jodo_set_error(JODO_ERR_ARG, "set_split_weights: %zu bytes, this configuration's tape has %zu", bytes, total);
    }
    p->split_w = tape_dev; p->split_bytes = tape_dev ? bytes : 0;
    return JODO_OK;
}
extern "C" int jodo_debug_set_max_blocks(jodo_plan* p, int mb) {
    if (!p) return jodo_set_error(JODO_ERR_ARG, "null plan");
    p->max_blocks = mb;
    return JODO_OK;
}
```

jodo_amd/csrc/dgt_plan.h:

```cpp
#pragma once
#include <stdint.h>
#include <stddef.h>
#include <vector>
#include "../../include/jodo_hip.h"

constexpr int JODO_ATT_SLOTS = 256;

struct DgtDims {
    int D, De, T, L, H, XH, SH, SC, C, r, nd, ch, cond_ch;
    int QKP;
    int ndp;
    int einp;
    int cnp, cep;
    int KNH, KEH;
    int MB;
    int64_t Mtot;
    float cutoff, edge_th;
    int wide;
};

struct PlanDev {
    const int* node_b;
    const int* node_i;
    const int* node_n;
    const int* node_noff;
    const int* node_eoff;
    const int* orig_n;
    const int* orig_noff;
    const int* orig_eoff;
    const int* item_strip;
    const int* item_t0;
    const int* item_t1;
    const int* item_part;
    const int* strip_parts;
    const int* pitem_strip;
    const int* pitem_t0;
    const int* pitem_t1;
    const int* ag_node;
    const int* ai_group;
    const int* ai_t0;
    const int* ai_t1;
    const int* ai_part;
    const int* ai_dir;
    const int* ad_group;
    const int* ad_t0;
    const int* ad_t1;
    const int* ad_part;
    const int* ad_big;
    const int* anode_parts;
    const int* aw_off;
    int a_persist;
    const int* ut_rows;
    int n_ut_pad;
    const int* gt_sa;
    const int* gt_sc;
    int n_gtiles;
    int n_agroups, n_aitems, n_aditems, amax_parts;
    int Nn, Nn_pad, n_strips, n_items, n_pitems, B, N, max_parts;
    int64_t rows;
};

struct WsLayout {
    size_t hid1, temb, tembs, mods, condh, condh2;
    size_t pos0, pos1, dpos, cpos, feat, h, hhat, astat, q, k, v, n2e, wrow, wcol, ua, ub, rmean, mfold, ffold, ahid, apred;
    size_t eflag, e, e2, ehid, epred, dposE, gramE;
    size_t ffold_s;
    size_t mfold_s;
    size_t total;
};

struct jodo_plan {
    jodo_cfg cfg;
    DgtDims dims;
    int B, N, Nn, Nn_pad, n_strips, n_items, n_pitems, max_parts;
    int n_agroups, n_aitems, n_aditems, amax_parts, n_ut_pad, n_gtiles;
    int a_persist;
    size_t off_aw_off;
    int has_big;
    size_t off_ag_node, off_ai_group, off_ai_t0, off_ai_t1, off_ai_part, off_ai_dir, off_ad_group, off_ad_t0, off_ad_t1, off_ad_part, off_ad_big, off_anode_parts, off_ut_rows, off_gt_sa, off_gt_sc;
    int64_t rows, dir_edges;
    std::vector<int32_t> desc;
    size_t off_node_b, off_node_i, off_node_n, off_node_noff, off_node_eoff, off_orig_n, off_orig_noff,
        off_orig_eoff, off_item_strip, off_item_t0, off_item_t1, off_item_part, off_strip_parts, off_pitem_strip, off_pitem_t0, off_pitem_t1;
    WsLayout ws;
    int prof_enabled;
    std::vector<void*> prof_ev;
    std::vector<int> prof_cls;
    std::vector<void*> prof_pool;
    int force_directed;
    void* dbg_timing;
    int max_blocks;
    int last_pos_buf;
    int last_e_buf;
    int opt[JODO_OPT_COUNT];
    const void* split_w;
    size_t split_bytes;
    int n_ai_dir;
    int pitems_single;
    int gt_cache_full, gt_cache_count;
};

int dgt_dims_from_cfg(const jodo_cfg* cfg, DgtDims* d);
```

Baseline: 173.6.

## Group gram tiles by row strip so one wave reuses row operand across columns

Adds a host-built list of gram items, each a row strip with a contiguous run of column-strip tiles, sorted so eligible-prefix tiles come first. A new strip-body kernel loads the row operand and its norms once, then loops over the column tiles, prefetching the next column while running the MFMA. This removes repeated row loads and per-tile metadata reads, but gives fewer, longer work items and so risks load imbalance. It also makes the 1024-strip round size a tunable option and adds a dirty flag that requires a re-upload after the lists change.

```diff
diff --git a/include/jodo_hip.h b/include/jodo_hip.h
--- a/include/jodo_hip.h
+++ b/include/jodo_hip.h
@@ -89,11 +89,14 @@
     JODO_OPT_AB_PRE = 11,
     JODO_OPT_Z_SPLIT = 12,
     JODO_OPT_SPLIT_BF16 = 13,
+    JODO_OPT_NODE_TAIL = 14,
+    JODO_OPT_NODE_ROUND = 15,
     JODO_OPT_COUNT
 };
 int jodo_plan_set_option(jodo_plan* plan, int option, int value);
 
 int jodo_debug_attn_schedule(const jodo_plan* plan, int64_t* out8);
+int jodo_debug_gram_items(const jodo_plan* plan, int64_t* out4);
 
 int jodo_debug_fetch(jodo_plan* plan, const void* workspace, int what, float* dst_dev, int64_t* count,
                      void* stream);
diff --git a/jodo_amd/capi.py b/jodo_amd/capi.py
--- a/jodo_amd/capi.py
+++ b/jodo_amd/capi.py
@@ -37,6 +37,8 @@
     dpm.argtypes = [i, i, i, i, p, p, p, p, i, i] + [p] * 11
     step.restype = dec.restype = dpm.restype = i
 
+
+OPT_NODE_POST_WAVES, OPT_NODE_MIX, OPT_NODE_TAIL, OPT_NODE_ROUND = 2, 7, 14, 15
 
 WALK_DIRECTED, WALK_PAIR = 0, 1
 
diff --git a/jodo_amd/csrc/dgt_forward.hip b/jodo_amd/csrc/dgt_forward.hip
--- a/jodo_amd/csrc/dgt_forward.hip
+++ b/jodo_amd/csrc/dgt_forward.hip
@@ -129,25 +129,29 @@
 }
 
 template <int R, int NW>
-__global__ __launch_bounds__(NW * 64, 1) void k_node_mix(KArgs A) {
+__global__ __launch_bounds__(NW * 64, 1) void k_node_mix(KArgs A, GramItems GI) {
     __shared__ float4 part[NW * 8 * 4 * 64];
-    const int wg = blockIdx.x, wave = threadIdx.x >> 6;
+    const int wave = threadIdx.x >> 6;
+    int wg = blockIdx.x;
     if (wg < A.mix_nw) { node_postw_body<R, NW>(A, wg + A.strip0, part); return; }
+    wg -= A.mix_nw;
     const int nab = (A.ab1 - A.ab0 + NW - 1) / NW;
-    if (wg < A.mix_nw + nab) {
-        const int it = A.ab0 + (wg - A.mix_nw) * NW + wave;
+    if (wg < nab) {
+        const int it = A.ab0 + wg * NW + wave;
         if (it < A.ab1) wide::node_ab_body<256>(A, it);
         return;
     }
-    const int t = A.g0 + (wg - A.mix_nw - nab) * NW + wave;
-    if (t < A.g1) wide::node_gram_body<256>(A, t);
+    const int t = A.g0 + (wg - nab) * NW + wave;
+    if (t >= A.g1) return;
+    if (GI.tail) wide::node_gram_strip_body<256>(A, GI, t); else wide::node_gram_body<256>(A, t);
 }
 
 int launch_node_post_256(jodo_plan* p, hipStream_t st, KArgs& A, bool with_ab, bool next_pre) {
     const DgtDims& d = p->dims;
     const int force = p->opt[JODO_OPT_NODE_POST_WAVES];
     const bool rem_only = force >= 10;
-    const int full = (force && !rem_only) ? (force == 1 ? p->n_strips : 0) : (p->n_strips / 1024) * 1024;
+    const int round = p->opt[JODO_OPT_NODE_ROUND];
+    const int full = (force && !rem_only) ? (force == 1 ? p->n_strips : 0) : (p->n_strips / round) * round;
     const int rem = p->n_strips - full;
     const int nw = rem_only ? force - 10 : (force ? force : (rem <= 256 ? 4 : (rem <= 512 ? 2 : 1)));
     const bool split_node = A.wsplit_node != nullptr && A.rot == 1;
@@ -175,14 +179,17 @@
             while (c < p->n_gtiles && sa[c] < full && sc[c] < full) ++c;
             p->gt_cache_full = full; p->gt_cache_count = c;
         }
-        const int gpre = A.rot ? p->gt_cache_count : 0;
+        const bool tail = p->opt[JODO_OPT_NODE_TAIL] != 0;
+        const int gpre = !A.rot ? 0 : (tail ? p->n_gitems_pre : p->gt_cache_count), gall = !A.rot ? 0 : (tail ? p->n_gitems : p->n_gtiles);
+        const int* dbase = static_cast<const int*>(static_cast<const void*>(A.pd.node_b)) - p->off_node_b;
+        const GramItems GI{dbase + p->off_gi_sa, dbase + p->off_gi_t0, dbase + p->off_gi_t1, dbase + p->off_gs_sc, tail ? 1 : 0};
         A.strip0 = full; A.mix_nw = rem; A.ab0 = 0; A.ab1 = 2 * full; A.g0 = 0; A.g1 = gpre;
         const int g1 = rem + (A.ab1 - A.ab0 + nw - 1) / nw + (A.g1 - A.g0 + nw - 1) / nw;
-        if (nw == 2) { if (d.r == 2) LAUNCH((k_node_mix<2, 2>), g1, 128, A); else LAUNCH((k_node_mix<4, 2>), g1, 128, A); }
-        else { if (d.r == 2) LAUNCH((k_node_mix<2, 4>), g1, 256, A); else LAUNCH((k_node_mix<4, 4>), g1, 256, A); }
-        A.strip0 = 0; A.mix_nw = 0; A.ab0 = 2 * full; A.ab1 = 2 * p->n_strips; A.g0 = gpre; A.g1 = A.rot ? p->n_gtiles : 0;
+        if (nw == 2) { if (d.r == 2) LAUNCH((k_node_mix<2, 2>), g1, 128, A, GI); else LAUNCH((k_node_mix<4, 2>), g1, 128, A, GI); }
+        else { if (d.r == 2) LAUNCH((k_node_mix<2, 4>), g1, 256, A, GI); else LAUNCH((k_node_mix<4, 4>), g1, 256, A, GI); }
+        A.strip0 = 0; A.mix_nw = 0; A.ab0 = 2 * full; A.ab1 = 2 * p->n_strips; A.g0 = gpre; A.g1 = gall;
         const int g2 = (A.ab1 - A.ab0 + 1) / 2 + (A.g1 - A.g0 + 1) / 2;
-        if (d.r == 2) LAUNCH((k_node_mix<2, 2>), g2, 128, A); else LAUNCH((k_node_mix<4, 2>), g2, 128, A);
+        if (d.r == 2) LAUNCH((k_node_mix<2, 2>), g2, 128, A, GI); else LAUNCH((k_node_mix<4, 2>), g2, 128, A, GI);
         A.ab0 = 0; A.g0 = 0;
         return JODO_OK;
     }
@@ -244,8 +251,8 @@
     }
     pro.reset();
     const int nblocks = (p->max_blocks >= 0 && p->max_blocks < d.L) ? p->max_blocks : d.L;
-    const bool fuse_pre = TUNED && p->opt[JODO_OPT_FUSE_NEXT_QKV] != 0 && nblocks > 1 && p->n_strips >= 1024;
-    const bool ab_pre = !fuse_pre && p->opt[JODO_OPT_AB_PRE] != 0 && nblocks > 1 && (!TUNED || (p->n_strips < 1024 && p->opt[JODO_OPT_NODE_POST_WAVES] == 0));
+    const bool fuse_pre = TUNED && p->opt[JODO_OPT_FUSE_NEXT_QKV] != 0 && nblocks > 1 && p->n_strips >= p->opt[JODO_OPT_NODE_ROUND];
+    const bool ab_pre = !fuse_pre && p->opt[JODO_OPT_AB_PRE] != 0 && nblocks > 1 && (!TUNED || (p->n_strips < p->opt[JODO_OPT_NODE_ROUND] && p->opt[JODO_OPT_NODE_POST_WAVES] == 0));
     int cur = 0;
     for (int l = 0; l < nblocks; ++l) {
         A.layer = l;
@@ -384,6 +391,7 @@
     if ((cond_x == nullptr) != (cond_edge_x == nullptr))
         return jodo_set_error(JODO_ERR_ARG, "dgt_forward: cond_x and cond_edge_x must both be given or both NULL");
     if (d.cond_ch > 0 && !context) return jodo_set_error(JODO_ERR_ARG, "dgt_forward: conditional model needs context");
+    if (p->desc_dirty) return jodo_set_error(JODO_ERR_ARG, "dgt_forward: JODO_OPT_NODE_ROUND changed the plan's lists after jodo_plan_upload; upload again");
     hipStream_t st = (hipStream_t)stream;
 
     KArgs A;
@@ -457,6 +465,7 @@
         case 3: src = ws + p->ws.hhat; n = (int64_t)p->Nn * p->amax_parts * p->dims.D; break;
         case 5: src = ws + p->ws.mods; n = p->dims.Mtot; break;
         case 6: src = ws + p->ws.q; n = (int64_t)p->Nn * p->dims.QKP; break;
+        case 7: src = ws + p->ws.gramE; n = p->rows; break;
         default: return jodo_set_error(JODO_ERR_ARG, "debug_fetch: unknown selector %d", what);
     }
     hipError_t e = hipMemcpyAsync(dst, src, (size_t)n * sizeof(float), hipMemcpyDeviceToDevice, (hipStream_t)stream);
diff --git a/jodo_amd/csrc/dgt_kernels_common.h b/jodo_amd/csrc/dgt_kernels_common.h
--- a/jodo_amd/csrc/dgt_kernels_common.h
+++ b/jodo_amd/csrc/dgt_kernels_common.h
@@ -39,6 +39,8 @@
     const float *xh, *edge_x, *cond_x, *cond_edge_x, *noise, *context;
     float *out_xh, *out_edge;
 };
+
+struct GramItems { const int *gi_sa, *gi_t0, *gi_t1, *gs_sc; int tail; };
 
 struct FoldOffs { int64_t c0[16], ine[16]; };
 
diff --git a/jodo_amd/csrc/dgt_kernels_wide.h b/jodo_amd/csrc/dgt_kernels_wide.h
--- a/jodo_amd/csrc/dgt_kernels_wide.h
+++ b/jodo_amd/csrc/dgt_kernels_wide.h
@@ -357,6 +357,93 @@
 }
 template <int D>
 __global__ __launch_bounds__(64) void k_node_gram(KArgs A) { node_gram_body<D>(A, A.g0 + (int)blockIdx.x); }
+
+template <int D>
+struct GramC {
+    float4 c0[(Dim<D>::ND - 2 * Dim<D>::NE) * 4], pc[(Dim<D>::ND - 2 * Dim<D>::NE) * 4];
+    int nc, noffc, ic, eoffc;
+};
+template <int D>
+__device__ __forceinline__ void gram_load_c(const KArgs& A, int sc, int j, int half, int lane, bool centre, GramC<D>& G) {
+    using X = Dim<D>;
+    const int vc = sc * 32 + j;
+    G.nc = A.pd.node_n[vc]; G.noffc = A.pd.node_noff[vc]; G.ic = A.pd.node_i[vc]; G.eoffc = A.pd.node_eoff[vc];
+    const int refc = (centre && G.nc > 0) ? G.noffc : vc;
+    const float4* cc = reinterpret_cast<const float4*>(A.wcol) + (size_t)sc * X::ND * 256 + lane;
+    const float4* mc = reinterpret_cast<const float4*>(A.wcol) + (size_t)(refc >> 5) * X::ND * 256 + (refc & 31) + 32 * half;
+#pragma unroll
+    for (int b = 2 * X::NE; b < X::ND; ++b)
+#pragma unroll
+        for (int q = 0; q < 4; ++q) {
+            G.c0[(b - 2 * X::NE) * 4 + q] = cc[(b * 4 + q) * 64];
+            G.pc[(b - 2 * X::NE) * 4 + q] = mc[(b * 4 + q) * 64];
+        }
+}
+template <int D>
+__device__ __forceinline__ void node_gram_strip_body(const KArgs& A, const GramItems& GI, int item) {
+    if (!rot_active(A)) return;
+    using X = Dim<D>;
+    constexpr int NQ = (X::ND - 2 * X::NE) * 4;
+    const int lane = threadIdx.x & 63, j = lane & 31, half = lane >> 5;
+    const int sa = GI.gi_sa[item], t0 = GI.gi_t0[item], t1 = GI.gi_t1[item];
+    const bool centre = A.rot != 2;
+    const float sgn = centre ? 1.f : 0.f;
+    GramC<D> G;
+    gram_load_c<D>(A, GI.gs_sc[t0], j, half, lane, centre, G);
+    float4 a[NQ];
+    float nRa[16];
+    int an[16], anoff[16], ai[16];
+    {
+        const int val = sa * 32 + j;
+        const int refa = (centre && A.pd.node_n[val] > 0) ? A.pd.node_noff[val] : val;
+        const float4* ra = reinterpret_cast<const float4*>(A.wrow) + (size_t)sa * X::ND * 256 + lane;
+        const float4* ma = reinterpret_cast<const float4*>(A.wcol) + (size_t)(refa >> 5) * X::ND * 256 + (refa & 31) + 32 * half;
+        float na[4] = {0.f, 0.f, 0.f, 0.f};
+#pragma unroll
+        for (int b = 2 * X::NE; b < X::ND; ++b)
+#pragma unroll
+            for (int q = 0; q < 4; ++q) {
+                const float4 a0 = ra[(b * 4 + q) * 64], pa = ma[(b * 4 + q) * 64];
+                const float4 v = make_float4(fmaf(sgn, pa.x, a0.x), fmaf(sgn, pa.y, a0.y), fmaf(sgn, pa.z, a0.z), fmaf(sgn, pa.w, a0.w));
+                a[(b - 2 * X::NE) * 4 + q] = v;
+                na[0] = fmaf(v.x, v.x, na[0]); na[1] = fmaf(v.y, v.y, na[1]); na[2] = fmaf(v.z, v.z, na[2]); na[3] = fmaf(v.w, v.w, na[3]);
+            }
+        const float nR = pair_sum((na[0] + na[1]) + (na[2] + na[3]));
+#pragma unroll
+        for (int s = 0; s < 16; ++s) {
+            const int m = 8 * (s >> 2) + 4 * half + (s & 3), va = sa * 32 + m;
+            nRa[s] = __shfl(nR, m);
+            an[s] = A.pd.node_n[va]; anoff[s] = A.pd.node_noff[va]; ai[s] = A.pd.node_i[va];
+        }
+    }
+#pragma unroll 1
+    for (int t = t0; t < t1; ++t) {
+        float4 c[NQ];
+        float nc4[4] = {0.f, 0.f, 0.f, 0.f};
+#pragma unroll
+        for (int k = 0; k < NQ; ++k) {
+            const float4 c0 = G.c0[k], pc = G.pc[k];
+            c[k] = make_float4(fmaf(-sgn, pc.x, c0.x), fmaf(-sgn, pc.y, c0.y), fmaf(-sgn, pc.z, c0.z), fmaf(-sgn, pc.w, c0.w));
+        }
+        const int nc = G.nc, noffc = G.noffc, ic = G.ic;
+        const size_t eoffc = (size_t)G.eoffc;
+        if (t + 1 < t1) gram_load_c<D>(A, GI.gs_sc[t + 1], j, half, lane, centre, G);
+        f32x16 acc = zero16();
+#pragma unroll
+        for (int k = 0; k < NQ; ++k) {
+            acc = __builtin_amdgcn_mfma_f32_32x32x2f32(a[k].x, c[k].x, acc, 0, 0, 0);
+            acc = __builtin_amdgcn_mfma_f32_32x32x2f32(a[k].y, c[k].y, acc, 0, 0, 0);
+            acc = __builtin_amdgcn_mfma_f32_32x32x2f32(a[k].z, c[k].z, acc, 0, 0, 0);
+            acc = __builtin_amdgcn_mfma_f32_32x32x2f32(a[k].w, c[k].w, acc, 0, 0, 0);
+            nc4[0] = fmaf(c[k].x, c[k].x, nc4[0]); nc4[1] = fmaf(c[k].y, c[k].y, nc4[1]); nc4[2] = fmaf(c[k].z, c[k].z, nc4[2]); nc4[3] = fmaf(c[k].w, c[k].w, nc4[3]);
+        }
+        const float nC = pair_sum((nc4[0] + nc4[1]) + (nc4[2] + nc4[3]));
+#pragma unroll
+        for (int s = 0; s < 16; ++s)
+            if (nc > 0 && an[s] > 0 && anoff[s] == noffc)
+                A.gramE[eoffc + (size_t)ai[s] * nc + ic] = nRa[s] + nC + 2.f * acc[s];
+    }
+}
 
 template <int D, int KQI>
 __global__ __launch_bounds__(64) void k_fold_coord(KArgs A, FoldOffs F, float* out, int need_rot, unsigned short* out_s = nullptr) {
diff --git a/jodo_amd/csrc/dgt_plan.cpp b/jodo_amd/csrc/dgt_plan.cpp
--- a/jodo_amd/csrc/dgt_plan.cpp
+++ b/jodo_amd/csrc/dgt_plan.cpp
@@ -24,6 +24,7 @@
     return out;
 }
 
+static void build_gram_items(jodo_plan* p);
 static void permute(std::vector<int32_t>& a, const std::vector<int>& ord) {
     std::vector<int32_t> b(a.size());
     for (size_t i = 0; i < ord.size(); ++i) b[i] = a[ord[i]];
@@ -99,6 +100,7 @@
     p->B = B; p->N = N; p->max_blocks = -1; p->last_pos_buf = 0; p->last_e_buf = 0;
     p->opt[JODO_OPT_FUSE_NEXT_QKV] = 1; p->opt[JODO_OPT_DIR_SPLIT] = 1; p->opt[JODO_OPT_NODE_POST_WAVES] = 0; p->opt[JODO_OPT_ATTN_VARIANT] = 0; p->opt[JODO_OPT_HEADS_MIX] = 1; p->opt[JODO_OPT_HALF_ROWS] = 1; p->opt[JODO_OPT_PRE_EMBED] = 1; p->opt[JODO_OPT_AB_PRE] = 1; p->opt[JODO_OPT_Z_SPLIT] = 1;
     p->opt[JODO_OPT_PIN_SYMMETRIC] = 0; p->opt[JODO_OPT_PIN_UNIFORM_T] = 0; p->opt[JODO_OPT_ROT_STATS] = 1; p->opt[JODO_OPT_NODE_MIX] = 1;
+    p->opt[JODO_OPT_NODE_TAIL] = 1; p->opt[JODO_OPT_NODE_ROUND] = 1024;
     p->opt[JODO_OPT_SPLIT_BF16] = 0; p->split_w = nullptr; p->split_bytes = 0;
     p->prof_enabled = 0; p->force_directed = 0; p->dbg_timing = nullptr;
 
@@ -337,6 +339,10 @@
         }
         p->n_gtiles = (int)gsa.size(); p->gt_cache_full = -1; p->gt_cache_count = 0;
         put(gsa, &p->off_gt_sa); put(gsc, &p->off_gt_sc);
+        const std::vector<int32_t> room(gsa.size(), 0);
+        put(room, &p->off_gi_sa); put(room, &p->off_gi_t0); put(room, &p->off_gi_t1); put(room, &p->off_gs_sc);
+        build_gram_items(p);
+        p->desc_dirty = 0;
     }
 
     const DgtDims& d = p->dims;
@@ -356,6 +362,64 @@
     w.ehid = take(R * d.KEH * f); w.epred = take(R * 4 * f); w.dposE = take(R * 4 * f); w.gramE = take(R * f);
     w.total = o;
     *out = p;
+    return JODO_OK;
+}
+
+static void build_gram_items(jodo_plan* p) {
+    const int round = p->opt[JODO_OPT_NODE_ROUND], full = (p->n_strips / round) * round, n = p->n_gtiles;
+    int32_t* d = p->desc.data();
+    std::vector<int> ord((size_t)n);
+    std::iota(ord.begin(), ord.end(), 0);
+    const int32_t* sa = d + p->off_gt_sa, *sc = d + p->off_gt_sc;
+    auto late = [&](int t) { return (sa[t] < full && sc[t] < full) ? 0 : 1; };
+    std::sort(ord.begin(), ord.end(), [&](int a, int b) {
+        if (late(a) != late(b)) return late(a) < late(b);
+        if (sa[a] != sa[b]) return sa[a] < sa[b];
+        return sc[a] < sc[b];
+    });
+    int ni = 0, npre = 0;
+    for (int k = 0; k < n; ++k) {
+        const int t = ord[k];
+        d[p->off_gs_sc + k] = sc[t];
+        if (k == 0 || sa[ord[k - 1]] != sa[t] || late(ord[k - 1]) != late(t)) {
+            if (ni > 0) d[p->off_gi_t1 + ni - 1] = k;
+            d[p->off_gi_sa + ni] = sa[t]; d[p->off_gi_t0 + ni] = k;
+            if (!late(t)) npre = ni + 1;
+            ++ni;
+        }
+    }
+    if (ni > 0) d[p->off_gi_t1 + ni - 1] = n;
+    p->n_gitems = ni; p->n_gitems_pre = npre; p->desc_dirty = 1;
+}
+
+extern "C" int jodo_debug_gram_items(const jodo_plan* p, int64_t* o) {
+    if (!p || !o) return jodo_set_error(JODO_ERR_ARG, "gram_items: null");
+    const int32_t* d = p->desc.data();
+    const int round = p->opt[JODO_OPT_NODE_ROUND], full = (p->n_strips / round) * round;
+    int parent = 0;
+    while (parent < p->n_gtiles && d[p->off_gt_sa + parent] < full && d[p->off_gt_sc + parent] < full) ++parent;
+    std::vector<std::pair<int, int>> mine, theirs;
+    int at = 0, seen_late = 0;
+    for (int i = 0; i < p->n_gitems; ++i) {
+        const int s = d[p->off_gi_sa + i], t0 = d[p->off_gi_t0 + i], t1 = d[p->off_gi_t1 + i];
+        if (t0 != at || t1 <= t0 || t1 > p->n_gtiles) return jodo_set_error(JODO_ERR_ARG, "gram_items: item %d covers [%d, %d), expected to start at %d", i, t0, t1, at);
+        at = t1;
+        if (s < 0 || s >= p->n_strips) return jodo_set_error(JODO_ERR_ARG, "gram_items: item %d names row strip %d", i, s);
+        for (int t = t0; t < t1; ++t) {
+            const int c = d[p->off_gs_sc + t];
+            if (c < 0 || c >= p->n_strips) return jodo_set_error(JODO_ERR_ARG, "gram_items: tile %d names column strip %d", t, c);
+            if (t > t0 && c <= d[p->off_gs_sc + t - 1]) return jodo_set_error(JODO_ERR_ARG, "gram_items: item %d repeats or disorders column strip %d", i, c);
+            const int is_late = (s < full && c < full) ? 0 : 1;
+            if (is_late != (i < p->n_gitems_pre ? 0 : 1) || is_late < seen_late) return jodo_set_error(JODO_ERR_ARG, "gram_items: tile %d of item %d is on the wrong side of the eligible prefix", t, i);
+            seen_late = is_late;
+            mine.push_back({s, c});
+        }
+    }
+    if (at != p->n_gtiles) return jodo_set_error(JODO_ERR_ARG, "gram_items: the items cover %d of %d tiles", at, p->n_gtiles);
+    for (int t = 0; t < p->n_gtiles; ++t) theirs.push_back({d[p->off_gt_sa + t], d[p->off_gt_sc + t]});
+    std::sort(mine.begin(), mine.end()); std::sort(theirs.begin(), theirs.end());
+    if (mine != theirs) return jodo_set_error(JODO_ERR_ARG, "gram_items: the items' tiles are not the tiles of the per-tile list");
+    o[0] = p->n_gitems; o[1] = p->n_gitems_pre; o[2] = p->n_gitems_pre > 0 ? d[p->off_gi_t1 + p->n_gitems_pre - 1] : 0; o[3] = parent;
     return JODO_OK;
 }
 
@@ -416,8 +480,8 @@
     cls[(p->opt[JODO_OPT_PRE_EMBED] != 0 && L > 0) ? JODO_PROF_NODE_PRE : JODO_PROF_PROLOGUE] += dir_iters * proj(De, d.einp + De);
     const int nqb = tuned ? 8 : d.SH;
     const double qkv = 2.0 * nqb * (D / 2) + proj(D, D);
-    const bool fuse_pre = tuned && p->opt[JODO_OPT_FUSE_NEXT_QKV] != 0 && L > 1 && p->n_strips >= 1024;
-    const bool ab_pre = !fuse_pre && p->opt[JODO_OPT_AB_PRE] != 0 && L > 1 && (!tuned || (p->n_strips < 1024 && p->opt[JODO_OPT_NODE_POST_WAVES] == 0));
+    const bool fuse_pre = tuned && p->opt[JODO_OPT_FUSE_NEXT_QKV] != 0 && L > 1 && p->n_strips >= p->opt[JODO_OPT_NODE_ROUND];
+    const bool ab_pre = !fuse_pre && p->opt[JODO_OPT_AB_PRE] != 0 && L > 1 && (!tuned || (p->n_strips < p->opt[JODO_OPT_NODE_ROUND] && p->opt[JODO_OPT_NODE_POST_WAVES] == 0));
     cls[JODO_PROF_NODE_PRE] += strips * qkv * ((fuse_pre || ab_pre) ? 1 : L);
     if (fuse_pre || ab_pre) cls[JODO_PROF_NODE_POST] += strips * qkv * (L - 1);
     cls[JODO_PROF_NODE_POST] += L * strips * (proj(De, D) + proj(r * D, D) + proj(D, r * D) + 2 * proj(D, D) + proj(d.cnp, D));
@@ -460,6 +524,7 @@
     hipError_t e = hipMemcpyAsync(desc_dev, p->desc.data(), p->desc.size() * sizeof(int32_t), hipMemcpyHostToDevice,
                                   (hipStream_t)stream);
     if (e != hipSuccess) return jodo_set_error(JODO_ERR_LAUNCH, "plan_upload: %s", hipGetErrorString(e));
+    p->desc_dirty = 0;
     return JODO_OK;
 }
 extern "C" int jodo_debug_set_timing_buffer(jodo_plan* p, void* dev16xu64) {
@@ -481,7 +546,9 @@
         return jodo_set_error(JODO_ERR_ARG, "plan_set_option: node-post waves per strip must be 0 (auto), 1, 2 or 4");
     if (option == JODO_OPT_SPLIT_BF16 && (value < 0 || value > 2))
         return jodo_set_error(JODO_ERR_ARG, "plan_set_option: the split-bf16 form is 0 (off), 1 (pair update + node kernel) or 2 (also the attention kernel: experiments, measured slower), got %d", value);
-    if ((option == JODO_OPT_FUSE_NEXT_QKV || option == JODO_OPT_DIR_SPLIT || option == JODO_OPT_NODE_MIX || option == JODO_OPT_HEADS_MIX || option == JODO_OPT_HALF_ROWS || option == JODO_OPT_PRE_EMBED || option == JODO_OPT_AB_PRE) && value != 0 && value != 1)
+    if (option == JODO_OPT_NODE_ROUND && (value < 1 || value > 65536))
+        return jodo_set_error(JODO_ERR_ARG, "plan_set_option: strips per full round must be 1 .. 65536, got %d", value);
+    if ((option == JODO_OPT_NODE_TAIL || option == JODO_OPT_FUSE_NEXT_QKV || option == JODO_OPT_DIR_SPLIT || option == JODO_OPT_NODE_MIX || option == JODO_OPT_HEADS_MIX || option == JODO_OPT_HALF_ROWS || option == JODO_OPT_PRE_EMBED || option == JODO_OPT_AB_PRE) && value != 0 && value != 1)
         return jodo_set_error(JODO_ERR_ARG, "plan_set_option: option %d is a switch (0 or 1), got %d", option, value);
     if (option == JODO_OPT_Z_SPLIT && (value < 0 || value > 2))
         return jodo_set_error(JODO_ERR_ARG, "plan_set_option: the Z split is 0 (off), 1 (four waves for a last round of <= 256 items) or 2 (also two waves up to 512), got %d", value);
@@ -493,7 +560,9 @@
         return jodo_set_error(JODO_ERR_ARG, "plan_set_option: a pin is 0 (none), 1 or 2, got %d", value);
     if (option == JODO_OPT_ATTN_VARIANT && (value < 0 || value > 3))
         return jodo_set_error(JODO_ERR_ARG, "plan_set_option: attention variant must be 0..3, got %d", value);
+    const bool relist = option == JODO_OPT_NODE_ROUND && p->opt[option] != value;
     p->opt[option] = value;
+    if (relist) { build_gram_items(p); p->gt_cache_full = -1; }
     return JODO_OK;
 }
 extern "C" int jodo_debug_attn_schedule(const jodo_plan* p, int64_t* o) {
diff --git a/jodo_amd/csrc/dgt_plan.h b/jodo_amd/csrc/dgt_plan.h
--- a/jodo_amd/csrc/dgt_plan.h
+++ b/jodo_amd/csrc/dgt_plan.h
@@ -77,7 +77,7 @@
     int a_persist;
     size_t off_aw_off;
     int has_big;
-    size_t off_ag_node, off_ai_group, off_ai_t0, off_ai_t1, off_ai_part, off_ai_dir, off_ad_group, off_ad_t0, off_ad_t1, off_ad_part, off_ad_big, off_anode_parts, off_ut_rows, off_gt_sa, off_gt_sc;
+    size_t off_ag_node, off_ai_group, off_ai_t0, off_ai_t1, off_ai_part, off_ai_dir, off_ad_group, off_ad_t0, off_ad_t1, off_ad_part, off_ad_big, off_anode_parts, off_ut_rows, off_gt_sa, off_gt_sc, off_gi_sa, off_gi_t0, off_gi_t1, off_gs_sc;
     int64_t rows, dir_edges;
     std::vector<int32_t> desc;
     size_t off_node_b, off_node_i, off_node_n, off_node_noff, off_node_eoff, off_orig_n, off_orig_noff,
@@ -98,6 +98,7 @@
     int n_ai_dir;
     int pitems_single;
     int gt_cache_full, gt_cache_count;
+    int n_gitems, n_gitems_pre, desc_dirty;
 };
 
 int dgt_dims_from_cfg(const jodo_cfg* cfg, DgtDims* d);
```

Result: no change. 174.9, median of 6 (+0.8%).
